# Spimp/sparc_ldpc

Hardware: AMD Instinct MI355X
Metric: decoded codewords/sec (T AMP iters) at L=512,M=512; achieved HBM GB/s vs roofline (higher is better)
Workload: dtype f32; 1 GPU; BASELINE configs[1]: L=512 M=512 R=1 P=4, T=64, single codeword; L=512, M=512, n=4608, T=64, backend=hadamard, precision=fp32, early_stop=False, parallelism=reps sharded over 1 GPU(s)

## Files before the change

### include/sparc_amp.h

```cpp
#ifndef SPARC_AMP_H
#define SPARC_AMP_H

#include <stdint.h>

#ifdef __cplusplus
extern "C" {
#endif

typedef struct sa_ctx sa_ctx;

enum {
  SA_OK = 0,
  SA_ERR_ARG = -1,
  SA_ERR_HIP = -2,
  SA_ERR_NOMEM = -3,
  SA_ERR_ORDERING = -4,
  SA_ERR_UNSUPPORTED = -5,
  SA_ERR_NO_DEVICE = -6
};

enum {
  SA_BACKEND_HADAMARD = 0,
  SA_BACKEND_DENSE = 1,
  SA_BACKEND_HOST = 2,
  SA_BACKEND_MATRIX = 3
};

enum { SA_PREC_F32 = 0, SA_PREC_F64 = 1 };

enum {
  SA_FLAG_NO_EARLY_STOP = 1,
  SA_FLAG_BETA0 = 0x100,
  SA_PTR_DEVICE = 0x200
};

int sa_create(sa_ctx** out, int L, int M, int n, const uint32_t* ordering,
              int backend, int precision, int device);

enum {
  SA_PLAN_DEFAULT = 0,
  SA_PLAN_SEC3 = 1 << 0,
  SA_PLAN_NO_SEC3 = 1 << 1,
  SA_PLAN_ROW16 = 1 << 2,
  SA_PLAN_NO_ROW16 = 1 << 3,
  SA_PLAN_NO_PT = 1 << 4,
  SA_PLAN_ZIL = 1 << 5,
  SA_PLAN_NO_ZIL = 1 << 6,
  SA_PLAN_WB8 = 1 << 7,
  SA_PLAN_WB16 = 1 << 8,
  SA_PLAN_NO_BANKS = 1 << 9,
  SA_PLAN_EAGER = 1 << 10,
  SA_PLAN_ONE_PASS = 1 << 11,
  SA_PLAN_NO_LANES = 1 << 12,
  SA_PLAN_SEC4Q = 1 << 13,
  SA_PLAN_NO_SEC4Q = 1 << 14,
  SA_PLAN_NO_FUSED_TAIL = 1 << 15,
  SA_PLAN_ALL = (1 << 16) - 1
};
int sa_create_ex(sa_ctx** out, int L, int M, int n, const uint32_t* ordering,
                 int backend, int precision, int device, int plan);

int sa_create_matrix(sa_ctx** out, int L, int M, int n, const double* A,
                     int precision, int device);

int sa_create_matrix_random(sa_ctx** out, int L, int M, int n, uint64_t seed, double scale,
                            int precision, int device);

int sa_subset(const sa_ctx* parent, const int64_t* sections, int Ls, sa_ctx** out);

int sa_create_twin(sa_ctx* src, sa_ctx** out);

void sa_destroy(sa_ctx* ctx);

int sa_Ab(sa_ctx* ctx, int B, const double* beta, double* out);

int sa_Az(sa_ctx* ctx, int B, const double* z, double* out);

int sa_amp(sa_ctx* ctx, int B, const double* y, const double* Pl, int T,
           const double* beta0, double* beta_out, int* iters_out, int flags);

int sa_reserve(sa_ctx* ctx, int B, int T);
int sa_stage(sa_ctx* ctx, int B, const double* y, const double* Pl, const double* beta0);
int sa_stage_power_batch(sa_ctx* ctx, int B, const double* Pl);
int sa_run(sa_ctx* ctx, int B, int T, int flags);
int sa_wait(sa_ctx* ctx);
int sa_fetch(sa_ctx* ctx, int B, double* beta_out, int* iters_out);
int sa_fetch_z(sa_ctx* ctx, int B, double* z_out);
int sa_fetch_y(sa_ctx* ctx, int B, double* y_out);
double sa_run_event_ms(sa_ctx* ctx);

int sa_profile(sa_ctx* ctx, int B, int T, int flags, double* out);
int sa_profile_kinds(void);
int sa_profile_rep(sa_ctx* ctx, int B, int T, int flags, int rep, double* out);
int sa_profile_dispatch(sa_ctx* ctx, int B, int T, int flags, double* out);

int sa_decide(sa_ctx* ctx, int B, int32_t* idx_out);

enum { SA_DECIDE_SLOTS = 4 };
int sa_decide_async(sa_ctx* ctx, int B, int slot);
int sa_decide_collect(sa_ctx* ctx, int B, int slot, int32_t* idx_out);


int sa_encode(sa_ctx* ctx, int B, const int32_t* idx, const double* noise);

int sa_stage_onehot(sa_ctx* ctx, int B, const int32_t* idx);

int sa_stage_onehot_scaled(sa_ctx* ctx, int B, const int32_t* idx, double scale);

int sa_llr(sa_ctx* ctx, int B, int l0, int ns, double* llr, int flags);

enum { SA_LLR_REFERENCE = 0, SA_LLR_TWO_SIDED = 1 };
int sa_llr_ex(sa_ctx* ctx, int B, int l0, int ns, double* llr, int flags, int mode, double clip);

int sa_soft_beta0(sa_ctx* ctx, int B, int l0, int ns, const double* app, int flags);

int sa_hard_cancel(sa_ctx* ctx, int B, int l0, int ns, const double* app, int flags, sa_ctx* dst,
                   int32_t* idx_out);

int sa_threshold(sa_ctx* ctx, int B, int l0, int ns, const double* app, int flags, double threshold,
                 int32_t* idx_out);

int sa_cancel(sa_ctx* ctx, int B, const int32_t* idx, sa_ctx* dst);

int sa_cancel_scaled(sa_ctx* ctx, int B, const int32_t* idx, double scale, sa_ctx* dst);

int sa_host_init(sa_ctx* ctx, int B, int T, const double* y, const double* Pl, const double* beta0,
                 const double* ab0);
int sa_host_tau(sa_ctx* ctx, int B, int t, int flags, int* stopped);
int sa_host_eta(sa_ctx* ctx, int B, int t, int flags, const double* az);
int sa_host_residual(sa_ctx* ctx, int B, int t, int flags, const double* ab);

int sa_draw_reps(const uint32_t* seeds, int count, int L, int M, int n, double sigma, int32_t* idx_out,
                 double* noise_out, int threads);
int sa_mc_stage(sa_ctx* ctx, int nreps, const int32_t* idx, const double* noise);
int sa_mc_run(sa_ctx* ctx, int B, int T, int flags, int32_t* dec_out, int32_t* iters_out, int32_t* errs_out,
              double* ms_out);
int sa_mc_draw(sa_ctx* ctx, int nreps, const uint32_t* seeds, const double* sigma, double* ms_out);
int sa_mc_fetch_draws(sa_ctx* ctx, int nreps, int32_t* idx_out, double* noise_out);
int sa_make_ordering(int L, int M, int n, uint32_t seed, uint32_t* out);

enum { SA_SE_MAX_M = 4096 };
int sa_se(int device, int B, int L, int M, int n, const double* Pl, const double* sigma, int T, int S,
          const uint32_t* seeds, const double* U, double* tau2_out, double* x_out, int64_t* miss_out,
          double* sec_out, double* ms_out);
int sa_se_draws(int device, int S, int M, const uint32_t* seeds, double* U_out);

typedef enum sa_sec_path {
  SA_SEC_K_SEC = 0,
  SA_SEC_K_SEC2 = 1,
  SA_SEC_K_SECB = 2,
  SA_SEC_DENSE = 3,
  SA_SEC_K_SEC4 = 4,
  SA_SEC_K_SEC43 = 5,
  SA_SEC_DENSE_I8 = 6,
  SA_SEC_MATRIX = 7,
  SA_SEC_K_SECG = 8,
  SA_SEC_K_SEC44 = 9
} sa_sec_path;
typedef enum sa_row_kernel {
  SA_ROW_K_ROW = 0,
  SA_ROW_K_ROW2 = 1,
  SA_ROW_K_ROWV16 = 2,
  SA_ROW_K_ROWV8 = 3,
  SA_ROW_K_ROW2_16 = 4,
  SA_ROW_K_ROWC = 5
} sa_row_kernel;
int sa_plan(sa_ctx* ctx, int B, int64_t* out8);
int sa_plan_batched(sa_ctx* ctx, int B, int64_t* out4);
int sa_info(const sa_ctx* ctx, int64_t* out8);
int sa_device_count(void);
const char* sa_last_error(void);
const char* sa_version(void);

#ifdef __cplusplus
}
#endif
#endif
```

### sparc_ldpc_amd/_lib.py

```python
from __future__ import annotations

import ctypes as ct
import os

import numpy as np

LIB_NAME = "libsparc_amp.so"
LIB_PATH = os.environ.get("SPARC_AMP_LIB") or os.path.join(os.path.dirname(os.path.abspath(__file__)), LIB_NAME)

SA_OK = 0
SA_ERR_ARG = -1
SA_ERR_HIP = -2
SA_ERR_NOMEM = -3
SA_ERR_ORDERING = -4
SA_ERR_UNSUPPORTED = -5
SA_ERR_NO_DEVICE = -6

SA_BACKEND_HADAMARD = 0
SA_BACKEND_DENSE = 1
SA_BACKEND_HOST = 2
SA_BACKEND_MATRIX = 3
SA_PREC_F32 = 0
SA_PREC_F64 = 1
SA_FLAG_NO_EARLY_STOP = 1
SA_FLAG_BETA0 = 0x100
SA_PTR_DEVICE = 0x200
SA_SE_MAX_M = 4096
SA_LLR_MODES = {"reference": 0, "two_sided": 1}

SA_PLAN = {
    "SEC3": 1 << 0, "NO_SEC3": 1 << 1, "ROW16": 1 << 2, "NO_ROW16": 1 << 3, "NO_PT": 1 << 4,
    "ZIL": 1 << 5, "NO_ZIL": 1 << 6, "WB8": 1 << 7, "WB16": 1 << 8, "NO_BANKS": 1 << 9, "EAGER": 1 << 10,
    "ONE_PASS": 1 << 11, "NO_LANES": 1 << 12, "SEC4Q": 1 << 13, "NO_SEC4Q": 1 << 14,
    "NO_FUSED_TAIL": 1 << 15,
}


def plan_bits(plan) -> int:
    if plan is None:
        return 0
    if isinstance(plan, int):
        return plan
    if isinstance(plan, str):
        plan = [plan]
    bits = 0
    for name in plan:
        key = name.upper()
        if key not in SA_PLAN:
            raise ValueError(f"unknown plan option {name!r}; known: {sorted(SA_PLAN)}")
        bits |= SA_PLAN[key]
    return bits

EXPORTS = (
    "sa_create", "sa_create_ex", "sa_create_matrix", "sa_create_matrix_random", "sa_subset", "sa_create_twin", "sa_destroy", "sa_Ab", "sa_Az", "sa_amp",
    "sa_reserve", "sa_stage", "sa_stage_power_batch", "sa_run", "sa_wait", "sa_fetch", "sa_fetch_z", "sa_fetch_y", "sa_run_event_ms",
    "sa_profile", "sa_profile_rep", "sa_profile_dispatch", "sa_profile_kinds", "sa_decide",
    "sa_decide_async", "sa_decide_collect", "sa_info", "sa_device_count", "sa_last_error", "sa_version",
    "sa_encode", "sa_stage_onehot", "sa_llr", "sa_llr_ex", "sa_soft_beta0", "sa_hard_cancel",
    "sa_threshold", "sa_cancel", "sa_plan", "sa_plan_batched", "sa_stage_onehot_scaled", "sa_cancel_scaled",
    "sa_host_init", "sa_host_tau", "sa_host_eta", "sa_host_residual",
    "sa_draw_reps", "sa_mc_stage", "sa_mc_run", "sa_make_ordering", "sa_mc_draw", "sa_mc_fetch_draws",
    "sa_se", "sa_se_draws",
)

_P = ct.c_void_p
_I = ct.c_int
_D = ct.POINTER(ct.c_double)
_SIG = {
    "sa_create": (_I, [ct.POINTER(_P), _I, _I, _I, ct.POINTER(ct.c_uint32), _I, _I, _I]),
    "sa_create_ex": (_I, [ct.POINTER(_P), _I, _I, _I, ct.POINTER(ct.c_uint32), _I, _I, _I, _I]),
    "sa_create_matrix": (_I, [ct.POINTER(_P), _I, _I, _I, _D, _I, _I]),
    "sa_create_matrix_random": (_I, [ct.POINTER(_P), _I, _I, _I, ct.c_uint64, ct.c_double, _I, _I]),
    "sa_subset": (_I, [_P, ct.POINTER(ct.c_int64), _I, ct.POINTER(_P)]),
    "sa_create_twin": (_I, [_P, ct.POINTER(_P)]),
    "sa_destroy": (None, [_P]),
    "sa_Ab": (_I, [_P, _I, _D, _D]),
    "sa_Az": (_I, [_P, _I, _D, _D]),
    "sa_amp": (_I, [_P, _I, _D, _D, _I, _D, _D, ct.POINTER(ct.c_int), _I]),
    "sa_reserve": (_I, [_P, _I, _I]),
    "sa_stage": (_I, [_P, _I, _D, _D, _D]),
    "sa_stage_power_batch": (_I, [_P, _I, _D]),
    "sa_run": (_I, [_P, _I, _I, _I]),
    "sa_wait": (_I, [_P]),
    "sa_fetch": (_I, [_P, _I, _D, ct.POINTER(ct.c_int)]),
    "sa_fetch_z": (_I, [_P, _I, _D]),
    "sa_fetch_y": (_I, [_P, _I, _D]),
    "sa_run_event_ms": (ct.c_double, [_P]),
    "sa_profile": (_I, [_P, _I, _I, _I, _D]),
    "sa_profile_rep": (_I, [_P, _I, _I, _I, _I, _D]),
    "sa_profile_dispatch": (_I, [_P, _I, _I, _I, _D]),
    "sa_profile_kinds": (_I, []),
    "sa_decide_async": (_I, [_P, _I, _I]),
    "sa_decide_collect": (_I, [_P, _I, _I, ct.POINTER(ct.c_int32)]),
    "sa_decide": (_I, [_P, _I, ct.POINTER(ct.c_int32)]),
    "sa_info": (_I, [_P, ct.POINTER(ct.c_int64)]),
    "sa_device_count": (_I, []),
    "sa_last_error": (ct.c_char_p, []),
    "sa_version": (ct.c_char_p, []),
    "sa_encode": (_I, [_P, _I, ct.POINTER(ct.c_int32), _D]),
    "sa_threshold": (_I, [_P, _I, _I, _I, _P, _I, ct.c_double, ct.POINTER(ct.c_int32)]),
    "sa_cancel": (_I, [_P, _I, ct.POINTER(ct.c_int32), _P]),
    "sa_plan": (_I, [_P, _I, ct.POINTER(ct.c_int64)]),
    "sa_plan_batched": (_I, [_P, _I, ct.POINTER(ct.c_int64)]),
    "sa_stage_onehot": (_I, [_P, _I, ct.POINTER(ct.c_int32)]),
    "sa_stage_onehot_scaled": (_I, [_P, _I, ct.POINTER(ct.c_int32), ct.c_double]),
    "sa_cancel_scaled": (_I, [_P, _I, ct.POINTER(ct.c_int32), ct.c_double, _P]),
    "sa_llr": (_I, [_P, _I, _I, _I, _P, _I]),
    "sa_llr_ex": (_I, [_P, _I, _I, _I, _P, _I, _I, ct.c_double]),
    "sa_soft_beta0": (_I, [_P, _I, _I, _I, _P, _I]),
    "sa_hard_cancel": (_I, [_P, _I, _I, _I, _P, _I, _P, ct.POINTER(ct.c_int32)]),
    "sa_host_init": (_I, [_P, _I, _I, _D, _D, _D, _D]),
    "sa_host_tau": (_I, [_P, _I, _I, _I, ct.POINTER(ct.c_int)]),
    "sa_host_eta": (_I, [_P, _I, _I, _I, _D]),
    "sa_host_residual": (_I, [_P, _I, _I, _I, _D]),
    "sa_draw_reps": (_I, [ct.POINTER(ct.c_uint32), _I, _I, _I, _I, ct.c_double, ct.POINTER(ct.c_int32), _D, _I]),
    "sa_mc_stage": (_I, [_P, _I, ct.POINTER(ct.c_int32), _D]),
    "sa_mc_run": (_I, [_P, _I, _I, _I, ct.POINTER(ct.c_int32), ct.POINTER(ct.c_int32), ct.POINTER(ct.c_int32), _D]),
    "sa_make_ordering": (_I, [_I, _I, _I, ct.c_uint32, ct.POINTER(ct.c_uint32)]),
    "sa_mc_draw": (_I, [_P, _I, ct.POINTER(ct.c_uint32), _D, _D]),
    "sa_mc_fetch_draws": (_I, [_P, _I, ct.POINTER(ct.c_int32), _D]),
    "sa_se": (_I, [_I, _I, _I, _I, _I, _D, _D, _I, _I, ct.POINTER(ct.c_uint32), _D, _D, _D, ct.POINTER(ct.c_int64), _D, _D]),
    "sa_se_draws": (_I, [_I, _I, _I, ct.POINTER(ct.c_uint32), _D]),
}

_lib = None

_SRC_DIR = os.path.join(os.path.dirname(os.path.abspath(__file__)), "csrc")
_INC_DIR = os.path.join(os.path.dirname(os.path.dirname(os.path.abspath(__file__))), "include")


def source_hash() -> str:
    import hashlib
    h = hashlib.sha256()
    files = sorted(f for f in os.listdir(_SRC_DIR) if f.endswith((".hip", ".h")) or f == "Makefile")
    paths = [os.path.join(_SRC_DIR, f) for f in files]
    if os.path.isdir(_INC_DIR):
        paths += [os.path.join(_INC_DIR, f) for f in sorted(os.listdir(_INC_DIR)) if f.endswith(".h")]
    for p in paths:
        h.update(os.path.basename(p).encode() + b"\0")
        with open(p, "rb") as fh:
            h.update(fh.read())
    return h.hexdigest()[:16]


class SparcAmpError(RuntimeError):

    def __init__(self, code: int, msg: str):
        super().__init__(f"libsparc_amp error {code}: {msg}")
        self.code = code


def load(path: str = LIB_PATH) -> ct.CDLL:
    global _lib
    if _lib is not None:
        return _lib
    if not os.path.exists(path):
        raise ImportError(
            f"{path} is missing: build it with `python -c 'import __graft_entry__ as g; g.build()'` "
            "(hipcc --offload-arch=gfx950). There is no CPU fallback.")
    lib = ct.CDLL(path)
    for name, (res, args) in _SIG.items():
        if not hasattr(lib, name):
            continue
        fn = getattr(lib, name)
        fn.restype = res
        fn.argtypes = args
    _lib = lib
    return lib


class SparcAmpArgumentError(SparcAmpError, AssertionError):
    """SA_ERR_ARG: the reference's ``assert`` cases.  An AssertionError, as the
    reference raises, and a SparcAmpError like every other refusal of the library."""


def check(rc: int) -> None:
    if rc != SA_OK:
        msg = load().sa_last_error().decode(errors="replace")
        if rc == SA_ERR_ARG:
            raise SparcAmpArgumentError(rc, msg)
        raise SparcAmpError(rc, msg)


def dptr(a: np.ndarray):
    return a.ctypes.data_as(_D)
# ... 5 lines not shown
```

### sparc_ldpc_amd/csrc/sa_common.h

```cpp
#pragma once
#include <hip/hip_runtime.h>
#include <hip/hip_ext.h>

#include <cfloat>
#include <cmath>
#include <cstdint>
#include <cstdio>
#include <cstdlib>
#include <cstring>
#include <algorithm>
#include <map>
#include <random>
#include <thread>
#include <string>
#include <tuple>
#include <type_traits>
#include <vector>

#include "sparc_amp.h"

namespace sa {

extern thread_local std::string g_err;
int fail(int code, const std::string& msg);
// ... 659 lines not shown
      *reinterpret_cast<float4*>(p + e0) = make_float4(x[i], x[i + 1], x[i + 2], x[i + 3]);
    } else {
#pragma unroll
      for (int q = 0; q < Q; ++q)
        if (e0 + q < M) p[e0 + q] = x[i + q];
    }
  }
}

template <typename real, int E>
__device__ __forceinline__ void load_section_any(const real* p, real (&x)[E], int lane, int M) {
  constexpr int Q = E < 4 ? E : 4;
#pragma unroll
  for (int i = 0; i < E; i += Q) {
    const int e0 = elem_index<E>(lane, i);
    if (Q == 4 && sizeof(real) == 4 && (M & 3) == 0 && e0 + 4 <= M) {
      const float4 t = *reinterpret_cast<const float4*>(p + e0);
      x[i] = t.x; x[i + 1] = t.y; x[i + 2] = t.z; x[i + 3] = t.w;
    } else {
#pragma unroll
      for (int q = 0; q < Q; ++q) x[i + q] = e0 + q < M ? p[e0 + q] : (real)0;
    }
  }
}

template <typename real, int E>
__device__ __forceinline__ void store_section_any(real* p, const real (&x)[E], int lane, int M) {
  constexpr int Q = E < 4 ? E : 4;
#pragma unroll
  for (int i = 0; i < E; i += Q) {
    const int e0 = elem_index<E>(lane, i);
    if (Q == 4 && sizeof(real) == 4 && (M & 3) == 0 && e0 + 4 <= M) {
      *reinterpret_cast<float4*>(p + e0) = make_float4(x[i], x[i + 1], x[i + 2], x[i + 3]);
    } else {
#pragma unroll
      for (int q = 0; q < Q; ++q)
        if (e0 + q < M) p[e0 + q] = x[i + q];
    }
  }
}


enum { SEC_AMP = 0, SEC_AZ = 1, SEC_AB = 2 };
enum { ROW_INIT0 = 0, ROW_INIT = 1, ROW_AMP = 2, ROW_ABOUT = 3 };

constexpr int kSpw = 4;
constexpr int kRowsPerBlk = 64;

template <typename real>
struct SecArgs {
  const uint16_t* __restrict__ inv;
  const uint16_t* __restrict__ invb;
  const uint16_t* __restrict__ invl;
  const uint32_t* __restrict__ hs;
  const ushort4* __restrict__ fwd;
  const ushort4* __restrict__ fwdb;
  const uint32_t* __restrict__ fwd2;
  const uint32_t* __restrict__ fwd3;
  const uint32_t* __restrict__ inv32;
  const real* __restrict__ c;
  const real* __restrict__ z;
  real* __restrict__ beta;
  real* __restrict__ beta_out;
  real* __restrict__ out;
  real* __restrict__ abp;
  real* __restrict__ bbp;
  const real* __restrict__ zzp;
  real* __restrict__ tau;
  int* __restrict__ iters;
  int L, M, n, w, nhi, G, NZ, T1, t, mode, early_stop;
  int cst;
  int RS;
  int pt;
  int B, NC;
  int zil;
  int gpx;
  real sqrt_n;
  const int* tb;
  int dead;
  int bzero;
  int32_t* dec;
  int itset;
};

template <typename real>
struct RowArgs {
  const real* __restrict__ tau;
  const real* __restrict__ y;
  const real* __restrict__ z_in;
  const real* __restrict__ bbp;
  const real* __restrict__ Pb;
  const real* __restrict__ abp;
  int n, G, Gb, NZ, T1, t, mode, early_stop;
  int Pbst;
  int pt;
  int Bc;
  int itset;
  real sqrt_n;
  real* __restrict__ z;
  real* __restrict__ zzp;
  real* __restrict__ out;
  int* __restrict__ iters;
  const int* tb;
};

constexpr int kZU = 10;
#define SA_ZU_EACH(X) X(0) X(1) X(2) X(3) X(4) X(5) X(6) X(7) X(8) X(9)
template <typename real, int NT = 256>
struct ZStage {
  using vec_t = typename std::conditional<sizeof(real) == 4, f4, d2v>::type;
  static constexpr int V = 16 / sizeof(real);
#define SA_ZU_DECL(u) vec_t t##u;
  SA_ZU_EACH(SA_ZU_DECL)
#undef SA_ZU_DECL
  int nv;
  __device__ __forceinline__ void issue(const real* zb, int n, int tid) {
    nv = ((reinterpret_cast<uintptr_t>(zb) & 15) == 0) ? n / V : 0;
    const vec_t* zv = reinterpret_cast<const vec_t*>(zb);
    const int last = nv > 0 ? nv - 1 : 0;
#define SA_ZU_LOAD(u) { const int j = u * NT + tid; t##u = zv[j < nv ? j : last]; }
    SA_ZU_EACH(SA_ZU_LOAD)
#undef SA_ZU_LOAD
  }
  __device__ __forceinline__ void store(real* zs, const real* zb, int n, int tid) const {
    vec_t* zsv = reinterpret_cast<vec_t*>(zs);
    const vec_t* zv = reinterpret_cast<const vec_t*>(zb);
#define SA_ZU_STORE(u) { const int j = u * NT + tid; if (j < nv) zsv[j] = t##u; }
    SA_ZU_EACH(SA_ZU_STORE)
#undef SA_ZU_STORE
    for (int j = kZU * NT + tid; j < nv; j += NT) zsv[j] = zv[j];
    for (int i = nv * V + tid; i < n; i += NT) zs[i] = zb[i];
    if (tid == 0) zs[n] = 0;
  }
};

template <typename real, int NT, int AUX = 0>
__device__ __forceinline__ bool stage_z_dma(const real* zb, real* zs, int n, int tid) {
  if (reinterpret_cast<uintptr_t>(zb) & 15) return false;
  const int lane = tid & 63, nbytes = n * (int)sizeof(real);
  for (int ch = tid >> 6; ch * 1024 < nbytes; ch += NT / 64) {
    const int off = ch * 1024 + lane * 16;
    if (off + 16 <= nbytes)
      __builtin_amdgcn_global_load_lds((__attribute__((address_space(1))) void*)((const char*)zb + off),
                                       (__attribute__((address_space(3))) void*)((char*)zs + ch * 1024), 16, 0, AUX);
  }
  return true;
}

template <typename real>
__device__ __forceinline__ void finish_z_dma(const real* zb, real* zs, int n, int tid) {
  const int n0 = n * (int)sizeof(real) / 16 * 16 / (int)sizeof(real);
  if (tid < n - n0) zs[n0 + tid] = zb[n0 + tid];
  if (tid == 0) zs[n] = 0;
}

template <int E, int KH>
__device__ __forceinline__ void load_buckets(const uint16_t* __restrict__ il, int h0, int nhi, int M,
                                             int lane, ushort4 (&tb)[KH][(E + 3) / 4]) {
  constexpr int Q = E < 4 ? E : 4;
#pragma unroll
  for (int hh = 0; hh < KH; ++hh) {
    const int h = h0 + hh < nhi ? h0 + hh : nhi - 1;
    const uint16_t* ih = il + (size_t)h * M;
#pragma unroll
    for (int i = 0; i < E; i += Q) {
      int e0 = elem_index<E>(lane, i);
// ... 158 lines not shown
```

### sparc_ldpc_amd/csrc/sa_glue.hip

```cpp
#include "sa_host.h"

namespace sa {

template <typename real>
__global__ void __launch_bounds__(256) k_colsum(const ushort4* __restrict__ fwd, const double* __restrict__ cd,
                                                const int32_t* __restrict__ idx, int ldi, int l0, int ns,
                                                const real* __restrict__ base, const double* __restrict__ add,
                                                real* __restrict__ out, int n, double sqrt_n, double amp) {
  extern __shared__ int32_t sidx[];
  const int b = blockIdx.y, r = blockIdx.x * 256 + threadIdx.x;
  for (int i = threadIdx.x; i < ns; i += 256) sidx[i] = idx[(size_t)b * ldi + i];
  __syncthreads();
  if (r >= n) return;
  double acc = 0.0;
  const int g0 = l0 / kSpw, g1 = (l0 + ns + kSpw - 1) / kSpw;
  for (int g = g0; g < g1; ++g) {
    const ushort4 f = fwd[(size_t)g * n + r];
    const unsigned short fq[4] = {f.x, f.y, f.z, f.w};
#pragma unroll
    for (int q = 0; q < 4; ++q) {
      const int l = g * kSpw + q;
      if (l < l0 || l >= l0 + ns || sidx[l - l0] < 0) continue;
      const unsigned k = fq[q] & 0x7fffu;
      const unsigned neg = (fq[q] >> 15) ^ (__popc(k & (unsigned)sidx[l - l0]) & 1u);
// ... 165 lines not shown

int grid_of(size_t tot) {
  const size_t g = (tot + 255) / 256;
  return (int)(g < 65536 ? (g > 0 ? g : 1) : 65536);
}

constexpr int kGlueMaxM = 8192;

int check_glue(sa_ctx* c, int B, int l0, int ns) {
  if (check_ctx(c)) return SA_ERR_ARG;
  if (B <= 0 || B > c->Bcap) return fail(SA_ERR_ARG, "batch larger than the context's workspace");
  if (l0 < 0 || ns <= 0 || l0 + ns > c->L) return fail(SA_ERR_ARG, "section range outside [0, L)");
  if (!c->power_set) return fail(SA_ERR_ARG, "power allocation not staged");
  if (c->M < 2) return fail(SA_ERR_UNSUPPORTED, "M < 2 carries no bits");
  if (!c->pow2) return fail(SA_ERR_UNSUPPORTED, "bit-level glue needs M a power of two (bits2indices, sparc_ldpc.py:317)");
  if (c->M > kGlueMaxM) return fail(SA_ERR_UNSUPPORTED, "SPARC<->LDPC glue stages a section in LDS: M <= 8192");
  return SA_OK;
}

int dev_in(sa_ctx* c, const double* p, size_t count, int flags, const double** out) {
  if (flags & SA_PTR_DEVICE) {
    *out = p;
    return SA_OK;
  }
  int rc = ensure_stage(c, count);
  if (rc) return rc;
  HIP_TRY(hipMemcpyAsync(c->at().d_stage, p, count * 8, hipMemcpyHostToDevice, c->at().stream));
  *out = c->at().d_stage;
  return SA_OK;
}

template <typename real>
int launch_colsum(sa_ctx* c, const int32_t* d_idx, int ldi, int l0, int ns, const real* base, const double* add,
                  real* out, int B, double amp = 1.0) {
  dim3 grid((c->n + 255) / 256, B);
  k_colsum<real><<<grid, 256, (size_t)ns * sizeof(int32_t), c->at().stream>>>(
      (const ushort4*)c->d_fwd, c->d_cd, d_idx, ldi, l0, ns, base, add, out, c->n, std::sqrt((double)c->n), amp);
  HIP_TRY(hipGetLastError());
  return SA_OK;
}

}

using namespace sa;

extern "C" {

int sa_encode(sa_ctx* c, int B, const int32_t* idx, const double* noise) {
  if (check_ctx(c)) return SA_ERR_ARG;
  if (B <= 0 || !idx) return fail(SA_ERR_ARG, "sa_encode: bad arguments");
  if (!c->power_set) return fail(SA_ERR_ARG, "sa_encode: power allocation not staged");
  if (int rc0 = check_tables(c, "sa_encode")) return rc0;
  if (!c->pow2) return fail(SA_ERR_UNSUPPORTED, "sa_encode: the row-parallel encoder needs M a power of two");
  HIP_TRY(hipSetDevice(c->device));
  int rc = ensure_workspace(c, B, c->Tcap > 0 ? c->Tcap : 1);
  if (rc) return rc;
  sa_lane& ln = c->at();
  for (size_t i = 0; i < (size_t)B * c->L; ++i)
    if (idx[i] < 0 || idx[i] >= c->M) return fail(SA_ERR_ARG, "sa_encode: index outside [0, M)");
  HIP_TRY(hipMemcpyAsync(c->d_idx, idx, (size_t)B * c->L * sizeof(int32_t), hipMemcpyHostToDevice, ln.stream));
  const double* d_noise = nullptr;
  if (noise && (rc = dev_in(c, noise, (size_t)B * c->n, 0, &d_noise))) return rc;
  if ((rc = y_begin_write(c, ln.stream, B))) return rc;
  rc = c->prec == SA_PREC_F64
           ? launch_colsum<double>(c, c->d_idx, c->L, 0, c->L, nullptr, d_noise, (double*)ln.d_y, B)
           : launch_colsum<float>(c, c->d_idx, c->L, 0, c->L, nullptr, d_noise, (float*)ln.d_y, B);
  if (rc) return rc;
  HIP_TRY(hipStreamSynchronize(ln.stream));
  return y_mark(c);
}

namespace {
int stage_onehot_impl(sa_ctx* c, int B, const int32_t* idx, double scale, bool allow_empty) {
  if (check_ctx(c)) return SA_ERR_ARG;
  if (B <= 0 || B > c->Bcap || !idx) return fail(SA_ERR_ARG, "sa_stage_onehot: bad arguments");
  if (!c->power_set) return fail(SA_ERR_ARG, "sa_stage_onehot: power allocation not staged");
  if (!std::isfinite(scale)) return fail(SA_ERR_ARG, "sa_stage_onehot: scale must be finite");
  if (c->dead) return fail(SA_ERR_UNSUPPORTED, "sa_stage_onehot: M must be a power of two (bits2indices)");
  for (size_t i = 0; i < (size_t)B * c->L; ++i)
    if (idx[i] >= c->M || (idx[i] < 0 && !(allow_empty && idx[i] == -1)))
      return fail(SA_ERR_ARG, "sa_stage_onehot: index outside [0, M)");
  HIP_TRY(hipSetDevice(c->device));
  sa_lane& ln = c->at();
  ln.fused_B = 0;
  HIP_TRY(hipMemcpyAsync(c->d_idx, idx, (size_t)B * c->L * sizeof(int32_t), hipMemcpyHostToDevice, ln.stream));
  const size_t tot = (size_t)B * c->L * c->M;
  if (c->prec == SA_PREC_F64)
    k_onehot<double><<<grid_of(tot), 256, 0, ln.stream>>>(c->d_idx, c->d_cd, c->L, c->M, B, scale, (double*)ln.d_beta);
  else
    k_onehot<float><<<grid_of(tot), 256, 0, ln.stream>>>(c->d_idx, c->d_cd, c->L, c->M, B, scale, (float*)ln.d_beta);
  HIP_TRY(hipGetLastError());
  HIP_TRY(hipStreamSynchronize(ln.stream));
  return SA_OK;
}
}

int sa_stage_onehot(sa_ctx* c, int B, const int32_t* idx) { return stage_onehot_impl(c, B, idx, 1.0, false); }

int sa_stage_onehot_scaled(sa_ctx* c, int B, const int32_t* idx, double scale) {
  return stage_onehot_impl(c, B, idx, scale, true);
}

int sa_llr(sa_ctx* c, int B, int l0, int ns, double* llr, int flags) {
  return sa_llr_ex(c, B, l0, ns, llr, flags, SA_LLR_REFERENCE, INFINITY);
}

int sa_llr_ex(sa_ctx* c, int B, int l0, int ns, double* llr, int flags, int mode, double clip) {
  int rc = check_glue(c, B, l0, ns);
  if (rc) return rc;
  if (!llr) return fail(SA_ERR_ARG, "sa_llr: llr is NULL");
  if (mode != SA_LLR_REFERENCE && mode != SA_LLR_TWO_SIDED) return fail(SA_ERR_ARG, "sa_llr_ex: unknown mode");
  if (!(clip >= 0.0)) return fail(SA_ERR_ARG, "sa_llr_ex: clip must be positive, or 0 / +inf for none");
  const double lim = std::isinf(clip) ? 0.0 : clip;
  HIP_TRY(hipSetDevice(c->device));
  sa_lane& ln = c->at();
  const int lgM = ilog2(c->M);
  const size_t cnt = (size_t)B * ns * lgM;
  double* d_out = llr;
  if (!(flags & SA_PTR_DEVICE)) {
    if ((rc = ensure_stage(c, cnt))) return rc;
    d_out = ln.d_stage;
  }
  const size_t lds = (size_t)c->M * sizeof(double);
  if (mode == SA_LLR_TWO_SIDED) {
    if (c->prec == SA_PREC_F64)
      k_llr2<double><<<B * ns, 64, lds, ln.stream>>>((const double*)ln.d_beta, c->d_cd, c->L, c->M, lgM, l0, ns, lim,
                                                     d_out);
    else
      k_llr2<float><<<B * ns, 64, lds, ln.stream>>>((const float*)ln.d_beta, c->d_cd, c->L, c->M, lgM, l0, ns, lim,
                                                    d_out);
  } else {
    if (c->prec == SA_PREC_F64)
      k_llr<double><<<B * ns, 64, lds, ln.stream>>>((const double*)ln.d_beta, c->d_cd, c->L, c->M, lgM, l0, ns, d_out);
    else
      k_llr<float><<<B * ns, 64, lds, ln.stream>>>((const float*)ln.d_beta, c->d_cd, c->L, c->M, lgM, l0, ns, d_out);
    if (lim > 0.0) k_llr_clip<<<grid_of(cnt), 256, 0, ln.stream>>>(d_out, cnt, lim);
  }
  HIP_TRY(hipGetLastError());
  if (!(flags & SA_PTR_DEVICE)) HIP_TRY(hipMemcpyAsync(llr, d_out, cnt * 8, hipMemcpyDeviceToHost, ln.stream));
  HIP_TRY(hipStreamSynchronize(ln.stream));
  return SA_OK;
}

int sa_soft_beta0(sa_ctx* c, int B, int l0, int ns, const double* app, int flags) {
  int rc = check_glue(c, B, l0, ns);
  if (rc) return rc;
  if (!app) return fail(SA_ERR_ARG, "sa_soft_beta0: app is NULL");
  HIP_TRY(hipSetDevice(c->device));
  sa_lane& ln = c->at();
  ln.fused_B = 0;
  const int lgM = ilog2(c->M);
  const size_t na = (size_t)B * ns * lgM;
  const double* d_app = app;
  if (!(flags & SA_PTR_DEVICE)) {
    if ((rc = ensure_stage(c, na))) return rc;
    HIP_TRY(hipMemcpyAsync(ln.d_stage, app, na * 8, hipMemcpyHostToDevice, ln.stream));
    d_app = ln.d_stage;
  }
  const size_t tot = (size_t)B * c->L * c->M, lds = (size_t)c->M * sizeof(double);
  if (c->prec == SA_PREC_F64) {
    if (ns < c->L) k_rescale<double><<<grid_of(tot), 256, 0, ln.stream>>>((double*)ln.d_beta, c->d_cd, c->L, c->M, l0, ns, B);
    k_soft_sec<double><<<B * ns, 64, lds, ln.stream>>>(d_app, c->d_cd, c->L, c->M, lgM, l0, ns, (double*)ln.d_beta);
  } else {
    if (ns < c->L) k_rescale<float><<<grid_of(tot), 256, 0, ln.stream>>>((float*)ln.d_beta, c->d_cd, c->L, c->M, l0, ns, B);
    k_soft_sec<float><<<B * ns, 64, lds, ln.stream>>>(d_app, c->d_cd, c->L, c->M, lgM, l0, ns, (float*)ln.d_beta);
  }
  HIP_TRY(hipGetLastError());
  HIP_TRY(hipStreamSynchronize(ln.stream));
  return SA_OK;
}

int sa_hard_cancel(sa_ctx* c, int B, int l0, int ns, const double* app, int flags, sa_ctx* dst, int32_t* idx_out) {
  if (dst && check_tables(c, "sa_hard_cancel")) return SA_ERR_UNSUPPORTED;
  int rc = check_glue(c, B, l0, ns);
  if (rc) return rc;
  if (!app) return fail(SA_ERR_ARG, "sa_hard_cancel: app is NULL");
  if (dst && (dst->n != c->n || dst->prec != c->prec || dst->device != c->device))
    return fail(SA_ERR_ARG, "sa_hard_cancel: dst must share n, precision and device");
  HIP_TRY(hipSetDevice(c->device));
  if (dst && (rc = ensure_workspace(dst, B, dst->Tcap > 0 ? dst->Tcap : 1))) return rc;
  sa_lane& ln = c->at();
  const int lgM = ilog2(c->M);
  const double* d_app = nullptr;
  if ((rc = dev_in(c, app, (size_t)B * ns * lgM, flags, &d_app))) return rc;
  k_app_idx<<<(B * ns + 255) / 256, 256, 0, ln.stream>>>(d_app, lgM, ns, B, c->d_idx);
  HIP_TRY(hipGetLastError());
  if (dst) {
    if ((rc = y_sync(c)) || (rc = y_begin_write(dst, ln.stream, B))) return rc;
    rc = c->prec == SA_PREC_F64
             ? launch_colsum<double>(c, c->d_idx, ns, l0, ns, (const double*)ln.d_y, nullptr, (double*)dst->at().d_y, B)
             : launch_colsum<float>(c, c->d_idx, ns, l0, ns, (const float*)ln.d_y, nullptr, (float*)dst->at().d_y, B);
    if (rc) return rc;
  }
  if (idx_out)
    HIP_TRY(hipMemcpyAsync(idx_out, c->d_idx, (size_t)B * ns * sizeof(int32_t), hipMemcpyDeviceToHost, ln.stream));
  HIP_TRY(hipStreamSynchronize(ln.stream));
  return dst ? y_mark(dst) : SA_OK;
}

int sa_threshold(sa_ctx* c, int B, int l0, int ns, const double* app, int flags, double threshold,
                 int32_t* idx_out) {
  int rc = check_glue(c, B, l0, ns);
  if (rc) return rc;
  if (!app || !idx_out) return fail(SA_ERR_ARG, "sa_threshold: null argument");
  HIP_TRY(hipSetDevice(c->device));
  sa_lane& ln = c->at();
  const int lgM = ilog2(c->M);
  const double* d_app = nullptr;
  if ((rc = dev_in(c, app, (size_t)B * ns * lgM, flags, &d_app))) return rc;
  k_threshold<<<B * ns, 256, (size_t)c->M * sizeof(double), ln.stream>>>(d_app, c->M, lgM, ns, threshold, c->d_idx);
  HIP_TRY(hipGetLastError());
  HIP_TRY(hipMemcpyAsync(idx_out, c->d_idx, (size_t)B * ns * sizeof(int32_t), hipMemcpyDeviceToHost, ln.stream));
  HIP_TRY(hipStreamSynchronize(ln.stream));
  return SA_OK;
}

int sa_cancel_scaled(sa_ctx* c, int B, const int32_t* idx, double scale, sa_ctx* dst) {
  if (check_ctx(c) || check_ctx(dst)) return SA_ERR_ARG;
  if (int rc0 = check_tables(c, "sa_cancel")) return rc0;
  if (!c->pow2) return fail(SA_ERR_UNSUPPORTED, "sa_cancel: needs M a power of two");
  if (B <= 0 || B > c->Bcap || !idx) return fail(SA_ERR_ARG, "sa_cancel: bad arguments");
  if (!c->power_set) return fail(SA_ERR_ARG, "sa_cancel: power allocation not staged");
  if (dst->n != c->n || dst->prec != c->prec || dst->device != c->device)
    return fail(SA_ERR_ARG, "sa_cancel: dst must share n, precision and device");
  for (size_t i = 0; i < (size_t)B * c->L; ++i)
    if (idx[i] >= c->M) return fail(SA_ERR_ARG, "sa_cancel: index >= M");
  if (!std::isfinite(scale)) return fail(SA_ERR_ARG, "sa_cancel: scale must be finite");
  HIP_TRY(hipSetDevice(c->device));
  int rc;
  if ((rc = ensure_workspace(dst, B, dst->Tcap > 0 ? dst->Tcap : 1))) return rc;
  sa_lane& ln = c->at();
  HIP_TRY(hipMemcpyAsync(c->d_idx, idx, (size_t)B * c->L * sizeof(int32_t), hipMemcpyHostToDevice, ln.stream));
  if ((rc = y_sync(c)) || (rc = y_begin_write(dst, ln.stream, B))) return rc;
// ... 12 lines not shown
```

### sparc_ldpc_amd/csrc/sa_host.h

```cpp
#pragma once
#include "sa_common.h"

namespace sa {

struct Prof {
  std::vector<std::tuple<int, hipEvent_t, hipEvent_t>> ev;
  int rep = 1;
  bool dispatch = false;
  int kind = 0;
  int begin(hipStream_t s, int k) {
    kind = k;
    if (dispatch) return 0;
    hipEvent_t a = nullptr, b = nullptr;
    if (add(&a, &b)) return -1;
    return hipEventRecord(a, s) == hipSuccess ? 0 : -1;
  }
  void end(hipStream_t s) {
    if (!dispatch) (void)hipEventRecord(std::get<2>(ev.back()), s);
  }
  int add(hipEvent_t* a, hipEvent_t* b) {
    *a = *b = nullptr;
    if (hipEventCreate(a) != hipSuccess || hipEventCreate(b) != hipSuccess) return -1;
    ev.emplace_back(kind, *a, *b);
    return 0;
  }
  ~Prof() {
    for (auto& e : ev) {
      (void)hipEventDestroy(std::get<1>(e));
      (void)hipEventDestroy(std::get<2>(e));
    }
  }
};

enum { K_SEC = 0, K_ROW = 1, K_DAZ = 2, K_DDEN = 3, K_DAB = 4, K_QNT = 5, K_NKINDS = 6 };

}

struct sa_lane {
  hipStream_t stream = nullptr;
  hipEvent_t ev0 = nullptr, ev1 = nullptr;
  void *d_y = nullptr, *d_z = nullptr, *d_beta = nullptr, *d_abp = nullptr;
  void *d_bbp = nullptr, *d_zzp = nullptr, *d_tau = nullptr;
  void* d_beta2 = nullptr;
  int* d_iters = nullptr;
  double* d_stage = nullptr;
  size_t stage_cap = 0;
  int beta2_cap = 0;
  std::map<std::tuple<int, int, int, int>, hipGraphExec_t> graphs;
  hipEvent_t y_ev = nullptr;
  unsigned long long y_ver = 0;
  bool y_read = false;
  int32_t *h_dec = nullptr, *d_dec = nullptr;
  int fused_B = 0;
  int row_B = 0, row_T = 0;
};

struct sa_ctx {
  sa::Prof* prof = nullptr;
  enum { kLanes = 2 };
  sa_lane lane[kLanes];
  int cur = 0;
  sa_lane& at() { return lane[cur]; }
  const sa_lane& at() const { return lane[cur]; }
  bool lanes_on = false;
  unsigned long long y_ver = 0;
  int y_lane = 0;
  std::vector<double> h_Pl;
  std::vector<double> h_Plb;
  int L = 0, M = 0, n = 0, w = 0, nhi = 0, backend = 0, prec = 0, device = 0;
  int plan = 0;
  bool pow2 = true;
  int Mu = 0, dead = 0;
  int G = 0, NZ = 0, E = 1;
  int n_cus = 256;
  int Gb = 0, CB = 0;
  int WB = 8;
  int gpx = 1 << 20;
  size_t secb_lds = 0;
  int RS = 1, KS = 1, Gd = 0;
  size_t lda = 0;
  size_t sec_lds = 0;
  int G2 = 0;
  int G3 = 0;
  bool sec3 = false;
  size_t sec3_lds = 0;
  int G4 = 0;
  bool sec4q = false;
  size_t sec4q_lds = 0;
  uint32_t* d_fwd3 = nullptr;
  bool pt_on = false;
  bool sec4 = false;
  size_t sec4_lds = 0;
  int NZ16 = 0;
  int NZh = 0;
  bool row16 = false;
  int NZ4 = 0, NZ2 = 0;
  bool zil_last = false;
  size_t sec2_lds = 0;
  std::vector<uint32_t> ordering;
  uint16_t* d_inv = nullptr;
  bool big = false;
  uint32_t* d_inv32 = nullptr;
  uint16_t* d_invb = nullptr;
  uint16_t* d_fwdb = nullptr;
  uint16_t* d_invl = nullptr;
  uint32_t* d_hs = nullptr;
  bool borrowed = false;
  bool invb_done = false;
  uint16_t* d_fwd = nullptr;
  uint32_t* d_fwd2 = nullptr;
  void* d_A = nullptr;
  int8_t *d_A8 = nullptr, *d_AT8 = nullptr, *d_zq = nullptr, *d_bq = nullptr;
  double *d_zsc = nullptr, *d_bsc0 = nullptr, *d_bfix = nullptr;
  long long np8 = 0, LMp8 = 0;
  int Bp8 = 0;
  long long np = 0, nk = 0, LMy = 0;
  void *d_AT = nullptr, *d_xz = nullptr, *d_xb = nullptr;
  int fg_cap = 0;
  double cmax = 0;
  int Bcap = 0, Tcap = 0;
  void *d_out = nullptr, *d_c = nullptr, *d_azp = nullptr;
  int* d_stop = nullptr;
  int32_t* d_idx = nullptr;
  double* d_cd = nullptr;
  double P = 0;
  bool power_set = false;
  void* d_cb = nullptr;
  void* d_Pb = nullptr;
  void* d_P1 = nullptr;
  bool pb_on = false;
  bool shared_power = false;
  size_t bytes = 0;
  int last_B = 0, last_T = 0;
  int32_t* h_dec = nullptr;
  int32_t* d_dec = nullptr;
  size_t dec_cap = 0;
  hipEvent_t dec_ev[SA_DECIDE_SLOTS] = {};
// ... 47 lines not shown
  return SA_OK;
}

constexpr int kI8MinB = 4;
constexpr int kI8MaxS = 16;
constexpr int kFMinB = 4;
constexpr int kFMaxS = 16;

inline size_t rsz(const sa_ctx* c) { return c->prec == SA_PREC_F64 ? 8 : 4; }

inline bool is_dense(const sa_ctx* c) { return c->backend == SA_BACKEND_DENSE || c->backend == SA_BACKEND_MATRIX; }
inline bool use_i8(const sa_ctx* c, int B) { return c->backend == SA_BACKEND_DENSE && B >= kI8MinB; }
inline bool use_fgemm(const sa_ctx* c, int B) { return c->backend == SA_BACKEND_MATRIX && B >= kFMinB; }
inline bool use_batched(const sa_ctx* c, int B) { return c->CB > 0 && B >= 4; }

inline bool zil_for(const sa_ctx* c, int B) {
  const bool on = (c->plan & SA_PLAN_NO_ZIL) ? false : true;
  return on && c->backend == SA_BACKEND_HADAMARD && use_batched(c, B) && c->CB * (int)rsz(c) == 16;
}

int dense_parts(const sa_ctx* c, int B);

struct Plan {
  sa_sec_path sec = SA_SEC_K_SEC;
  sa_row_kernel row = SA_ROW_K_ROW;
  int nz = 0;
  int G = 0, Gb = 0;
  int pt = 0;
  int rs = 1;
  int CB = 1;
  bool zil = false;
  bool dense() const { return sec == SA_SEC_DENSE || sec == SA_SEC_DENSE_I8 || sec == SA_SEC_MATRIX; }
  bool batched() const { return sec == SA_SEC_K_SECB; }
  bool multiwave() const {
    return sec == SA_SEC_K_SEC2 || sec == SA_SEC_K_SEC4 || sec == SA_SEC_K_SEC43 || sec == SA_SEC_K_SEC44;
  }
  bool row_sets_iters() const { return row == SA_ROW_K_ROW2 || row == SA_ROW_K_ROW2_16; }
  bool it_row() const { return !dense() && !batched() && row_sets_iters(); }
  bool bzero() const { return sec == SA_SEC_K_SEC4 || sec == SA_SEC_K_SEC43 || sec == SA_SEC_K_SEC44; }
};

inline Plan plan_for(const sa_ctx* c, int B) {
  Plan p;
  const bool f32 = c->prec == SA_PREC_F32;
  p.zil = zil_for(c, B);
  if (p.zil) {
    p.row = SA_ROW_K_ROWC; p.nz = c->NZ2;
  } else if ((long long)B * c->NZ < 4LL * c->n_cus) {
    if (c->row16 && B == 1) { p.row = SA_ROW_K_ROW2_16; p.nz = c->NZh; }
    else { p.row = SA_ROW_K_ROW2; p.nz = c->NZ16; }
  } else if (c->n % (f32 ? 4 : 2) == 0 && (long long)B * (f32 ? c->NZ4 : c->NZ2) >= 2LL * c->n_cus) {
    p.row = SA_ROW_K_ROWV16; p.nz = f32 ? c->NZ4 : c->NZ2;
  } else if (f32 && c->n % 2 == 0 && (long long)B * c->NZ2 >= 2LL * c->n_cus) {
    p.row = SA_ROW_K_ROWV8; p.nz = c->NZ2;
  } else {
    p.row = SA_ROW_K_ROW; p.nz = c->NZ;
  }
  const int wgs = c->G * B;
  p.rs = std::min(4, std::max(1, (c->n_cus + wgs - 1) / wgs));
  if (is_dense(c)) {
    p.sec = use_i8(c, B) ? SA_SEC_DENSE_I8 : (use_fgemm(c, B) ? SA_SEC_MATRIX : SA_SEC_DENSE);
    p.G = dense_parts(c, B);
    p.Gb = c->Gd;
  } else if (use_batched(c, B)) {
    p.sec = SA_SEC_K_SECB;
    p.G = p.Gb = c->Gb;
    p.CB = c->CB;
  } else if (c->backend == SA_BACKEND_HADAMARD && c->G2 > 0 && c->G2 * B * 2 >= c->n_cus) {
    p.sec = c->sec3 ? SA_SEC_K_SEC43 : (c->sec4q ? SA_SEC_K_SEC44 : (c->sec4 ? SA_SEC_K_SEC4 : SA_SEC_K_SEC2));
    p.G = p.Gb = c->sec3 ? c->G3 : (c->sec4q ? c->G4 : c->G2);
    if (p.sec != SA_SEC_K_SEC2 && p.row_sets_iters() && c->pt_on) p.pt = p.row == SA_ROW_K_ROW2_16 ? 16 : kRow2Rows;
  } else {
    p.sec = c->big ? SA_SEC_K_SECG : SA_SEC_K_SEC;
    p.G = p.Gb = c->G;
  }
  return p;
}

inline bool fused_tail(const sa_ctx* c, const Plan& p, int T, int flags) {
  return p.bzero() && p.it_row() && (flags & SA_FLAG_NO_EARLY_STOP) && T > 0 && c->dead == 0 && !c->prof &&
         !(c->plan & SA_PLAN_NO_FUSED_TAIL);
}

template <typename real>
SecArgs<real> sec_args(sa_ctx* c, const Plan& p, int mode, int t, int early_stop, const int* tb = nullptr) {
  SecArgs<real> a;
  const sa_lane& ln = c->at();
  a.inv = c->d_inv; a.inv32 = c->d_inv32; a.invb = c->d_invb; a.invl = c->d_invl; a.hs = c->d_hs;
  a.fwd = (const ushort4*)c->d_fwd;
  a.fwdb = (const ushort4*)c->d_fwdb; a.fwd2 = c->d_fwd2; a.fwd3 = c->d_fwd3; a.c = (const real*)c->d_c;
  a.z = (const real*)ln.d_z; a.beta = (real*)ln.d_beta; a.beta_out = (real*)ln.d_beta; a.out = (real*)c->d_out;
  a.abp = (real*)ln.d_abp; a.bbp = (real*)ln.d_bbp; a.zzp = (const real*)ln.d_zzp;
  a.tau = (real*)ln.d_tau; a.iters = ln.d_iters;
  a.L = c->L; a.M = c->M; a.n = c->n; a.w = c->w; a.nhi = c->nhi; a.G = c->G; a.NZ = p.nz;
  a.T1 = c->Tcap + 1; a.t = t; a.mode = mode; a.early_stop = early_stop;
  a.RS = 1;
  a.pt = 0;
  a.B = 0; a.NC = 0; a.zil = 0; a.gpx = 1 << 20;
  a.cst = c->pb_on ? c->L : 0;
  if (c->pb_on) a.c = (const real*)c->d_cb;
  a.sqrt_n = (real)std::sqrt((double)c->n);
  a.tb = tb;
  a.dead = c->dead;
  a.bzero = 0;
  a.dec = nullptr;
  a.itset = 0;
  return a;
}

template <typename real>
RowArgs<real> row_args(sa_ctx* c, const Plan& p, int mode, int t, int early_stop, int G, int Gb, const int* tb = nullptr) {
  RowArgs<real> a;
  const sa_lane& ln = c->at();
  a.y = (const real*)ln.d_y; a.z = (real*)ln.d_z; a.z_in = a.z; a.abp = (const real*)ln.d_abp;
  a.bbp = (const real*)ln.d_bbp; a.zzp = (real*)ln.d_zzp; a.tau = (const real*)ln.d_tau;
  a.out = (real*)c->d_out;
  a.n = c->n; a.G = G; a.NZ = p.nz;
  a.Gb = Gb; a.T1 = c->Tcap + 1; a.t = t; a.mode = mode;
  a.early_stop = early_stop;
  a.sqrt_n = c->backend != SA_BACKEND_HADAMARD ? (real)1 : (real)std::sqrt((double)c->n);
  a.Pb = c->pb_on ? (const real*)c->d_Pb : (const real*)c->d_P1;
  a.Pbst = c->pb_on ? 1 : 0;
  a.pt = 0;
  a.Bc = 0;
  a.tb = tb;
  a.iters = ln.d_iters;
  a.itset = 0;
  return a;
}

template <typename F>
void parallel_for(int count, int grain, F f) {
  const int blocks = (count + grain - 1) / grain;
  unsigned nth = std::thread::hardware_concurrency();
  nth = nth == 0 ? 1 : (nth > 16 ? 16 : nth);
  if ((int)nth > blocks) nth = blocks > 0 ? blocks : 1;
  auto run = [&](int t) {
    for (int b = t; b < blocks; b += (int)nth)
      for (int i = b * grain; i < count && i < (b + 1) * grain; ++i) f(i);
  };
  std::vector<std::thread> th;
  for (int t = 1; t < (int)nth; ++t) th.emplace_back(run, t);
  run(0);
  for (auto& x : th) x.join();
}

int check_ctx(const sa_ctx* c);
int check_tables(const sa_ctx* c, const char* what);
int dev_alloc(sa_ctx* c, void** p, size_t bytes);
void dev_free(void* p);
using GraphMap = std::map<std::tuple<int, int, int, int>, hipGraphExec_t>;
void graphs_clear(GraphMap& m);
void drop_graphs(sa_ctx* c);
int sync_all(sa_ctx* c);
inline void lane_switch(sa_ctx* c, int k) { c->cur = k; }
int lanes_release(sa_ctx* c);
int row_flush(sa_ctx* c, int k);
inline int tail_settle(sa_ctx* c) {
  c->at().fused_B = 0;
  return row_flush(c, c->cur);
}
int y_sync(sa_ctx* c, int k);
int y_begin_write(sa_ctx* c, int k, hipStream_t s, int B);
int y_mark(sa_ctx* c, int k);
inline int y_sync(sa_ctx* c) { return y_sync(c, c->cur); }
inline int y_begin_write(sa_ctx* c, hipStream_t s, int B) { return y_begin_write(c, c->cur, s, B); }
inline int y_mark(sa_ctx* c) { return y_mark(c, c->cur); }
int ensure_workspace(sa_ctx* c, int B, int T);
int ensure_stage(sa_ctx* c, sa_lane& l, size_t count);
int upload(sa_ctx* c, sa_lane& l, void* dst, const double* src, size_t count);
int download(sa_ctx* c, sa_lane& l, double* dst, const void* src, size_t count);
inline int ensure_stage(sa_ctx* c, size_t count) { return ensure_stage(c, c->at(), count); }
inline int upload(sa_ctx* c, void* dst, const double* src, size_t count) { return upload(c, c->at(), dst, src, count); }
inline int download(sa_ctx* c, double* dst, const void* src, size_t count) { return download(c, c->at(), dst, src, count); }
int set_power(sa_ctx* c, const double* Pl);
int ensure_invb(sa_ctx* c);
int create_impl(sa_ctx** out, int L, int M, int n, const uint32_t* ordering, int backend, int prec, int device,
                int plan, const sa_ctx* share = nullptr);
extern __global__ void k_fill32(uint32_t* p, uint32_t v, size_t nw);

template <typename real>
int launch_sec(sa_ctx* c, const Plan& p, int B, int mode, int t, int es, void* bin = nullptr, void* bout = nullptr);
template <typename real>
int launch_sec2(sa_ctx* c, const Plan& p, int B, int t, int es, void* bin, void* bout, int bzero = 0,
                int32_t* dec = nullptr, int itset = 0);
hipError_t sec_lds_attrs();

template <typename real>
int launch_secb(sa_ctx* c, const Plan& p, int B, int t, int es, const int* tb = nullptr);
hipError_t secb_lds_attrs();
bool secb_no_static_lds();

template <typename real>
int launch_row(sa_ctx* c, const Plan& p, int B, int mode, int t, int es, int G, int Gb, int itset = 0,
               const int* tb = nullptr);
int launch_decide(sa_ctx* c, int B, int32_t* idx);

int dense_den_groups(const sa_ctx* c);
template <typename real>
int dense_start(sa_ctx* c, const Plan& p, int B);
template <typename real>
int dense_iter(sa_ctx* c, const Plan& p, int B, int t, int es);
template <typename real>
int dense_ab(sa_ctx* c, const Plan& p, int B);
template <typename real>
int dense_az(sa_ctx* c, const Plan& p, int B);
int ensure_i8(sa_ctx* c, int B);
int ensure_fgemm(sa_ctx* c, int B);
int i8_set_bfix(sa_ctx* c);
int build_dense(sa_ctx* c);
int matrix_init(sa_ctx* c);
hipError_t dense_lds_attrs();

void mc_release(sa_ctx* c);
hipError_t mc_lds_attrs();

#ifdef SA_STAMPS
hipError_t stamps_add_sec(unsigned long long* out);
hipError_t stamps_add_secb(unsigned long long* out);
#endif

}
```

### sparc_ldpc_amd/csrc/sa_mc.hip

```cpp
#include "sa_host.h"
#include "legacy_mt.h"
#include "legacy_mt_dev.h"

#include <thread>

namespace sa {

using legacy_rng::LegacyMT;


struct McArgs {
  int* rep;
  int* tb;
  int* done;
  int* fresh;
  int* fin_list;
  int* fresh_list;
  int* ctl;
  int* iters;
  int32_t* dec;
  int32_t* its;
  int32_t* errs;
  const int32_t* idx;
  const double* noise;
// ... 402 lines not shown
}

int sa_mc_stage(sa_ctx* c, int nreps, const int32_t* idx, const double* noise) {
  if (check_tables(c, "sa_mc_stage")) return SA_ERR_UNSUPPORTED;
  if (nreps <= 0 || !idx || !noise) return fail(SA_ERR_ARG, "sa_mc_stage: bad arguments");
  for (size_t i = 0; i < (size_t)nreps * c->L; ++i)
    if (idx[i] < 0 || idx[i] >= c->M) return fail(SA_ERR_ARG, "sa_mc_stage: index outside [0, M)");
  HIP_TRY(hipSetDevice(c->device));
  lane_switch(c, 0);
  if (int rc = mc_ensure_reps(c, nreps)) return rc;
  HIP_TRY(hipMemcpyAsync(c->d_mc_idx, idx, (size_t)nreps * c->L * sizeof(int32_t), hipMemcpyHostToDevice, c->at().stream));
  HIP_TRY(hipMemcpyAsync(c->d_mc_noise, noise, (size_t)nreps * c->n * sizeof(double), hipMemcpyHostToDevice,
                         c->at().stream));
  HIP_TRY(hipStreamSynchronize(c->at().stream));
  c->mc_nreps = nreps;
  return SA_OK;
}

int sa_mc_draw(sa_ctx* c, int nreps, const uint32_t* seeds, const double* sigma, double* ms_out) {
  if (int rc = check_tables(c, "sa_mc_draw")) return rc;
  if (nreps <= 0 || !seeds || !sigma) return fail(SA_ERR_ARG, "sa_mc_draw: bad arguments");
  if (!c->pow2 || c->M < 2)
    return fail(SA_ERR_UNSUPPORTED, "sa_mc_draw: the device generator draws randint(0, M) for M a power of two only");
  if (c->n > (1 << 27) || c->L > (1 << 27)) return fail(SA_ERR_UNSUPPORTED, "sa_mc_draw: n or L above 2^27");
  HIP_TRY(hipSetDevice(c->device));
  lane_switch(c, 0);
  int rc;
  if ((rc = mc_ensure_reps(c, nreps))) return rc;
  if ((rc = mc_ensure_seeds(c, nreps))) return rc;
  c->mc_nreps = 0;
  sa_lane& ln = c->at();
  HIP_TRY(hipMemcpyAsync(c->d_mc_seeds, seeds, (size_t)nreps * sizeof(uint32_t), hipMemcpyHostToDevice, ln.stream));
  HIP_TRY(hipMemcpyAsync(c->d_mc_sigma, sigma, (size_t)nreps * sizeof(double), hipMemcpyHostToDevice, ln.stream));
  HIP_TRY(hipMemsetAsync(c->d_mc_err, 0, sizeof(int), ln.stream));
  HIP_TRY(hipEventRecord(ln.ev0, ln.stream));
  k_mc_draw<<<nreps, legacy_rng_dev::kThreads, 0, ln.stream>>>(c->d_mc_seeds, c->d_mc_sigma, c->d_mc_idx,
                                                                c->d_mc_noise, c->L, c->M, c->n,
                                                                legacy_rng_dev::randn_chunk_cap(c->n), c->d_mc_err);
  HIP_TRY(hipGetLastError());
  HIP_TRY(hipEventRecord(ln.ev1, ln.stream));
  int err = 0;
  HIP_TRY(hipMemcpyAsync(&err, c->d_mc_err, sizeof(int), hipMemcpyDeviceToHost, ln.stream));
  HIP_TRY(hipStreamSynchronize(ln.stream));
  if (err) return fail(SA_ERR_HIP, "sa_mc_draw: a rep's randn ran into the chunk cap");
  if (ms_out) {
    float ms = -1.f;
    HIP_TRY(hipEventElapsedTime(&ms, ln.ev0, ln.ev1));
    *ms_out = ms;
  }
  c->mc_nreps = nreps;
  return SA_OK;
}

int sa_mc_fetch_draws(sa_ctx* c, int nreps, int32_t* idx_out, double* noise_out) {
  if (check_ctx(c)) return SA_ERR_ARG;
  if (nreps <= 0 || nreps > c->mc_nreps) return fail(SA_ERR_ARG, "sa_mc_fetch_draws: nreps outside the staged reps");
  HIP_TRY(hipSetDevice(c->device));
  hipStream_t st = c->lane[0].stream;
  if (idx_out)
    HIP_TRY(hipMemcpyAsync(idx_out, c->d_mc_idx, (size_t)nreps * c->L * sizeof(int32_t), hipMemcpyDeviceToHost, st));
  if (noise_out)
    HIP_TRY(hipMemcpyAsync(noise_out, c->d_mc_noise, (size_t)nreps * c->n * sizeof(double), hipMemcpyDeviceToHost, st));
  HIP_TRY(hipStreamSynchronize(st));
  return SA_OK;
}

int sa_mc_run(sa_ctx* c, int B, int T, int flags, int32_t* dec_out, int32_t* iters_out, int32_t* errs_out,
              double* ms_out) {
  if (check_ctx(c)) return SA_ERR_ARG;
  if (B < 4 || B > kMcStepThreads || T <= 0) return fail(SA_ERR_ARG, "sa_mc_run: B in [4, 1024], T > 0");
  if (c->mc_nreps <= 0) return fail(SA_ERR_ARG, "sa_mc_run: no reps staged (sa_mc_stage)");
  if (!c->shared_power || c->pb_on) return fail(SA_ERR_ARG, "sa_mc_run: one power allocation must be staged");
  if (c->backend != SA_BACKEND_HADAMARD || !c->pow2 || c->big || !zil_for(c, B))
    return fail(SA_ERR_UNSUPPORTED, "sa_mc_run: needs the batched codeword-interleaved Hadamard decode "
                                    "(k_secb + k_rowc)");
  HIP_TRY(hipSetDevice(c->device));
  lane_switch(c, 0);
  int rc;
  if ((rc = ensure_workspace(c, B, T))) return rc;
  if ((rc = ensure_invb(c))) return rc;
  if ((rc = mc_ensure_slots(c, B))) return rc;
  sa_lane& ln = c->at();
  ln.row_B = ln.row_T = 0;
  ln.fused_B = 0;
  if (!c->h_mc_live) {
    HIP_TRY(hipHostMalloc((void**)&c->h_mc_live, 4 * sizeof(int), hipHostMallocDefault));
    for (auto& e : c->mc_ev) HIP_TRY(hipEventCreateWithFlags(&e, hipEventDisableTiming));
  }
  const int es = (flags & SA_FLAG_NO_EARLY_STOP) ? 0 : 1;
  const bool f64 = c->prec == SA_PREC_F64;
  const int nreps = c->mc_nreps;
  const Plan p = plan_for(c, B);
  c->zil_last = true;
  {
    const int S = c->slot_cap, n0 = std::min(B, nreps);
    std::vector<int> h(6 * (size_t)S + 8, -1);
    for (int b = 0; b < S; ++b) {
      const bool on = b < n0;
      h[b] = on ? b : -1;
      h[S + b] = on ? 0 : -1;
      h[2 * (size_t)S + b] = -1;
      h[3 * (size_t)S + b] = on ? 1 : 0;
      h[5 * (size_t)S + b] = b;
    }
    int* ctl = h.data() + 6 * (size_t)S;
    ctl[0] = n0;
    ctl[1] = n0;
    ctl[2] = nreps;
    ctl[3] = 0;
    ctl[4] = n0;
    HIP_TRY(hipMemcpyAsync(c->d_slots, h.data(), h.size() * sizeof(int), hipMemcpyHostToDevice, ln.stream));
    HIP_TRY(hipMemsetAsync(ln.d_beta, 0, (size_t)B * c->L * c->M * rsz(c), ln.stream));
    k_fill32<<<(B + 255) / 256, 256, 0, ln.stream>>>((uint32_t*)ln.d_iters, 0xffffffffu, (size_t)B);
    k_fill32<<<(nreps + 255) / 256, 256, 0, ln.stream>>>((uint32_t*)(c->d_mc_its + c->mc_cap), 0u, (size_t)nreps);
    HIP_TRY(hipGetLastError());
    HIP_TRY(hipStreamSynchronize(ln.stream));
  }
  HIP_TRY(hipEventRecord(ln.ev0, ln.stream));
  const McArgs a = mc_args(c, B, T);
  if ((rc = f64 ? mc_encode_all<double>(c, a, nreps) : mc_encode_all<float>(c, a, nreps))) return rc;
  if ((rc = f64 ? mc_turnover<double>(c, a) : mc_turnover<float>(c, a))) return rc;
  const int K = 8;
  const auto key = std::make_tuple(B, T, K, flags & 0xff);
  auto it = c->mc_graphs.find(key);
  if (it == c->mc_graphs.end()) {
    hipGraphExec_t ex = nullptr;
    rc = capture_graph(ln.stream, [&] {
      return f64 ? mc_iterations<double>(c, p, B, T, K, es) : mc_iterations<float>(c, p, B, T, K, es);
    }, &ex);
    if (rc) return rc;
    it = c->mc_graphs.emplace(key, ex).first;
  }
  const long long max_replays = ((long long)(nreps + B - 1) / B * T + T + K - 1) / K + 2;
  int* live_dev = c->d_slots + 6 * c->slot_cap + 1;
  long long r = 0;
  for (; r < max_replays; ++r) {
    HIP_TRY(hipGraphLaunch(it->second, ln.stream));
    HIP_TRY(hipMemcpyAsync(c->h_mc_live + (r & 3), live_dev, sizeof(int), hipMemcpyDeviceToHost, ln.stream));
    HIP_TRY(hipEventRecord(c->mc_ev[r & 3], ln.stream));
    if (r >= 2) {
      HIP_TRY(hipEventSynchronize(c->mc_ev[(r - 2) & 3]));
      if (c->h_mc_live[(r - 2) & 3] == 0) break;
    }
  }
  HIP_TRY(hipEventRecord(ln.ev1, ln.stream));
  HIP_TRY(hipStreamSynchronize(ln.stream));
  int ctl[2] = {0, 0};
  HIP_TRY(hipMemcpy(ctl, c->d_slots + 6 * c->slot_cap, sizeof(ctl), hipMemcpyDeviceToHost));
  if (ctl[1] != 0 || ctl[0] != nreps) return fail(SA_ERR_HIP, "sa_mc_run: the stream did not drain");
  if (ms_out) {
    float ms = -1.f;
    HIP_TRY(hipEventElapsedTime(&ms, ln.ev0, ln.ev1));
    *ms_out = ms;
  }
  if (dec_out)
    HIP_TRY(hipMemcpyAsync(dec_out, c->d_mc_dec, (size_t)nreps * c->L * sizeof(int32_t), hipMemcpyDeviceToHost,
                           ln.stream));
  if (iters_out)
    HIP_TRY(hipMemcpyAsync(iters_out, c->d_mc_its, (size_t)nreps * sizeof(int32_t), hipMemcpyDeviceToHost, ln.stream));
  if (errs_out)
    HIP_TRY(hipMemcpyAsync(errs_out, c->d_mc_its + c->mc_cap, (size_t)nreps * sizeof(int32_t), hipMemcpyDeviceToHost,
                           ln.stream));
  HIP_TRY(hipStreamSynchronize(ln.stream));
  c->last_B = B;
  c->last_T = T;
  return SA_OK;
// ... 4 lines not shown
```

### sparc_ldpc_amd/csrc/sa_row.hip

```cpp
#include "sa_host.h"

namespace sa {

template <typename real, int kRowWaves>
__global__ void __launch_bounds__(kRowWaves * 64) k_row(RowArgs<real> a) {
  __shared__ real red[kRowWaves][kRowsPerBlk];
  const int b = blockIdx.y, tid = threadIdx.x, lane = tid & 63, wv = tid >> 6;
  const int r = blockIdx.x * kRowsPerBlk + lane;
  const int n = a.n;
  real tau = 1, last = 0;
  if (a.mode == ROW_AMP) {
    tau = ld_vmem(a.tau + (size_t)b * a.T1 + a.t);
    last = a.t > 0 ? ld_vmem(a.tau + (size_t)b * a.T1 + a.t - 1) : (real)0;
  }
  const size_t o = (size_t)b * n + (r < n ? r : 0);
  real yv = 0, zv = 0, Pv = 0, bbv[2] = {0, 0};
  if (wv == 0) {
    yv = a.y[o];
    if (a.mode == ROW_AMP) {
      zv = a.z[o];
      Pv = ld_vmem(a.Pb + (size_t)b * a.Pbst);
      const real* bp = a.bbp + (size_t)b * a.Gb;
      bbv[0] = lane < a.Gb ? bp[lane] : (real)0;
      bbv[1] = lane + 64 < a.Gb ? bp[lane + 64] : (real)0;
// ... 296 lines not shown
    constexpr int U = 256 / NG;
    if (pt && (R == 16 || sizeof(real) == 4) && G == NG * U) {
      const real* pb = abp_p + (size_t)b * G * ((size_t)NZ * R) + (size_t)blockIdx.x * G * R;
      real tt[U];
#pragma unroll
      for (int u = 0; u < U; ++u)
        tt[u] = ld_off(pb, (unsigned)(((pg + NG * u) * R + rl) * (int)sizeof(real)));
#pragma unroll
      for (int u = 0; u < U; ++u) acc += tt[u];
    } else if (pt && (R == 16 || sizeof(real) == 4) && G == NG * (U / 2)) {
      constexpr int UH = U / 2;
      const real* pb = abp_p + (size_t)b * G * ((size_t)NZ * R) + (size_t)blockIdx.x * G * R;
      real tt[UH];
#pragma unroll
      for (int u = 0; u < UH; ++u)
        tt[u] = ld_off(pb, (unsigned)(((pg + NG * u) * R + rl) * (int)sizeof(real)));
#pragma unroll
      for (int u = 0; u < UH; ++u) acc += tt[u];
    } else
    for (int g0 = pg; g0 < G; g0 += NG * U) {
      real tt[U];
#pragma unroll
      for (int u = 0; u < U; ++u) {
        const int g = g0 + NG * u;
        tt[u] = p[(size_t)(g < G ? g : pg) * gs];
      }
#pragma unroll
      for (int u = 0; u < U; ++u)
        if (g0 + NG * u < G) acc += tt[u];
    }
    red[pg][rl] = acc;
  }
  if (mode == ROW_AMP && es && tau == last) return;
  const real tau2 = tau * tau;
  __syncthreads();
  if (tid >= 64) return;
  if (itset != 0 && blockIdx.x == 0 && tid == 0) iters_p[b] = itset;
  real ons = 0;
  if (mode == ROW_AMP) {
    real bb;
    if (Gb <= 256) {
      real sacc = 0;
#pragma unroll
      for (int q = 0; q < 4; ++q) sacc += bbv[q];
      bb = wave_sum(sacc);
    } else {
      bb = wave_sum_parts(bbp_p + (size_t)b * Gb, Gb);
    }
    ons = Pv - bb / (real)n;
  }
  real zn = 0;
  if (tid < R && r < n) {
    if (mode == ROW_INIT0) {
      zn = yv;
    } else {
      real acc = 0;
#pragma unroll
      for (int q = 0; q < NG; ++q) acc += red[q][rl];
      const real ab = acc / sqrt_n;
      if (mode == ROW_ABOUT) {
        out_p[o] = ab;
        return;
      }
      zn = yv - ab;
      if (mode == ROW_AMP) zn += (zv / tau2) * ons;
    }
    z_p[o] = zn;
  }
  if (mode == ROW_ABOUT) return;
  const real sz = wave_sum(zn * zn);
  if (tid == 0) zzp_p[(size_t)b * NZ + blockIdx.x] = sz;
}

template <typename real, int E>
__global__ void __launch_bounds__(256) k_decide(const real* beta, int32_t* idx, int L, int M, int dead) {
  const int lane = threadIdx.x & 63;
  const int l = blockIdx.x * 4 + (threadIdx.x >> 6), b = blockIdx.y;
  if (l >= L) return;
  const int bi = section_argmax<real, E>(beta + ((size_t)b * L + l) * M, lane, M, dead);
  if (lane == 0) idx[(size_t)b * L + l] = bi;
}

template <typename real>
int launch_row(sa_ctx* c, const Plan& p, int B, int mode, int t, int es, int G, int Gb, int itset, const int* tb) {
  RowArgs<real> a = row_args<real>(c, p, mode, t, es, G, Gb, tb);
  a.pt = mode == ROW_AMP ? p.pt : 0;
  if (itset && !p.row_sets_iters()) return fail(SA_ERR_UNSUPPORTED, "launch_row: only k_row2 writes iters");
  a.itset = itset;
  if (c->prof) c->prof->begin(c->at().stream, K_ROW);
  switch (mode == ROW_ABOUT ? SA_ROW_K_ROW : p.row) {
    case SA_ROW_K_ROWC: {
      constexpr int CBz = 16 / (int)sizeof(real);
      a.Bc = B;
      if ((a.G + 3) / 4 > 8 && (a.G + 3) / 4 <= 12)
        plaunch(c, k_rowc<real, CBz, 12>, dim3(p.nz, (B + CBz - 1) / CBz), 256, 0, a, mode == ROW_AMP ? 1 : 0);
      else
        plaunch(c, k_rowc<real, CBz>, dim3(p.nz, (B + CBz - 1) / CBz), 256, 0, a, mode == ROW_AMP ? 1 : 0);
      break;
    }
    case SA_ROW_K_ROW2: plaunch(c, k_row2<real>, dim3(p.nz, B), 512, 0, a); break;
    case SA_ROW_K_ROW2_16: plaunch(c, k_row2<real, 16>, dim3(p.nz, B), 512, 0, a); break;
    case SA_ROW_K_ROWV16: {
      constexpr int V = 16 / (int)sizeof(real);
      plaunch(c, k_rowv<real, V>, dim3(p.nz, B), 256, 0, a);
      break;
    }
    case SA_ROW_K_ROWV8:
      if constexpr (sizeof(real) == 4) {
        plaunch(c, k_rowv<float, 2>, dim3(p.nz, B), 256, 0, a);
        break;
      } else {
        return SA_ERR_UNSUPPORTED;
      }
    case SA_ROW_K_ROW: plaunch(c, k_row<real, 4>, dim3(c->NZ, B), 4 * 64, 0, a); break;
  }
  if (c->prof) c->prof->end(c->at().stream);
  HIP_TRY(hipGetLastError());
  return SA_OK;
}

int launch_decide(sa_ctx* c, int B, int32_t* idx) {
  dim3 grid((c->L + 3) / 4, B);
  const sa_lane& ln = c->at();
#define SA_DEC(EE)                                                                                             \
  case EE:                                                                                                     \
    if (c->prec == SA_PREC_F64)                                                                                \
      k_decide<double, EE><<<grid, 256, 0, ln.stream>>>((const double*)ln.d_beta, idx, c->L, c->M, c->dead);   \
    else                                                                                                       \
      k_decide<float, EE><<<grid, 256, 0, ln.stream>>>((const float*)ln.d_beta, idx, c->L, c->M, c->dead);     \
    break;
  switch (c->E) { SA_DEC(1) SA_DEC(2) SA_DEC(4) SA_DEC(8) SA_DEC(16) SA_DEC(32) SA_DEC(64) }
#undef SA_DEC
  HIP_TRY(hipGetLastError());
  return SA_OK;
}

template int launch_row<float>(sa_ctx*, const Plan&, int, int, int, int, int, int, int, const int*);
template int launch_row<double>(sa_ctx*, const Plan&, int, int, int, int, int, int, int, const int*);

}
```

### sparc_ldpc_amd/csrc/sa_sec.hip

```cpp
#include "sa_host.h"

namespace sa {



template <typename real, int E>
__global__ void __launch_bounds__(256) k_sec(SecArgs<real> a) {
  STAMP(0);
  extern __shared__ __attribute__((aligned(16))) unsigned char smem[];
  constexpr int KH = E >= 16 ? 2 : (E >= 8 ? 16 : 16);
  constexpr int NQ = (E + 3) / 4;
  constexpr int KR = 8;
  int g, rsi;
  if (a.RS > 1 && (a.G & 7) == 0) {
    const int j = blockIdx.x, u = j >> 3;
    rsi = u % a.RS;
    g = (u / a.RS) * 8 + (j & 7);
  } else {
    g = blockIdx.x / a.RS;
    rsi = blockIdx.x % a.RS;
  }
  const int b = blockIdx.y;
  const int rows_per = (a.n + a.RS - 1) / a.RS;
  const int rb0 = rsi * rows_per, rb1 = min(a.n, rb0 + rows_per);
// ... 398 lines not shown
  S2 = red[w0 * 4 + 2] + red[(w0 + 1) * 4 + 2];
  const real scale = cl / S;
#pragma unroll
  for (int i = 0; i < E2; ++i) v[i] = have ? v[i] * scale : (real)0;
  if (have) store_section<real, E2>(blo, v, lane, Mh);
  const real bb = have ? S2 * scale * scale : (real)0;

  STAMP(5);
  fwht_wave<real, E2>(v, lane, 64);
  top_bit_stage<real, E2>(v, mine, other, lane, w);
  STAMP(6);
  {
    real* tl = ts + sidx * M + eoff;
#pragma unroll
    for (int i = 0; i < E2; ++i) tl[elem_index<E2>(lane, i)] = v[i];
  }
  if (lane == 0) red[wv * 4 + 3] = bb;
  __syncthreads();
  STAMP(7);
  if (tid == 0) a.bbp[(size_t)b * a.G + g] = red[0 * 4 + 3] + red[2 * 4 + 3];
  real* abp = a.abp + ((size_t)b * a.G + g) * n;
  for (int r0 = 0; r0 < n; r0 += 256 * KR) {
    if (r0 > 0) {
#pragma unroll
      for (int u = 0; u < KR; ++u) {
        const int r = r0 + u * 256 + tid;
        f[u] = fw[r < n ? r : 0];
      }
    }
#pragma unroll
    for (int u = 0; u < KR; ++u) {
      const int r = r0 + u * 256 + tid;
      if (r < n) {
        const uint32_t e = f[u];
        const real v0 = ts[e & 0x7fffu];
        const real v1 = ts[M + ((e >> 16) & 0x7fffu)];
        real t = (e & 0x8000u) ? -v0 : v0;
        t += (e & 0x80000000u) ? -v1 : v1;
        st_part(&abp[r], t);
      }
    }
  }
#ifdef SA_STAMPS
  STAMP(8);
  asm volatile("s_waitcnt vmcnt(0)" ::: "memory");
  STAMP(9);
#endif
}
template <typename real, int EQ, int QW>
__device__ __forceinline__ void topq_stage(real (&v)[EQ], real* xs, int lane, int q) {
  constexpr int QS = EQ * 64;
#pragma unroll
  for (int i = 0; i < EQ; ++i) xs[q * QS + i * 64 + lane] = v[i];
  __syncthreads();
#pragma unroll
  for (int i = 0; i < EQ; ++i) {
    real x[QW];
#pragma unroll
    for (int j = 0; j < QW; ++j) x[j] = xs[j * QS + i * 64 + lane];
#pragma unroll
    for (int k = 0, span = 1; span < QW; ++k, span <<= 1)
#pragma unroll
      for (int j = 0; j < QW; j += 2 * span) x[j] = ((q >> k) & 1) ? x[j] - x[j + span] : x[j] + x[j + span];
    v[i] = x[0];
  }
  __syncthreads();
}

template <typename real, int QW, bool MAX>
__device__ __forceinline__ real combine_q(const real* red, int w0, int f) {
  real x[QW];
#pragma unroll
  for (int j = 0; j < QW; ++j) x[j] = red[(w0 + j) * 4 + f];
#pragma unroll
  for (int span = 1; span < QW; span <<= 1)
#pragma unroll
    for (int j = 0; j < QW; j += 2 * span) {
      if constexpr (MAX) x[j] = x[j] > x[j + span] ? x[j] : x[j + span];
      else x[j] = x[j] + x[j + span];
    }
  return x[0];
}

template <typename real, int EQ, int QW, int SPW = 2>
__device__ __forceinline__ void secq_body(const SecArgs<real>& a) {
  static_assert(SPW == 2 || SPW == 3 || SPW == 4, "sections per workgroup");
  STAMP(0);
  extern __shared__ __attribute__((aligned(16))) unsigned char smem[];
  constexpr int NT = SPW * QW * 64;
  constexpr int KH = EQ >= 8 ? 4 : ((SPW == 3 || (SPW == 4 && sizeof(real) == 8)) ? 8 : 16);
  constexpr int NQ = (EQ + 3) / 4;
  constexpr int KR = ((SPW == 3 ? 8448 : 4608) + NT - 1) / NT;
  constexpr int FW = SPW == 4 ? 2 : 1;
  const int g = blockIdx.x, b = blockIdx.y;
  const int tid = threadIdx.x, lane = tid & 63, wv = tid >> 6;
  const int sidx = wv / QW, q = wv % QW;
  const int M = a.M, n = a.n, Mq = M / QW;
  const size_t LM = (size_t)a.L * M;
  const int l = g * SPW + sidx;
  const bool have = l < a.L;
  const int lc = have ? l : a.L - 1;
  const int eoff = q * Mq;

  real* zs = reinterpret_cast<real*>(smem);
  const int zslots = ((n + 1) * (int)sizeof(real) + 15) / 16 * 16 / (int)sizeof(real);
  real* ts = zs + zslots;
  real* xb = ts + SPW * M;
  real* red = xb + SPW * M;

  real v[EQ];
  real bprev[EQ];
  const real* bl = a.beta + (size_t)b * LM + (size_t)lc * M + eoff;
  real* blo = a.beta_out + (size_t)b * LM + (size_t)lc * M + eoff;
  const uint16_t* ibase = a.inv + (size_t)g * SPW * a.w;
  const unsigned ioff = (unsigned)((lc - g * SPW) * a.w + eoff);
  const uint32_t* fw = (SPW == 3 ? a.fwd3 : a.fwd2) + (size_t)(SPW == 4 ? 2 * g : g) * n;
  const uint32_t* fw1 = a.fwd2 + (size_t)(2 * g + 1 < (a.L + 1) / 2 ? 2 * g + 1 : 2 * g) * n;
  ushort4 tb[KH][NQ];
  uint32_t f[KR][FW];

  const real* zb = a.z + (size_t)b * n;
  ZStage<real, NT> zst;
  const real* zzb = a.zzp + (size_t)b * a.NZ;
  ZZParts<real, 5> zz;
  const bool dma = stage_z_dma<real, NT>(zb, zs, n, tid);
  if (!dma) zst.issue(zb, n, tid);
  zz.issue(zzb, a.NZ, lane);
  const real last = a.t > 0 ? ld_vmem(a.tau + (size_t)b * a.T1 + a.t - 1) : (real)0;
  load_buckets_off<EQ, KH>(ibase, ioff, 0, a.nhi, M, lane, tb);
  load_section<real, EQ>(bl, bprev, lane, Mq);
  const real cl = ld_vmem(a.c + (size_t)b * a.cst + lc);
  const real tau = zz.tau(zzb, a.NZ, n);
  if (a.bzero) {
#pragma unroll
    for (int i = 0; i < EQ; ++i) bprev[i] = 0;
  }
  const bool stop = a.early_stop && (tau == last);
  if (g == 0 && tid == 0) {
    a.tau[(size_t)b * a.T1 + a.t] = tau;
    if (stop && a.iters[b] < 0) a.iters[b] = a.t;
    if (a.itset != 0 && !stop) a.iters[b] = a.itset;
  }
  if (stop) {
    if (dma) asm volatile("s_waitcnt vmcnt(0)" ::: "memory");
    if (a.bzero && have) {
      store_section<real, EQ>(a.beta + (size_t)b * LM + (size_t)lc * M + eoff, bprev, lane, Mq);
    }
    return;
  }
  const real tau2 = tau * tau;
  const real inv_sn = (real)1 / a.sqrt_n;
  const real kk = cl / tau2;
  STAMP(1);
  if (!dma) zst.store(zs, zb, n, tid);
  else finish_z_dma<real>(zb, zs, n, tid);
  __syncthreads();
  STAMP(2);
#ifdef SA_STAMPS
  asm volatile("s_waitcnt vmcnt(0)" ::: "memory");
  STAMP(10);
#endif
#pragma unroll
  for (int i = 0; i < EQ; ++i) v[i] = 0;
  for (int h0 = 0; h0 < a.nhi; h0 += KH) {
    ushort4 tn[KH][NQ];
    const bool more = h0 + KH < a.nhi;
    if (more) load_buckets_off<EQ, KH>(ibase, ioff, h0 + KH, a.nhi, M, lane, tn);
    gather_buckets<real, EQ, KH>(zs, h0, a.nhi, tb, v);
    if (more) {
#pragma unroll
      for (int hh = 0; hh < KH; ++hh)
#pragma unroll
        for (int j = 0; j < NQ; ++j) tb[hh][j] = tn[hh][j];
    }
  }
  real* xs = xb + sidx * M;
#pragma unroll
  for (int u = 0; u < KR; ++u) {
    const int r = u * NT + tid;
    f[u][0] = ld_off(fw, (unsigned)(r < n ? r : 0) * 4u);
    if constexpr (SPW == 4) f[u][1] = ld_off(fw1, (unsigned)(r < n ? r : 0) * 4u);
  }
  STAMP(3);
  fwht_wave<real, EQ>(v, lane, 64);
  topq_stage<real, EQ, QW>(v, xs, lane, q);
  STAMP(4);


  real mx = neg_inf<real>();
#pragma unroll
  for (int i = 0; i < EQ; ++i) {
    v[i] = fma(v[i], inv_sn, bprev[i]) * kk;
    mx = v[i] > mx ? v[i] : mx;
  }
  mx = wave_max(mx);
  if (lane == 0) red[wv * 4] = mx;
  __syncthreads();
  const int w0 = wv & ~(QW - 1);
  mx = combine_q<real, QW, true>(red, w0, 0);
  real S = 0, S2 = 0;
#pragma unroll
  for (int i = 0; i < EQ; ++i) {
    v[i] = dexp<real>(v[i] - mx);
    S += v[i];
    S2 += v[i] * v[i];
  }
  wave_sum2(S, S2);
  if (lane == 0) {
    red[wv * 4 + 1] = S;
    red[wv * 4 + 2] = S2;
  }
  __syncthreads();
  S = combine_q<real, QW, false>(red, w0, 1);
  S2 = combine_q<real, QW, false>(red, w0, 2);
  const real scale = cl * rcp_fast(S);
#pragma unroll
  for (int i = 0; i < EQ; ++i) v[i] = have ? v[i] * scale : (real)0;
  if (have) store_section<real, EQ>(blo, v, lane, Mq);
  const real bb = have ? S2 * scale * scale : (real)0;
  real dbest = neg_inf<real>();
  int dbi = M;
  if (a.dec) {
#pragma unroll
    for (int i = 0; i < EQ; ++i) {
      const int e = eoff + elem_index<EQ>(lane, i);
      if (v[i] > dbest || (v[i] == dbest && e < dbi)) { dbest = v[i]; dbi = e; }
    }
#pragma unroll
    for (int m = 32; m >= 1; m >>= 1) {
      const real ob = __shfl_xor(dbest, m);
      const int oi = __shfl_xor(dbi, m);
      if (ob > dbest || (ob == dbest && oi < dbi)) { dbest = ob; dbi = oi; }
    }
  }

  STAMP(5);
  fwht_wave<real, EQ>(v, lane, 64);
  topq_stage<real, EQ, QW>(v, xs, lane, q);
  STAMP(6);
  {
    real* tl = ts + sidx * M + eoff;
#pragma unroll
    for (int i = 0; i < EQ; ++i) tl[elem_index<EQ>(lane, i)] = v[i];
  }
  if (lane == 0) {
    red[wv * 4 + 3] = bb;
    if (a.dec) {
      red[wv * 4] = dbest;
      red[wv * 4 + 1] = (real)dbi;
    }
  }
  __syncthreads();
  STAMP(7);
  if (a.dec && have && q == 0 && lane == 0) {
    real best = red[wv * 4];
    int bi = (int)red[wv * 4 + 1];
#pragma unroll
    for (int j = 1; j < QW; ++j) {
      const real ob = red[(wv + j) * 4];
      const int oi = (int)red[(wv + j) * 4 + 1];
      if (ob > best || (ob == best && oi < bi)) { best = ob; bi = oi; }
    }
    a.dec[(size_t)b * a.L + l] = bi >= M ? 0 : bi;
  }
  if (tid == 0) {
    real bsum = red[0 * 4 + 3] + red[QW * 4 + 3];
    if constexpr (SPW >= 3) bsum += red[2 * QW * 4 + 3];
    if constexpr (SPW == 4) bsum += red[3 * QW * 4 + 3];
    a.bbp[(size_t)b * a.G + g] = bsum;
  }
  real* abp = a.abp + ((size_t)b * a.G + g) * n;
  const int psh = a.pt == 16 ? 4 : 5;
  const size_t npad = (size_t)((n + (1 << psh) - 1) >> psh) << psh;
  real* abq = a.abp + (size_t)b * a.G * npad + ((size_t)g << psh);
  real* const sbase = a.pt ? abq : abp;
  const int sh = a.pt ? psh : 31;
  const size_t gstride = (size_t)a.G << sh;
  const int smask = (int)((1u << sh) - 1u);
  static_assert(NT % 32 == 0, "a pass of rows is a whole number of row blocks");
  const size_t ustep = sh < 31 ? (size_t)(NT >> sh) * gstride : (size_t)NT;
  for (int r0 = 0; r0 < n; r0 += NT * KR) {
    if (r0 > 0) {
#pragma unroll
      for (int u = 0; u < KR; ++u) {
        const int r = r0 + u * NT + tid;
        f[u][0] = fw[r < n ? r : 0];
        if constexpr (SPW == 4) f[u][1] = fw1[r < n ? r : 0];
      }
    }
    real* const pbase = sbase + (size_t)((r0 + tid) >> sh) * gstride + ((r0 + tid) & smask);
    auto row = [&](int u, int r) {
      real t;
      if constexpr (SPW == 2) {
        const uint32_t e = f[u][0];
        const real v0 = ts[e & 0x7fffu];
        const real v1 = ts[M + ((e >> 16) & 0x7fffu)];
        t = (e & 0x8000u) ? -v0 : v0;
        t += (e & 0x80000000u) ? -v1 : v1;
      } else if constexpr (SPW == 4) {
        const uint32_t e = f[u][0], e1 = f[u][1];
        const real v0 = ts[e & 0x7fffu];
        const real v1 = ts[M + ((e >> 16) & 0x7fffu)];
        const real v2 = ts[2 * M + (e1 & 0x7fffu)];
        const real v3 = ts[3 * M + ((e1 >> 16) & 0x7fffu)];
        t = (e & 0x8000u) ? -v0 : v0;
        t += (e & 0x80000000u) ? -v1 : v1;
        real t1 = (e1 & 0x8000u) ? -v2 : v2;
        t1 += (e1 & 0x80000000u) ? -v3 : v3;
        t += t1;
      } else {
        const uint32_t e = f[u][0];
        const real v0 = ts[e & 0x1ffu];
        const real v1 = ts[M + ((e >> 10) & 0x1ffu)];
        const real v2 = ts[2 * M + ((e >> 20) & 0x1ffu)];
        t = (e & 0x200u) ? -v0 : v0;
        t += (e & 0x80000u) ? -v1 : v1;
        t += (e & 0x20000000u) ? -v2 : v2;
      }
      if constexpr (SPW == 3) st_part(pbase + u * ustep, t);
      else st_part(&sbase[(size_t)(r >> sh) * gstride + (r & smask)], t);
    };
    if (r0 + NT * KR <= n) {
#pragma unroll
      for (int u = 0; u < KR; ++u) row(u, r0 + u * NT + tid);
    } else if (SPW == 4 && r0 + NT * (KR - 1) <= n) {
#pragma unroll
      for (int u = 0; u < KR - 1; ++u) row(u, r0 + u * NT + tid);
      if (r0 + (KR - 1) * NT + tid < n) row(KR - 1, r0 + (KR - 1) * NT + tid);
    } else {
#pragma unroll
      for (int u = 0; u < KR; ++u) {
        const int r = r0 + u * NT + tid;
        if (r < n) row(u, r);
      }
    }
  }
#ifdef SA_STAMPS
  STAMP(8);
  asm volatile("s_waitcnt vmcnt(0)" ::: "memory");
  STAMP(9);
#endif
}

template <typename real, int E4>
__global__ void __launch_bounds__(512) k_sec4(SecArgs<real> a) { secq_body<real, E4, 4, 2>(a); }
template <typename real, int E4>
__global__ void __launch_bounds__(768) k_sec43(SecArgs<real> a) { secq_body<real, E4, 4, 3>(a); }
template <typename real, int E4>
__global__ void __launch_bounds__(1024) k_sec44(SecArgs<real> a) { secq_body<real, E4, 4, 4>(a); }

template <typename real, int E>
void launch_sec_e(sa_ctx* c, const Plan& p, int B, SecArgs<real> a) {
  a.RS = p.rs;
  dim3 grid(c->G * a.RS, B);
  if (c->prof) c->prof->begin(c->at().stream, K_SEC);
  if (c->big)
    plaunch(c, k_secg<real, E>, grid, 256, c->sec_lds, a);
  else
    plaunch(c, k_sec<real, E>, grid, 256, c->sec_lds, a);
  if (c->prof) c->prof->end(c->at().stream);
}

template <typename real>
int launch_sec2(sa_ctx* c, const Plan& p, int B, int t, int es, void* bin, void* bout, int bzero, int32_t* dec,
                int itset) {
  SecArgs<real> a = sec_args<real>(c, p, SEC_AMP, t, es);
  a.pt = p.pt;
  if (bzero && !p.bzero()) return fail(SA_ERR_UNSUPPORTED, "k_sec2 reads its previous estimate");
  if ((dec || itset) && (!p.bzero() || es || c->dead))
    return fail(SA_ERR_UNSUPPORTED, "launch_sec2: no fused decision on this path");
  a.bzero = bzero;
  a.dec = dec;
  a.itset = itset;
  a.beta = (real*)bin;
  a.beta_out = (real*)bout;
  a.G = p.G;
  dim3 grid(a.G, B);
  if (c->prof) c->prof->begin(c->at().stream, K_SEC);
  switch (p.sec) {
    case SA_SEC_K_SEC43:
      switch (c->M / 256) {
        case 1: plaunch(c, k_sec43<real, 1>, grid, 768, c->sec3_lds, a); break;
        case 2: plaunch(c, k_sec43<real, 2>, grid, 768, c->sec3_lds, a); break;
        default: return fail(SA_ERR_UNSUPPORTED, "k_sec43: M");
      }
      break;
    case SA_SEC_K_SEC44:
      switch (c->M / 256) {
        case 1: plaunch(c, k_sec44<real, 1>, grid, 1024, c->sec4q_lds, a); break;
        case 2: plaunch(c, k_sec44<real, 2>, grid, 1024, c->sec4q_lds, a); break;
        default: return fail(SA_ERR_UNSUPPORTED, "k_sec44: M");
      }
      break;
    case SA_SEC_K_SEC4:
      switch (c->M / 256) {
        case 1: plaunch(c, k_sec4<real, 1>, grid, 512, c->sec4_lds, a); break;
        case 2: plaunch(c, k_sec4<real, 2>, grid, 512, c->sec4_lds, a); break;
        case 4: plaunch(c, k_sec4<real, 4>, grid, 512, c->sec4_lds, a); break;
        case 8: plaunch(c, k_sec4<real, 8>, grid, 512, c->sec4_lds, a); break;
        case 16: plaunch(c, k_sec4<real, 16>, grid, 512, c->sec4_lds, a); break;
        default: return fail(SA_ERR_UNSUPPORTED, "k_sec4: M");
      }
      break;
    case SA_SEC_K_SEC2:
      switch (c->M / 128) {
        case 1: plaunch(c, k_sec2<real, 1>, grid, 256, c->sec2_lds, a); break;
        case 2: plaunch(c, k_sec2<real, 2>, grid, 256, c->sec2_lds, a); break;
        case 4: plaunch(c, k_sec2<real, 4>, grid, 256, c->sec2_lds, a); break;
        case 8: plaunch(c, k_sec2<real, 8>, grid, 256, c->sec2_lds, a); break;
        case 16: plaunch(c, k_sec2<real, 16>, grid, 256, c->sec2_lds, a); break;
        case 32: plaunch(c, k_sec2<real, 32>, grid, 256, c->sec2_lds, a); break;
        default: return fail(SA_ERR_UNSUPPORTED, "k_sec2: M");
      }
      break;
    default: return fail(SA_ERR_ARG, "launch_sec2: the plan runs no multi-wave section kernel");
  }
  if (c->prof) c->prof->end(c->at().stream);
  HIP_TRY(hipGetLastError());
  return SA_OK;
}

template <typename real>
int launch_sec(sa_ctx* c, const Plan& p, int B, int mode, int t, int es, void* bin, void* bout) {
  SecArgs<real> a = sec_args<real>(c, p, mode, t, es);
  if (bin) a.beta = (real*)bin;
  if (bout) a.beta_out = (real*)bout;
  switch (c->E) {
    case 1: launch_sec_e<real, 1>(c, p, B, a); break;
    case 2: launch_sec_e<real, 2>(c, p, B, a); break;
    case 4: launch_sec_e<real, 4>(c, p, B, a); break;
    case 8: launch_sec_e<real, 8>(c, p, B, a); break;
    case 16: launch_sec_e<real, 16>(c, p, B, a); break;
    case 32: launch_sec_e<real, 32>(c, p, B, a); break;
    case 64: launch_sec_e<real, 64>(c, p, B, a); break;
    default: return fail(SA_ERR_UNSUPPORTED, "bad E");
  }
  HIP_TRY(hipGetLastError());
  return SA_OK;
}

template int launch_sec<float>(sa_ctx*, const Plan&, int, int, int, int, void*, void*);
template int launch_sec<double>(sa_ctx*, const Plan&, int, int, int, int, void*, void*);
template int launch_sec2<float>(sa_ctx*, const Plan&, int, int, int, void*, void*, int, int32_t*, int);
template int launch_sec2<double>(sa_ctx*, const Plan&, int, int, int, void*, void*, int, int32_t*, int);

template <typename real>
static hipError_t sec_lds_attrs_t() {
  const int mx = 160 * 1024;
  hipError_t e = hipSuccess;
#define SA_A(F) if (e == hipSuccess) e = hipFuncSetAttribute((const void*)F, hipFuncAttributeMaxDynamicSharedMemorySize, mx);
  SA_A((k_sec<real, 1>)) SA_A((k_sec<real, 2>)) SA_A((k_sec<real, 4>)) SA_A((k_sec<real, 8>))
  SA_A((k_sec<real, 16>)) SA_A((k_sec<real, 32>)) SA_A((k_sec<real, 64>))
  SA_A((k_secg<real, 1>)) SA_A((k_secg<real, 2>)) SA_A((k_secg<real, 4>)) SA_A((k_secg<real, 8>))
  SA_A((k_secg<real, 16>)) SA_A((k_secg<real, 32>)) SA_A((k_secg<real, 64>))
  SA_A((k_sec2<real, 1>)) SA_A((k_sec2<real, 2>)) SA_A((k_sec2<real, 4>)) SA_A((k_sec2<real, 8>))
  SA_A((k_sec2<real, 16>)) SA_A((k_sec2<real, 32>))
  SA_A((k_sec4<real, 1>)) SA_A((k_sec4<real, 2>)) SA_A((k_sec4<real, 4>)) SA_A((k_sec4<real, 8>))
  SA_A((k_sec4<real, 16>))
  SA_A((k_sec43<real, 1>)) SA_A((k_sec43<real, 2>))
  SA_A((k_sec44<real, 1>)) SA_A((k_sec44<real, 2>))
#undef SA_A
  return e;
}

hipError_t sec_lds_attrs() {
  hipError_t e = sec_lds_attrs_t<float>();
  return e == hipSuccess ? sec_lds_attrs_t<double>() : e;
}

#ifdef SA_STAMPS
hipError_t stamps_add_sec(unsigned long long* out) {
  unsigned long long s[16 * 16];
  hipError_t e = hipMemcpyFromSymbol(s, HIP_SYMBOL(g_stamps), sizeof(s));
  for (int i = 0; i < 16 * 16; ++i) out[i] += s[i];
  return e;
}
#endif

}
```

### sparc_ldpc_amd/csrc/sparc_amp.hip

```cpp

#define SA_VERSION "sparc_amp 0.4 gfx950"

#include "sa_host.h"

namespace sa {

thread_local std::string g_err;

int fail(int code, const std::string& msg) {
  g_err = msg;
  return code;
}

template <typename src_t, typename dst_t>
__global__ void k_convert(const src_t* s, dst_t* d, size_t N) {
  for (size_t i = blockIdx.x * (size_t)blockDim.x + threadIdx.x; i < N;
       i += (size_t)gridDim.x * blockDim.x)
    d[i] = (dst_t)s[i];
}

__global__ void k_fill32(uint32_t* p, uint32_t v, size_t nw) {
  for (size_t i = blockIdx.x * (size_t)blockDim.x + threadIdx.x; i < nw; i += (size_t)gridDim.x * blockDim.x)
    p[i] = v;
}
// ... 30 lines not shown

void dev_free(void* p) {
  if (p) (void)hipFree(p);
}


int sync_all(sa_ctx* c) {
  for (auto& l : c->lane)
    if (l.stream) HIP_TRY(hipStreamSynchronize(l.stream));
  return SA_OK;
}

static int y_wait_reader(sa_ctx* c, int k, hipStream_t s) {
  sa_lane& o = c->lane[1 - k];
  if (c->lanes_on && o.y_read) {
    HIP_TRY(hipStreamWaitEvent(s, o.y_ev, 0));
    o.y_read = false;
  }
  return SA_OK;
}

int y_begin_write(sa_ctx* c, int k, hipStream_t s, int B) {
  if (c->lane[k].row_B) {
    sa_lane& l = c->lane[k];
    if (int rc = row_flush(c, k)) return rc;
    if (s != l.stream) {
      HIP_TRY(hipEventRecord(l.y_ev, l.stream));
      HIP_TRY(hipStreamWaitEvent(s, l.y_ev, 0));
    }
  }
  if (!c->lanes_on) return SA_OK;
  if (B < c->Bcap) {
    if (int rc = y_sync(c, k)) return rc;
    if (s != c->lane[k].stream) HIP_TRY(hipStreamWaitEvent(s, c->lane[k].y_ev, 0));
  }
  return y_wait_reader(c, k, s);
}

int y_mark(sa_ctx* c, int k) {
  sa_lane& l = c->lane[k];
  l.y_ver = ++c->y_ver;
  c->y_lane = k;
  if (l.y_ev) HIP_TRY(hipEventRecord(l.y_ev, l.stream));
  return SA_OK;
}

int y_sync(sa_ctx* c, int k) {
  sa_lane& l = c->lane[k];
  if (!c->lanes_on || l.y_ver == c->y_ver) return SA_OK;
  sa_lane& src = c->lane[c->y_lane];
  if (int rcf = row_flush(c, k)) return rcf;
  HIP_TRY(hipStreamWaitEvent(l.stream, src.y_ev, 0));
  if (int rc = y_wait_reader(c, k, l.stream)) return rc;
  HIP_TRY(hipMemcpyAsync(l.d_y, src.d_y, (size_t)c->Bcap * c->n * rsz(c), hipMemcpyDeviceToDevice, l.stream));
  HIP_TRY(hipEventRecord(l.y_ev, l.stream));
  l.y_ver = c->y_ver;
  l.y_read = true;
  return SA_OK;
}

static int lane_open(sa_lane& l) {
  if (!l.stream) HIP_TRY(hipStreamCreateWithFlags(&l.stream, hipStreamNonBlocking));
  if (!l.ev0) HIP_TRY(hipEventCreate(&l.ev0));
  if (!l.ev1) HIP_TRY(hipEventCreate(&l.ev1));
  if (!l.y_ev) HIP_TRY(hipEventCreateWithFlags(&l.y_ev, hipEventDisableTiming));
  return SA_OK;
}

static int beta2_alloc(sa_ctx* c, sa_lane& l, size_t nB) {
  int rc = dev_alloc(c, &l.d_beta2, nB * c->L * c->M * rsz(c));
  if (!rc) l.beta2_cap = (int)nB;
  return rc;
}

static int lane_alloc(sa_ctx* c, sa_lane& l, size_t nB, size_t nBp, int T, int Gmax, bool beta2) {
  const size_t s = rsz(c), LM = (size_t)c->L * c->M;
  int rc;
  if ((rc = dev_alloc(c, &l.d_y, nB * c->n * s))) return rc;
  if ((rc = dev_alloc(c, &l.d_z, nBp * c->n * s))) return rc;
  if ((rc = dev_alloc(c, &l.d_beta, nB * LM * s))) return rc;
  if ((rc = dev_alloc(c, &l.d_abp, nBp * Gmax * ((size_t)c->NZ16 * kRow2Rows) * s))) return rc;
  if ((rc = dev_alloc(c, &l.d_bbp, nB * Gmax * s))) return rc;
  if ((rc = dev_alloc(c, &l.d_zzp, nB * c->NZh * s))) return rc;
  if ((rc = dev_alloc(c, &l.d_tau, nB * (T + 1) * s))) return rc;
  if ((rc = dev_alloc(c, (void**)&l.d_iters, nB * sizeof(int)))) return rc;
  if (hipHostMalloc((void**)&l.h_dec, nB * c->L * sizeof(int32_t), hipHostMallocDefault) != hipSuccess ||
      hipHostGetDevicePointer((void**)&l.d_dec, l.h_dec, 0) != hipSuccess) {
    if (l.h_dec) (void)hipHostFree(l.h_dec);
    l.h_dec = l.d_dec = nullptr;
    return fail(SA_ERR_NOMEM, "hipHostMalloc(lane decisions) failed");
  }
  return beta2 ? beta2_alloc(c, l, nB) : SA_OK;
}

static void lane_free(sa_lane& l) {
  void** bufs[] = {&l.d_y, &l.d_z, &l.d_beta, &l.d_beta2, &l.d_abp, &l.d_bbp, &l.d_zzp, &l.d_tau, (void**)&l.d_iters};
  for (void** p : bufs) {
    dev_free(*p);
    *p = nullptr;
  }
  l.beta2_cap = 0;
  if (l.h_dec) (void)hipHostFree(l.h_dec);
  l.h_dec = l.d_dec = nullptr;
  l.fused_B = l.row_B = l.row_T = 0;
}

static void dec_rescue(sa_ctx* c, int k) {
  for (int s = 0; s < SA_DECIDE_SLOTS; ++s)
    if (c->dec_B[s] != 0 && c->dec_lane[s] == k && c->h_dec && c->lane[k].h_dec) {
      std::memcpy(c->h_dec + (size_t)s * c->dec_cap, c->lane[k].h_dec, (size_t)c->dec_B[s] * c->L * sizeof(int32_t));
      c->dec_lane[s] = -1;
    }
}

static int dec_spill(sa_ctx* c, int k) {
  sa_lane& l = c->lane[k];
  for (int s = 0; s < SA_DECIDE_SLOTS; ++s)
    if (c->dec_B[s] != 0 && c->dec_lane[s] == k) {
      const size_t N = (size_t)c->dec_B[s] * c->L;
      k_copy32<<<(int)std::min<size_t>((N + 255) / 256, 1024), 256, 0, l.stream>>>(l.d_dec, c->d_dec + (size_t)s * c->dec_cap, N);
      HIP_TRY(hipGetLastError());
      HIP_TRY(hipEventRecord(c->dec_ev[s], l.stream));
      c->dec_lane[s] = -1;
    }
  return SA_OK;
}

static void stage_free(sa_lane& l) {
  dev_free(l.d_stage);
  l.d_stage = nullptr;
  l.stage_cap = 0;
}

static int lane_create(sa_ctx* c) {
  sa_lane& l = c->lane[1];
  if (int rco = lane_open(l)) return rco;
  const int Gmax = std::max(c->G, std::max(c->G2, c->G3));
  if (int rc = lane_alloc(c, l, c->Bcap, c->Bcap, c->Tcap, Gmax, true)) return rc;
  if (int rc = ensure_stage(c, l, c->lane[0].stage_cap)) return rc;
  l.y_ver = 0;
  l.y_read = false;
  c->lanes_on = true;
  return SA_OK;
}

static bool pipelining(const sa_ctx* c) {
  for (int k = 0; k < SA_DECIDE_SLOTS; ++k)
    if (c->dec_B[k] != 0) return true;
  return c->at().ev1 && hipEventQuery(c->at().ev1) == hipErrorNotReady;
}

static bool lane_shape(const sa_ctx* c, int B) {
  return c->backend == SA_BACKEND_HADAMARD && !use_batched(c, B) && !(c->plan & (SA_PLAN_EAGER | SA_PLAN_NO_LANES));
}

void graphs_clear(GraphMap& m) {
  for (auto& kv : m) (void)hipGraphExecDestroy(kv.second);
  m.clear();
}

int lanes_release(sa_ctx* c) {
  int rc = sync_all(c);
  if (!c->lanes_on) return rc;
  if (!rc) dec_rescue(c, 1);
  lane_switch(c, 0);
  sa_lane &l0 = c->lane[0], &l = c->lane[1];
  if (!rc) rc = y_sync(c, 0);
  if (!rc && l0.stream && hipStreamSynchronize(l0.stream) != hipSuccess)
    rc = fail(SA_ERR_HIP, "lanes_release: sync failed");
  graphs_clear(l.graphs);
  lane_free(l);
  stage_free(l);
  l.y_read = false;
  l0.y_read = false;
  l0.y_ver = c->y_ver;
  c->y_lane = 0;
  c->lanes_on = false;
  return rc;
}

void drop_graphs(sa_ctx* c) {
  for (auto& l : c->lane) graphs_clear(l.graphs);
  graphs_clear(c->mc_graphs);
}

void free_workspace(sa_ctx* c) {
  lane_free(c->lane[0]);
// ... 41 lines not shown
  if ((rc = lane_alloc(c, c->lane[0], nB, nBp, nT, Gmax, false))) return rc;
  if ((rc = dev_alloc(c, &c->d_out, nB * (LM > (size_t)c->n ? LM : (size_t)c->n) * s))) return rc;
  if ((rc = dev_alloc(c, (void**)&c->d_stop, nB * sizeof(int)))) return rc;
  if ((rc = dev_alloc(c, (void**)&c->d_idx, nB * c->L * sizeof(int32_t)))) return rc;
  if ((rc = dev_alloc(c, &c->d_cb, nB * c->L * s))) return rc;
  if ((rc = dev_alloc(c, &c->d_Pb, nB * s))) return rc;
  if (is_dense(c))
    if ((rc = dev_alloc(c, &c->d_azp, nB * c->RS * c->lda * s))) return rc;
  if (c->backend == SA_BACKEND_HOST)
    if ((rc = dev_alloc(c, &c->d_azp, nB * c->lda * s))) return rc;
  c->Bcap = (int)nB;
  c->Tcap = nT;
  return SA_OK;
}

int ensure_stage(sa_ctx* c, sa_lane& l, size_t count) {
  if (count <= l.stage_cap) return SA_OK;
  HIP_TRY(hipStreamSynchronize(l.stream));
  stage_free(l);
  int rc = dev_alloc(c, (void**)&l.d_stage, count * sizeof(double));
  if (rc) return rc;
  l.stage_cap = count;
  return SA_OK;
}

int upload(sa_ctx* c, sa_lane& l, void* dst, const double* src, size_t count) {
  if (c->prec == SA_PREC_F64) {
    HIP_TRY(hipMemcpyAsync(dst, src, count * 8, hipMemcpyHostToDevice, l.stream));
    return SA_OK;
  }
  int rc = ensure_stage(c, l, count);
  if (rc) return rc;
  HIP_TRY(hipMemcpyAsync(l.d_stage, src, count * 8, hipMemcpyHostToDevice, l.stream));
  const int blocks = (int)((count + 255) / 256 < 4096 ? (count + 255) / 256 : 4096);
  k_convert<double, float><<<blocks > 0 ? blocks : 1, 256, 0, l.stream>>>(l.d_stage, (float*)dst, count);
  HIP_TRY(hipGetLastError());
  return SA_OK;
}

int download(sa_ctx* c, sa_lane& l, double* dst, const void* src, size_t count) {
  if (c->prec == SA_PREC_F64) {
    HIP_TRY(hipMemcpyAsync(dst, src, count * 8, hipMemcpyDeviceToHost, l.stream));
    return SA_OK;
  }
  int rc = ensure_stage(c, l, count);
  if (rc) return rc;
  const int blocks = (int)((count + 255) / 256 < 4096 ? (count + 255) / 256 : 4096);
  k_convert<float, double><<<blocks > 0 ? blocks : 1, 256, 0, l.stream>>>((const float*)src, l.d_stage, count);
  HIP_TRY(hipGetLastError());
  HIP_TRY(hipMemcpyAsync(dst, l.d_stage, count * 8, hipMemcpyDeviceToHost, l.stream));
  return SA_OK;
}




template <typename real>
int seq_ab(sa_ctx* c, int B) {
  const Plan p = plan_for(c, B);
  if (p.dense()) return dense_ab<real>(c, p, B);
  if (int rc = launch_sec<real>(c, p, B, SEC_AB, 0, 0)) return rc;
  return launch_row<real>(c, p, B, ROW_ABOUT, 0, 0, c->G, c->G);
}

template <typename real>
int seq_az(sa_ctx* c, int B) {
  const Plan p = plan_for(c, B);
  if (p.dense()) return dense_az<real>(c, p, B);
  return launch_sec<real>(c, p, B, SEC_AZ, 0, 0);
}

template <typename real>
int seq_amp(sa_ctx* c, int B, int T, int flags, int has_b0) {
  const int es = (flags & SA_FLAG_NO_EARLY_STOP) ? 0 : 1;
  sa_lane& ln = c->at();
  const Plan p = plan_for(c, B);
  const bool dense = p.dense(), batched = p.batched();
  c->zil_last = p.zil;
  int rc;
  const bool it_row = p.it_row() && T > 0;
  const bool bzero = !has_b0 && p.bzero() && T > 0;
  const int flip = (bzero && !es) ? (T & 1) : 0;
  const bool ft = fused_tail(c, p, T, flags);
  if (!it_row) k_fill32<<<(B + 255) / 256, 256, 0, ln.stream>>>((uint32_t*)ln.d_iters, 0xffffffffu, (size_t)B);
  if (has_b0) {
    if (dense) {
      if ((rc = dense_start<real>(c, p, B))) return rc;
    } else {
      if ((rc = launch_sec<real>(c, p, B, SEC_AB, 0, 0))) return rc;
      if ((rc = launch_row<real>(c, p, B, ROW_INIT, 0, 0, c->G, c->G, it_row ? -1 : 0))) return rc;
    }
  } else {
    if (!bzero) {
      const size_t nw = (size_t)B * c->L * c->M * rsz(c) / 4;
      k_fill32<<<(int)std::min<size_t>((nw + 255) / 256, 8192), 256, 0, ln.stream>>>((uint32_t*)ln.d_beta, 0u, nw);
    }
    if ((rc = launch_row<real>(c, p, B, ROW_INIT0, 0, 0, p.G, p.Gb, it_row ? -1 : 0))) return rc;
  }
  for (int t = 0; t < T; ++t) {
    if (dense) {
      if ((rc = dense_iter<real>(c, p, B, t, es))) return rc;
    } else if (batched) {
      if ((rc = launch_secb<real>(c, p, B, t, es))) return rc;
    } else {
      void* pin = ((t ^ flip) & 1) ? ln.d_beta2 : ln.d_beta;
      void* pout = ((t ^ flip) & 1) ? ln.d_beta : ln.d_beta2;
      if (p.multiwave()) {
        const bool tail = ft && t == T - 1;
        if ((rc = launch_sec2<real>(c, p, B, t, es, pin, pout, bzero && t == 0, tail ? ln.d_dec : nullptr, tail ? T : 0)))
          return rc;
      } else if ((rc = launch_sec<real>(c, p, B, SEC_AMP, t, es, pin, pout))) {
        return rc;
      }
    }
    if (ft && t == T - 1) break;
    if ((rc = launch_row<real>(c, p, B, ROW_AMP, t, es, p.G, p.Gb, it_row && t == T - 1 ? T : 0))) return rc;
  }
  if (!it_row) k_iters_final<<<(B + 255) / 256, 256, 0, ln.stream>>>(ln.d_iters, B, T);
  HIP_TRY(hipGetLastError());
  const bool home = !es && (((T - 1) ^ flip) & 1);
  if (!dense && !batched && T > 0 && !home) {
    const size_t LM = (size_t)c->L * c->M;
    k_beta_final<real><<<dim3((unsigned)std::min<size_t>((LM + 255) / 256, 4096), B), 256, 0, ln.stream>>>(
        (real*)ln.d_beta, (const real*)ln.d_beta2, ln.d_iters, LM);
    HIP_TRY(hipGetLastError());
  }
  return SA_OK;
}

int row_flush(sa_ctx* c, int k) {
  sa_lane& l = c->lane[k];
  if (!l.row_B) return SA_OK;
  const int B = l.row_B, T = l.row_T, keep = c->cur;
  l.row_B = l.row_T = 0;
  const Plan p = plan_for(c, B);
  lane_switch(c, k);
  const int rc = c->prec == SA_PREC_F64 ? launch_row<double>(c, p, B, ROW_AMP, T - 1, 0, p.G, p.Gb, 0)
                                        : launch_row<float>(c, p, B, ROW_AMP, T - 1, 0, p.G, p.Gb, 0);
  lane_switch(c, keep);
  return rc;
}

static void tail_mark(sa_ctx* c, int B, int T, int flags) {
  sa_lane& ln = c->at();
  const bool ft = fused_tail(c, plan_for(c, B), T, flags);
  ln.fused_B = ft ? B : 0;
  ln.row_B = ft ? B : 0;
  ln.row_T = ft ? T : 0;
}

int ensure_beta2(sa_ctx* c, int B) {
  if (is_dense(c) || use_batched(c, B) || c->at().beta2_cap >= c->Bcap) return SA_OK;
  if (int rcl = lanes_release(c)) return rcl;
  if (int rc = beta2_alloc(c, c->lane[0], c->Bcap)) return rc;
  drop_graphs(c);
  return SA_OK;
}

int ensure_invb(sa_ctx* c);

template <typename real>
int run_graph(sa_ctx* c, int B, int T, int flags, int has_b0) {
  int rc0 = ensure_beta2(c, B);
  if (!rc0 && use_batched(c, B)) rc0 = ensure_invb(c);
  if (rc0) return rc0;
  if (lane_shape(c, B) && !c->prof && !has_b0 && pipelining(c)) {
    if (!c->lanes_on)
      if (int rcl = lane_create(c)) return rcl;
    lane_switch(c, 1 - c->cur);
  } else if (use_batched(c, B)) {
    lane_switch(c, 0);
  }
  {
    sa_lane& l = c->at();
    l.row_B = l.row_T = 0;
    if (int rcd = dec_spill(c, c->cur)) return rcd;
    l.fused_B = 0;
  }
  if (int rcy = y_sync(c)) return rcy;
  sa_lane& ln = c->at();
  if (c->plan & SA_PLAN_EAGER) {
    HIP_TRY(hipEventRecord(ln.ev0, ln.stream));
    int rc = seq_amp<real>(c, B, T, flags, has_b0);
    if (rc) return rc;
    HIP_TRY(hipEventRecord(ln.ev1, ln.stream));
    tail_mark(c, B, T, flags);
    c->last_B = B;
    c->last_T = T;
    c->zil_last = zil_for(c, B);
    return SA_OK;
  }
  const auto key = std::make_tuple(B, T, flags | (c->pb_on ? 0x10000 : 0), has_b0);
  auto it = ln.graphs.find(key);
  if (it == ln.graphs.end()) {
    hipGraphExec_t ex = nullptr;
    if (int rc = capture_graph(ln.stream, [&] { return seq_amp<real>(c, B, T, flags, has_b0); }, &ex)) return rc;
    it = ln.graphs.emplace(key, ex).first;
  }
  HIP_TRY(hipEventRecord(ln.ev0, ln.stream));
  HIP_TRY(hipGraphLaunch(it->second, ln.stream));
  HIP_TRY(hipEventRecord(ln.ev1, ln.stream));
  tail_mark(c, B, T, flags);
  c->last_B = B;
  c->last_T = T;
  c->zil_last = zil_for(c, B);
  return SA_OK;
}

int check_ctx(const sa_ctx* c) {
  if (!c) return fail(SA_ERR_ARG, "null context");
  return SA_OK;
}

int check_tables(const sa_ctx* c, const char* what) {
  if (!c) return fail(SA_ERR_ARG, "null context");
  if (c->backend != SA_BACKEND_HADAMARD && c->backend != SA_BACKEND_DENSE)
    return fail(SA_ERR_UNSUPPORTED, std::string(what) + ": needs a design built from an ordering "
                                                        "(use sa_Ab for a caller's matrix)");
  return SA_OK;
}

int check_op(const sa_ctx* c, const char* what) {
  if (!c) return fail(SA_ERR_ARG, "null context");
  if (c->backend == SA_BACKEND_HOST)
    return fail(SA_ERR_UNSUPPORTED, std::string(what) + ": a host-operator context has no device operator");
  return SA_OK;
}

int upload_sections(sa_ctx* c, void* dst, const double* src, int B) {
  const size_t LM = (size_t)c->L * c->M;
  if (c->dead == 0) return upload(c, dst, src, (size_t)B * LM);
  std::vector<double> pad((size_t)B * LM, 0.0);
  for (size_t bl = 0; bl < (size_t)B * c->L; ++bl)
    std::memcpy(pad.data() + bl * c->M + c->dead, src + bl * c->Mu, (size_t)c->Mu * sizeof(double));
  int rc = upload(c, dst, pad.data(), pad.size());
  if (rc) return rc;
  HIP_TRY(hipStreamSynchronize(c->at().stream));
  return SA_OK;
}

int download_sections(sa_ctx* c, double* dst, const void* src, int B) {
  const size_t LM = (size_t)c->L * c->M;
  if (c->dead == 0) return download(c, dst, src, (size_t)B * LM);
  std::vector<double> pad((size_t)B * LM);
  int rc = download(c, pad.data(), src, pad.size());
  if (rc) return rc;
  HIP_TRY(hipStreamSynchronize(c->at().stream));
  for (size_t bl = 0; bl < (size_t)B * c->L; ++bl)
    std::memcpy(dst + bl * c->Mu, pad.data() + bl * c->M + c->dead, (size_t)c->Mu * sizeof(double));
  return SA_OK;
}

int set_power(sa_ctx* c, const double* Pl) {
  if (!Pl) return fail(SA_ERR_ARG, "Pl is NULL");
  std::vector<double> cl(c->L);
  double P = 0;
  for (int l = 0; l < c->L; ++l) {
    if (!(Pl[l] >= 0)) return fail(SA_ERR_ARG, "Pl must be non-negative");
    cl[l] = std::sqrt((double)c->n * Pl[l]);
    P += Pl[l];
  }
  for (int k = 0; k < sa_ctx::kLanes; ++k)
    if (int rcf = row_flush(c, k)) return rcf;
  const bool same = c->h_Pl.size() == (size_t)c->L && std::memcmp(c->h_Pl.data(), Pl, (size_t)c->L * 8) == 0;
  if (same) {
    c->pb_on = false;
    c->shared_power = true;
    c->power_set = true;
    return SA_OK;
  }
  if (int rcs = sync_all(c)) return rcs;
  c->h_Pl.clear();
  c->P = P;
  c->cmax = 0;
  for (int l = 0; l < c->L; ++l) c->cmax = cl[l] > c->cmax ? cl[l] : c->cmax;
  int rc = upload(c, c->d_c, cl.data(), c->L);
  if (!rc) rc = upload(c, c->d_P1, &P, 1);
  if (rc) return rc;
  HIP_TRY(hipMemcpyAsync(c->d_cd, cl.data(), (size_t)c->L * 8, hipMemcpyHostToDevice, c->at().stream));
  HIP_TRY(hipStreamSynchronize(c->at().stream));
  c->pb_on = false;
  c->shared_power = true;
  c->power_set = true;
  if (c->d_bfix && (rc = i8_set_bfix(c))) return rc;
  c->h_Pl.assign(Pl, Pl + c->L);
// ... 655 lines not shown
    dev_free(c->d_fwd3);
  }
  dev_free(c->d_A);
  dev_free(c->d_AT); dev_free(c->d_xz); dev_free(c->d_xb);
  dev_free(c->d_A8); dev_free(c->d_AT8); dev_free(c->d_zq); dev_free(c->d_bq);
  dev_free(c->d_zsc); dev_free(c->d_bsc0); dev_free(c->d_bfix);
  dev_free(c->d_c);
  dev_free(c->d_cd);
  dev_free(c->d_P1);
  for (auto& e : c->dec_ev)
    if (e) (void)hipEventDestroy(e);
  if (c->h_dec) (void)hipHostFree(c->h_dec);
  for (auto& l : c->lane) {
    stage_free(l);
    if (l.y_ev) (void)hipEventDestroy(l.y_ev);
    if (l.ev0) (void)hipEventDestroy(l.ev0);
    if (l.ev1) (void)hipEventDestroy(l.ev1);
    if (l.stream) (void)hipStreamDestroy(l.stream);
  }
  delete c;
}

int sa_Ab(sa_ctx* c, int B, const double* beta, double* out) {
  if (int rc0 = check_op(c, "sa_Ab")) return rc0;
  if (B <= 0 || !beta || !out) return fail(SA_ERR_ARG, "sa_Ab: bad arguments");
  HIP_TRY(hipSetDevice(c->device));
  int rc = ensure_workspace(c, B, c->Tcap > 0 ? c->Tcap : 1);
  if (rc) return rc;
  if ((rc = tail_settle(c))) return rc;
  if ((rc = upload_sections(c, c->at().d_beta, beta, B))) return rc;
  rc = c->prec == SA_PREC_F64 ? seq_ab<double>(c, B) : seq_ab<float>(c, B);
  if (rc) return rc;
  if ((rc = download(c, out, c->d_out, (size_t)B * c->n))) return rc;
  HIP_TRY(hipStreamSynchronize(c->at().stream));
  return SA_OK;
}

int sa_Az(sa_ctx* c, int B, const double* z, double* out) {
  if (int rc0 = check_op(c, "sa_Az")) return rc0;
  if (B <= 0 || !z || !out) return fail(SA_ERR_ARG, "sa_Az: bad arguments");
  HIP_TRY(hipSetDevice(c->device));
  int rc = ensure_workspace(c, B, c->Tcap > 0 ? c->Tcap : 1);
  if (rc) return rc;
  if ((rc = row_flush(c, c->cur))) return rc;
  if ((rc = upload(c, c->at().d_z, z, (size_t)B * c->n))) return rc;
  c->zil_last = false;
  if (c->prec == SA_PREC_F64) {
    rc = seq_az<double>(c, B);
  } else {
    rc = seq_az<float>(c, B);
  }
  if (rc) return rc;
  if ((rc = download_sections(c, out, c->d_out, B))) return rc;
  HIP_TRY(hipStreamSynchronize(c->at().stream));
  return SA_OK;
}

int sa_reserve(sa_ctx* c, int B, int T) {
  if (check_ctx(c)) return SA_ERR_ARG;
  if (B <= 0 || T < 0) return fail(SA_ERR_ARG, "sa_reserve: bad arguments");
  HIP_TRY(hipSetDevice(c->device));
  int rc = ensure_workspace(c, B, T > 0 ? T : 1);
  if (!rc && c->backend == SA_BACKEND_HADAMARD && use_batched(c, B)) rc = ensure_invb(c);
  return rc;
}

int sa_stage(sa_ctx* c, int B, const double* y, const double* Pl, const double* beta0) {
  if (check_ctx(c)) return SA_ERR_ARG;
  if (B <= 0) return fail(SA_ERR_ARG, "sa_stage: bad arguments");
  HIP_TRY(hipSetDevice(c->device));
  int rc = ensure_workspace(c, B, c->Tcap > 0 ? c->Tcap : 1);
  if (rc) return rc;
  if (Pl && (rc = set_power(c, Pl))) return rc;
  if (y) {
    const bool rotate = c->lanes_on && !beta0 && lane_shape(c, B) && pipelining(c);
    const int k = rotate ? 1 - c->cur : c->cur;
    sa_lane& l = c->lane[k];
    rc = y_begin_write(c, k, l.stream, B);
    if (!rc) rc = upload(c, l, l.d_y, y, (size_t)B * c->n);
    if (!rc) rc = y_mark(c, k);
    if (rc) return rc;
  }
  if (beta0) {
    c->at().fused_B = 0;
    if ((rc = upload_sections(c, c->at().d_beta, beta0, B))) return rc;
  }
  return SA_OK;
}

int sa_stage_power_batch(sa_ctx* c, int B, const double* Pl) {
  if (check_ctx(c)) return SA_ERR_ARG;
  if (B <= 0) return fail(SA_ERR_ARG, "sa_stage_power_batch: bad arguments");
  HIP_TRY(hipSetDevice(c->device));
  int rc = ensure_workspace(c, B, c->Tcap > 0 ? c->Tcap : 1);
  if (rc) return rc;
  return set_power_batch(c, B, Pl);
}

int sa_run(sa_ctx* c, int B, int T, int flags) {
  if (int rc0 = check_op(c, "sa_run")) return rc0;
  if (B <= 0 || T < 0) return fail(SA_ERR_ARG, "sa_run: bad arguments");
  if (!c->power_set) return fail(SA_ERR_ARG, "sa_run: power allocation not staged");
  if (B > c->Bcap) return fail(SA_ERR_ARG, "sa_run: batch larger than the staged batch");
  HIP_TRY(hipSetDevice(c->device));
  if (T > c->Tcap) {
    return fail(SA_ERR_ARG, "sa_run: T larger than the workspace (call sa_reserve first)");
  }
  const int has_b0 = (flags & SA_FLAG_BETA0) ? 1 : 0;
  return c->prec == SA_PREC_F64 ? run_graph<double>(c, B, T, flags & 0xff, has_b0)
                                : run_graph<float>(c, B, T, flags & 0xff, has_b0);
}

int sa_wait(sa_ctx* c) {
  if (check_ctx(c)) return SA_ERR_ARG;
  HIP_TRY(hipSetDevice(c->device));
  return sync_all(c);
}

double sa_run_event_ms(sa_ctx* c) {
  if (!c) return -1.0;
  float ms = -1.f;
  if (hipEventElapsedTime(&ms, c->at().ev0, c->at().ev1) != hipSuccess) return -1.0;
  return ms;
}

int sa_fetch_z(sa_ctx* c, int B, double* z_out) {
  if (check_ctx(c) || !z_out) return fail(SA_ERR_ARG, "sa_fetch_z: bad arguments");
  if (B <= 0 || B > c->Bcap) return fail(SA_ERR_ARG, "sa_fetch_z: bad batch");
  HIP_TRY(hipSetDevice(c->device));
  int rc;
  if ((rc = row_flush(c, c->cur))) return rc;
  if (c->zil_last) {
    const int CB = 16 / (int)rsz(c), NC = (B + CB - 1) / CB;
    std::vector<double> il((size_t)NC * CB * c->n);
    if ((rc = download(c, il.data(), c->at().d_z, il.size()))) return rc;
    HIP_TRY(hipStreamSynchronize(c->at().stream));
    for (int b = 0; b < B; ++b)
      for (int r = 0; r < c->n; ++r) z_out[(size_t)b * c->n + r] = il[((size_t)(b / CB) * c->n + r) * CB + b % CB];
    return SA_OK;
  }
  if ((rc = download(c, z_out, c->at().d_z, (size_t)B * c->n))) return rc;
  HIP_TRY(hipStreamSynchronize(c->at().stream));
  return SA_OK;
}

int sa_fetch_y(sa_ctx* c, int B, double* y_out) {
  if (check_ctx(c) || !y_out) return fail(SA_ERR_ARG, "sa_fetch_y: bad arguments");
  if (B <= 0 || B > c->Bcap) return fail(SA_ERR_ARG, "sa_fetch_y: bad batch");
  HIP_TRY(hipSetDevice(c->device));
  int rc;
  if ((rc = y_sync(c))) return rc;
  if ((rc = download(c, y_out, c->at().d_y, (size_t)B * c->n))) return rc;
  HIP_TRY(hipStreamSynchronize(c->at().stream));
  return SA_OK;
}

int sa_fetch(sa_ctx* c, int B, double* beta_out, int* iters_out) {
  if (check_ctx(c)) return SA_ERR_ARG;
  if (B <= 0 || B > c->Bcap) return fail(SA_ERR_ARG, "sa_fetch: bad batch");
  HIP_TRY(hipSetDevice(c->device));
  int rc;
  if (beta_out && (rc = download_sections(c, beta_out, c->at().d_beta, B))) return rc;
  const sa_lane& ln = c->at();
  if (iters_out) HIP_TRY(hipMemcpyAsync(iters_out, ln.d_iters, (size_t)B * sizeof(int), hipMemcpyDeviceToHost, ln.stream));
  HIP_TRY(hipStreamSynchronize(ln.stream));
  return SA_OK;
}

int sa_amp(sa_ctx* c, int B, const double* y, const double* Pl, int T, const double* beta0, double* beta_out,
           int* iters_out, int flags) {
  if (int rc0 = check_op(c, "sa_amp")) return rc0;
  if (B <= 0 || T < 0 || !y || !Pl || !beta_out) return fail(SA_ERR_ARG, "sa_amp: bad arguments");
  HIP_TRY(hipSetDevice(c->device));
  int rc = ensure_workspace(c, B, T > 0 ? T : 1);
  if (rc) return rc;
  if ((rc = sa_stage(c, B, y, Pl, beta0))) return rc;
  if (T == 0) {
    c->at().fused_B = 0;
    if (!beta0) HIP_TRY(hipMemsetAsync(c->at().d_beta, 0, (size_t)B * c->L * c->M * rsz(c), c->at().stream));
    HIP_TRY(hipMemsetAsync(c->at().d_iters, 0, (size_t)B * sizeof(int), c->at().stream));
  } else {
    if ((rc = sa_run(c, B, T, (flags & 0xff) | (beta0 ? SA_FLAG_BETA0 : 0)))) return rc;
  }
  return sa_fetch(c, B, beta_out, iters_out);
}

int sa_profile(sa_ctx* c, int B, int T, int flags, double* out) { return sa_profile_rep(c, B, T, flags, 1, out); }

int sa_profile_kinds(void) { return K_NKINDS; }

extern "C++" {
namespace {
int profile_impl(sa_ctx* c, int B, int T, int flags, int rep, bool dispatch, double* out) {
  if (int rc0 = check_op(c, "sa_profile")) return rc0;
  if (B <= 0 || T <= 0 || !out || B > c->Bcap || T > c->Tcap || !c->power_set || rep < 1 || rep > 1024)
    return fail(SA_ERR_ARG, "sa_profile: bad arguments (reserve and stage first)");
  HIP_TRY(hipSetDevice(c->device));
  if (int rcs = sync_all(c)) return rcs;
  if (int rcb = ensure_beta2(c, B)) return rcb;
  if (use_batched(c, B)) lane_switch(c, 0);
  c->at().row_B = c->at().row_T = 0;
  c->at().fused_B = 0;
  if (int rcy = y_sync(c)) return rcy;
  if (use_batched(c, B))
    if (int rci = ensure_invb(c)) return rci;
  Prof prof;
  prof.rep = rep;
  prof.dispatch = dispatch;
  c->prof = &prof;
  hipEvent_t e0 = nullptr, e1 = nullptr;
  HIP_TRY(hipEventCreate(&e0));
  HIP_TRY(hipEventCreate(&e1));
  HIP_TRY(hipEventRecord(e0, c->at().stream));
  const int has_b0 = (flags & SA_FLAG_BETA0) ? 1 : 0;
  int rc = c->prec == SA_PREC_F64 ? seq_amp<double>(c, B, T, flags & 0xff, has_b0)
                                  : seq_amp<float>(c, B, T, flags & 0xff, has_b0);
  c->prof = nullptr;
  (void)hipEventRecord(e1, c->at().stream);
  hipError_t e = hipStreamSynchronize(c->at().stream);
  if (rc == SA_OK && e != hipSuccess) rc = fail(SA_ERR_HIP, std::string("sa_profile: ") + hipGetErrorString(e));
  double sum[K_NKINDS] = {0}, cnt[K_NKINDS] = {0};
  if (rc == SA_OK) {
    for (auto& ev : prof.ev) {
      float ms = 0.f;
      if (hipEventElapsedTime(&ms, std::get<1>(ev), std::get<2>(ev)) == hipSuccess) {
        sum[std::get<0>(ev)] += ms / rep;
        cnt[std::get<0>(ev)] += 1;
      }
    }
    float tot = 0.f;
    (void)hipEventElapsedTime(&tot, e0, e1);
    for (int k = 0; k < K_NKINDS; ++k) {
      out[2 * k] = cnt[k] > 0 ? sum[k] / cnt[k] : 0.0;
      out[2 * k + 1] = cnt[k];
    }
    out[2 * K_NKINDS] = tot;
  }
  (void)hipEventDestroy(e0);
  (void)hipEventDestroy(e1);
  return rc;
}
}
}

int sa_profile_rep(sa_ctx* c, int B, int T, int flags, int rep, double* out) {
  return profile_impl(c, B, T, flags, rep, false, out);
}

int sa_profile_dispatch(sa_ctx* c, int B, int T, int flags, double* out) {
  return profile_impl(c, B, T, flags, 1, true, out);
}


int sa_decide(sa_ctx* c, int B, int32_t* idx_out) {
  if (check_ctx(c)) return SA_ERR_ARG;
  if (B <= 0 || B > c->Bcap || !idx_out) return fail(SA_ERR_ARG, "sa_decide: bad arguments");
  HIP_TRY(hipSetDevice(c->device));
  if (c->at().fused_B >= B) {
    HIP_TRY(hipStreamSynchronize(c->at().stream));
    std::memcpy(idx_out, c->at().h_dec, (size_t)B * c->L * sizeof(int32_t));
    return SA_OK;
  }
  if (int rc = launch_decide(c, B, c->d_idx)) return rc;
  HIP_TRY(hipMemcpyAsync(idx_out, c->d_idx, (size_t)B * c->L * sizeof(int32_t), hipMemcpyDeviceToHost, c->at().stream));
  HIP_TRY(hipStreamSynchronize(c->at().stream));
  return SA_OK;
}

int sa_decide_async(sa_ctx* c, int B, int slot) {
  if (check_ctx(c)) return SA_ERR_ARG;
  if (B <= 0 || B > c->Bcap || slot < 0 || slot >= SA_DECIDE_SLOTS)
    return fail(SA_ERR_ARG, "sa_decide_async: bad arguments");
  HIP_TRY(hipSetDevice(c->device));
  const size_t per = (size_t)c->Bcap * c->L;
  if (!c->h_dec || c->dec_cap < per) {
    for (int k = 0; k < SA_DECIDE_SLOTS; ++k)
      if (c->h_dec && c->dec_B[k] != 0)
        return fail(SA_ERR_ARG, "sa_decide_async: the staged batch grew while slot " + std::to_string(k) +
                                    " holds decisions not yet collected (sa_decide_collect them first)");
    if (int rcs = sync_all(c)) return rcs;
    if (c->h_dec) (void)hipHostFree(c->h_dec);
    c->h_dec = nullptr;
    c->d_dec = nullptr;
    c->dec_cap = 0;
    HIP_TRY(hipHostMalloc((void**)&c->h_dec, per * SA_DECIDE_SLOTS * sizeof(int32_t), hipHostMallocDefault));
    HIP_TRY(hipHostGetDevicePointer((void**)&c->d_dec, c->h_dec, 0));
    c->dec_cap = per;
    for (int k = 0; k < SA_DECIDE_SLOTS; ++k) {
      if (!c->dec_ev[k]) HIP_TRY(hipEventCreateWithFlags(&c->dec_ev[k], hipEventDisableTiming));
      c->dec_B[k] = 0;
      c->dec_lane[k] = -1;
    }
  }
  if (c->at().fused_B >= B) {
    c->dec_lane[slot] = c->cur;
    c->dec_B[slot] = B;
    return SA_OK;
  }
  c->dec_lane[slot] = -1;
  if (int rc = launch_decide(c, B, c->d_dec + (size_t)slot * c->dec_cap)) return rc;
  HIP_TRY(hipEventRecord(c->dec_ev[slot], c->at().stream));
  c->dec_B[slot] = B;
  return SA_OK;
}

int sa_decide_collect(sa_ctx* c, int B, int slot, int32_t* idx_out) {
  if (check_ctx(c)) return SA_ERR_ARG;
  if (slot < 0 || slot >= SA_DECIDE_SLOTS || !idx_out || !c->h_dec || c->dec_B[slot] != B || B <= 0)
    return fail(SA_ERR_ARG, "sa_decide_collect: no decision of this batch queued in the slot");
  HIP_TRY(hipSetDevice(c->device));
  if (const int k = c->dec_lane[slot]; k >= 0) {
    HIP_TRY(hipEventSynchronize(c->lane[k].ev1));
    std::memcpy(idx_out, c->lane[k].h_dec, (size_t)B * c->L * sizeof(int32_t));
    c->dec_B[slot] = 0;
    c->dec_lane[slot] = -1;
    return SA_OK;
  }
  HIP_TRY(hipEventSynchronize(c->dec_ev[slot]));
  std::memcpy(idx_out, c->h_dec + (size_t)slot * c->dec_cap, (size_t)B * c->L * sizeof(int32_t));
  c->dec_B[slot] = 0;
  return SA_OK;
}


int sa_plan(sa_ctx* c, int B, int64_t* o) {
  if (check_ctx(c) || !o || B <= 0) return fail(SA_ERR_ARG, "sa_plan: bad arguments");
  const Plan p = plan_for(c, B);
  o[0] = p.sec;
  o[1] = p.G;
  o[2] = (p.sec == SA_SEC_K_SEC || p.sec == SA_SEC_K_SECG) ? p.rs : 1;
  o[3] = p.CB;
  o[4] = p.nz;
  o[5] = c->w;
  o[6] = p.row;
  o[7] = c->n_cus;
  return SA_OK;
}

int sa_plan_batched(sa_ctx* c, int B, int64_t* o) {
  if (check_ctx(c) || !o || B <= 0) return fail(SA_ERR_ARG, "sa_plan_batched: bad arguments");
  if (is_dense(c) || !use_batched(c, B)) return fail(SA_ERR_ARG, "sa_plan_batched: this batch does not run k_secb");
  const int NC = (B + c->CB - 1) / c->CB;
  const bool xcd = (c->Gb % 8) == 0 && ((long long)c->Gb * NC) % 8 == 0;
  const int gx = xcd ? c->Gb / 8 : c->Gb;
  const int gp = xcd ? std::min(c->gpx, gx) : gx;
  o[0] = c->Gb;
  o[1] = c->WB;
  o[2] = gp;
  o[3] = (gx + gp - 1) / gp;
  return SA_OK;
}

int sa_info(const sa_ctx* c, int64_t* o) {
  if (check_ctx(c) || !o) return fail(SA_ERR_ARG, "sa_info: bad arguments");
  o[0] = c->L; o[1] = c->Mu; o[2] = c->n; o[3] = c->w; o[4] = c->backend; o[5] = c->prec;
  o[6] = c->device; o[7] = (int64_t)c->bytes;
  return SA_OK;
}

int sa_device_count(void) {
  int n = 0;
  if (hipGetDeviceCount(&n) != hipSuccess) return 0;
  return n;
}

const char* sa_last_error(void) { return g_err.c_str(); }

const char* sa_version(void) { return SA_VERSION; }

#ifdef SA_STAMPS
int sa_debug_stamps(unsigned long long* out) {
  HIP_TRY(hipDeviceSynchronize());
  std::memset(out, 0, sizeof(unsigned long long) * 16 * 16);
  HIP_TRY(stamps_add_sec(out));
  HIP_TRY(stamps_add_secb(out));
  return SA_OK;
}
#endif

}
```

### sparc_ldpc_amd/operators.py

```python
from __future__ import annotations

import hashlib
import os
from collections import OrderedDict

import numpy as np

from . import _lib
from ._lib import as_f64, check, dptr

__all__ = [
    "SparcOperator", "AbOp", "AzOp", "HostOperatorLoop", "make_ordering", "sub_fht", "block_sub_fht",
    "sparc_transforms", "sparc_transforms_shorter", "dense_transforms", "gaussian_transforms", "default_device",
]

_BACKENDS = {"hadamard": _lib.SA_BACKEND_HADAMARD, "dense": _lib.SA_BACKEND_DENSE}
_PRECS = {"fp32": _lib.SA_PREC_F32, "fp64": _lib.SA_PREC_F64}

DEFAULT_BACKEND = os.environ.get("SPARC_AMP_BACKEND", "hadamard")
DEFAULT_PRECISION = os.environ.get("SPARC_AMP_PRECISION", "fp32")


def default_device() -> int:
    lib = _lib.load()
# ... 166 lines not shown
            assert beta0.size == B * self.L * self.M, "β₀ must hold L*M values per codeword"
            b0p = dptr(beta0)
        out = np.empty((B, self.L * self.M))
        iters = np.empty(B, dtype=np.int32)
        flags = 0 if early_stop else _lib.SA_FLAG_NO_EARLY_STOP
        check(self._lib.sa_amp(self._ctx, B, dptr(y), dptr(Pl), T, b0p, dptr(out),
                               iters.ctypes.data_as(_lib.ct.POINTER(_lib.ct.c_int)), flags))
        return out, iters

    def decide(self, B: int) -> np.ndarray:
        idx = np.empty((B, self.L), dtype=np.int32)
        check(self._lib.sa_decide(self._ctx, B, idx.ctypes.data_as(_lib.ct.POINTER(_lib.ct.c_int32))))
        return idx

    DECIDE_SLOTS = 4

    def decide_async(self, B: int, slot: int) -> None:
        check(self._lib.sa_decide_async(self._ctx, int(B), int(slot)))

    def decide_collect(self, B: int, slot: int) -> np.ndarray:
        idx = np.empty((B, self.L), dtype=np.int32)
        check(self._lib.sa_decide_collect(self._ctx, int(B), int(slot),
                                          idx.ctypes.data_as(_lib.ct.POINTER(_lib.ct.c_int32))))
        return idx

    def reserve(self, B, T):
        check(self._lib.sa_reserve(self._ctx, int(B), int(T)))

    def stage(self, y, Pl=None, beta0=None):
        y = as_f64(y)
        B = y.shape[0] if y.ndim == 2 else 1
        Pl = None if Pl is None else as_f64(Pl)
        beta0 = None if beta0 is None else as_f64(beta0)
        check(self._lib.sa_stage(self._ctx, B, dptr(y), None if Pl is None else dptr(Pl),
                                 None if beta0 is None else dptr(beta0)))
        return B

    def run(self, B, T, early_stop=True, beta0=False):
        flags = (0 if early_stop else _lib.SA_FLAG_NO_EARLY_STOP) | (_lib.SA_FLAG_BETA0 if beta0 else 0)
        check(self._lib.sa_run(self._ctx, int(B), int(T), flags))

    def wait(self):
        check(self._lib.sa_wait(self._ctx))

    def last_run_ms(self) -> float:
        return float(self._lib.sa_run_event_ms(self._ctx))

    KERNEL_KINDS = ("k_sec", "k_row", "k_dense_az", "k_dense_den", "k_dense_ab", "k_i8_quant")

    def profile(self, B, T, early_stop=True, beta0=False, rep=1):
        flags = (0 if early_stop else _lib.SA_FLAG_NO_EARLY_STOP) | (_lib.SA_FLAG_BETA0 if beta0 else 0)
        nk = len(self.KERNEL_KINDS)
        if int(self._lib.sa_profile_kinds()) != nk:
            raise _lib.SparcAmpError(_lib.SA_ERR_UNSUPPORTED, f"libsparc_amp profiles {self._lib.sa_profile_kinds()} kernel kinds, "
                                f"this module knows {nk}: rebuild the library")
        out = np.zeros(2 * nk + 1)
        if rep == 0:
            check(self._lib.sa_profile_dispatch(self._ctx, int(B), int(T), flags, dptr(out)))
        else:
            check(self._lib.sa_profile_rep(self._ctx, int(B), int(T), flags, int(rep), dptr(out)))
        kinds = {k: (float(out[2 * i]), int(out[2 * i + 1])) for i, k in enumerate(self.KERNEL_KINDS)}
        return kinds, float(out[2 * nk])

    def fetch(self, B):
        out = np.empty((B, self.L * self.M))
        iters = np.empty(B, dtype=np.int32)
        check(self._lib.sa_fetch(self._ctx, B, dptr(out), iters.ctypes.data_as(_lib.ct.POINTER(_lib.ct.c_int))))
        return out, iters

    def iters(self, B):
        it = np.empty(B, dtype=np.int32)
        check(self._lib.sa_fetch(self._ctx, B, None, it.ctypes.data_as(_lib.ct.POINTER(_lib.ct.c_int))))
        return it

    SECTION_KERNELS = ("k_sec", "k_sec2", "k_secb", "dense", "k_sec4", "k_sec43", "dense_mfma", "matrix_mfma",
                       "k_secg", "k_sec44")
    ROW_KERNELS = ("k_row", "k_row2", "k_rowv16B", "k_rowv8B", "k_row2_16", "k_rowc")

    def fetch_z(self, B):
        z = np.empty((B, self.n))
        check(self._lib.sa_fetch_z(self._ctx, int(B), z.ctypes.data_as(_lib.ct.POINTER(_lib.ct.c_double))))
        return z

    def fetch_y(self, B):
        y = np.empty((B, self.n))
        check(self._lib.sa_fetch_y(self._ctx, int(B), dptr(y)))
        return y

    def plan(self, B):
        o = np.zeros(8, dtype=np.int64)
        check(self._lib.sa_plan(self._ctx, int(B), o.ctypes.data_as(_lib.ct.POINTER(_lib.ct.c_int64))))
        return dict(section_kernel=self.SECTION_KERNELS[int(o[0])], partials=int(o[1]), row_splits=int(o[2]),
                    codewords_per_wg=int(o[3]), zz_partials=int(o[4]), w=int(o[5]),
                    row_kernel=self.ROW_KERNELS[int(o[6])], cus=int(o[7]))

    def mc_supported(self, B):
        if self.backend != "hadamard" or not 4 <= int(B) <= 1024:
            return False
        p = self.plan(B)
        return p["section_kernel"] == "k_secb" and p["row_kernel"] == "k_rowc"

    def mc_stage(self, idx, noise):
        idx = np.ascontiguousarray(idx, dtype=np.int32)
        R = idx.shape[0]
        assert idx.shape == (R, self.L), "idx must be (R, L)"
        noise = as_f64(noise)
        assert noise.size == R * self.n, "noise must be (R, n)"
        check(self._lib.sa_mc_stage(self._ctx, R, idx.ctypes.data_as(_lib.ct.POINTER(_lib.ct.c_int32)), dptr(noise)))
        self._mc_reps = R
        return R

    def mc_draw(self, seeds, sigma):
        seeds = seed_array(seeds)
        R = len(seeds)
        sig = np.ascontiguousarray(np.broadcast_to(np.asarray(sigma, dtype=np.float64), (R,)))
        ms = np.zeros(1)
        self._mc_reps = 0
        check(self._lib.sa_mc_draw(self._ctx, R, seeds.ctypes.data_as(_lib.ct.POINTER(_lib.ct.c_uint32)), dptr(sig),
                                   dptr(ms)))
        self._mc_reps = R
        return float(ms[0])

    def mc_fetch_draws(self):
        R = int(getattr(self, "_mc_reps", 0))
        idx = np.empty((R, self.L), dtype=np.int32)
        noise = np.empty((R, self.n))
        check(self._lib.sa_mc_fetch_draws(self._ctx, R, idx.ctypes.data_as(_lib.ct.POINTER(_lib.ct.c_int32)),
                                          dptr(noise)))
        return idx, noise

    def mc_run(self, B, T, early_stop=True, decisions=True):
        R = int(getattr(self, "_mc_reps", 0))
        i32 = _lib.ct.POINTER(_lib.ct.c_int32)
        dec = np.empty((R, self.L), dtype=np.int32) if decisions else None
        its = np.empty(R, dtype=np.int32)
        errs = np.empty(R, dtype=np.int32)
        ms = np.zeros(1)
        flags = 0 if early_stop else _lib.SA_FLAG_NO_EARLY_STOP
        check(self._lib.sa_mc_run(self._ctx, int(B), int(T), flags, None if dec is None else dec.ctypes.data_as(i32),
                                  its.ctypes.data_as(i32), errs.ctypes.data_as(i32), dptr(ms)))
        return dec, its, errs, float(ms[0])

    def plan_batched(self, B):
        o = np.zeros(4, dtype=np.int64)
        check(self._lib.sa_plan_batched(self._ctx, int(B), o.ctypes.data_as(_lib.ct.POINTER(_lib.ct.c_int64))))
        return dict(groups=int(o[0]), sections_per_wg=int(o[1]), groups_per_pass=int(o[2]), passes=int(o[3]))

    def info(self):
        o = np.zeros(8, dtype=np.int64)
        check(self._lib.sa_info(self._ctx, o.ctypes.data_as(_lib.ct.POINTER(_lib.ct.c_int64))))
        keys = ("L", "M", "n", "w", "backend", "precision", "device", "device_bytes")
        return dict(zip(keys, (int(v) for v in o)))

    @staticmethod
    def _ptr(x):
        if isinstance(x, int):
            return _lib.ct.c_void_p(x), _lib.SA_PTR_DEVICE
        return _lib.ct.c_void_p(x.ctypes.data), 0

    def stage_power(self, B, Pl):
        Pl = as_f64(Pl).reshape(-1)
        assert Pl.size == self.L, "Pl must hold L section powers"
        check(self._lib.sa_stage(self._ctx, int(B), None, dptr(Pl), None))

    def stage_power_batch(self, B, Pl):
        Pl = as_f64(Pl)
        assert Pl.shape == (B, self.L), "Pl must be (B, L)"
        check(self._lib.sa_stage_power_batch(self._ctx, int(B), dptr(Pl)))

    def encode(self, idx, noise=None):
        idx = np.ascontiguousarray(idx, dtype=np.int32)
        B = idx.shape[0]
        assert idx.shape == (B, self.L)
        nz = None
        if noise is not None:
            noise = as_f64(noise)
            assert noise.size == B * self.n
# ... 255 lines not shown
```

Baseline: 2373 codewords/s.

## Add short-chain AMP schedule that skips init row launch and defers tail work

Adds a 'short chain' decode schedule for fused-tail runs with no beta0. The initial ROW_INIT0 launch is dropped: the first section pass reads y plus cached |y|^2 partials (refreshed only when y changes), and the first row pass takes y as its z input. The final section kernel runs only the estimate part; the row part is deferred to a flush that runs only if beta is later needed. This removes a kernel launch and some tail work per decode in exchange for more split-mode code paths and state tracking that must stay consistent.

```diff
diff --git a/include/sparc_amp.h b/include/sparc_amp.h
--- a/include/sparc_amp.h
+++ b/include/sparc_amp.h
@@ -55,7 +55,8 @@
   SA_PLAN_SEC4Q = 1 << 13,
   SA_PLAN_NO_SEC4Q = 1 << 14,
   SA_PLAN_NO_FUSED_TAIL = 1 << 15,
-  SA_PLAN_ALL = (1 << 16) - 1
+  SA_PLAN_NO_SHORT_CHAIN = 1 << 16,
+  SA_PLAN_ALL = (1 << 17) - 1
 };
 int sa_create_ex(sa_ctx** out, int L, int M, int n, const uint32_t* ordering,
                  int backend, int precision, int device, int plan);
@@ -87,6 +88,7 @@
 int sa_fetch(sa_ctx* ctx, int B, double* beta_out, int* iters_out);
 int sa_fetch_z(sa_ctx* ctx, int B, double* z_out);
 int sa_fetch_y(sa_ctx* ctx, int B, double* y_out);
+int sa_fetch_tau(sa_ctx* ctx, int B, int T, double* tau_out);
 double sa_run_event_ms(sa_ctx* ctx);
 
 int sa_profile(sa_ctx* ctx, int B, int T, int flags, double* out);
@@ -166,6 +168,7 @@
   SA_ROW_K_ROWC = 5
 } sa_row_kernel;
 int sa_plan(sa_ctx* ctx, int B, int64_t* out8);
+int sa_plan_run(sa_ctx* ctx, int B, int T, int flags, int64_t* out4);
 int sa_plan_batched(sa_ctx* ctx, int B, int64_t* out4);
 int sa_info(const sa_ctx* ctx, int64_t* out8);
 int sa_device_count(void);
diff --git a/sparc_ldpc_amd/_lib.py b/sparc_ldpc_amd/_lib.py
--- a/sparc_ldpc_amd/_lib.py
+++ b/sparc_ldpc_amd/_lib.py
@@ -32,7 +32,7 @@
     "SEC3": 1 << 0, "NO_SEC3": 1 << 1, "ROW16": 1 << 2, "NO_ROW16": 1 << 3, "NO_PT": 1 << 4,
     "ZIL": 1 << 5, "NO_ZIL": 1 << 6, "WB8": 1 << 7, "WB16": 1 << 8, "NO_BANKS": 1 << 9, "EAGER": 1 << 10,
     "ONE_PASS": 1 << 11, "NO_LANES": 1 << 12, "SEC4Q": 1 << 13, "NO_SEC4Q": 1 << 14,
-    "NO_FUSED_TAIL": 1 << 15,
+    "NO_FUSED_TAIL": 1 << 15, "NO_SHORT_CHAIN": 1 << 16,
 }
 
 
@@ -53,11 +53,11 @@
 
 EXPORTS = (
     "sa_create", "sa_create_ex", "sa_create_matrix", "sa_create_matrix_random", "sa_subset", "sa_create_twin", "sa_destroy", "sa_Ab", "sa_Az", "sa_amp",
-    "sa_reserve", "sa_stage", "sa_stage_power_batch", "sa_run", "sa_wait", "sa_fetch", "sa_fetch_z", "sa_fetch_y", "sa_run_event_ms",
+    "sa_reserve", "sa_stage", "sa_stage_power_batch", "sa_run", "sa_wait", "sa_fetch", "sa_fetch_z", "sa_fetch_y", "sa_fetch_tau", "sa_run_event_ms",
     "sa_profile", "sa_profile_rep", "sa_profile_dispatch", "sa_profile_kinds", "sa_decide",
     "sa_decide_async", "sa_decide_collect", "sa_info", "sa_device_count", "sa_last_error", "sa_version",
     "sa_encode", "sa_stage_onehot", "sa_llr", "sa_llr_ex", "sa_soft_beta0", "sa_hard_cancel",
-    "sa_threshold", "sa_cancel", "sa_plan", "sa_plan_batched", "sa_stage_onehot_scaled", "sa_cancel_scaled",
+    "sa_threshold", "sa_cancel", "sa_plan", "sa_plan_run", "sa_plan_batched", "sa_stage_onehot_scaled", "sa_cancel_scaled",
     "sa_host_init", "sa_host_tau", "sa_host_eta", "sa_host_residual",
     "sa_draw_reps", "sa_mc_stage", "sa_mc_run", "sa_make_ordering", "sa_mc_draw", "sa_mc_fetch_draws",
     "sa_se", "sa_se_draws",
@@ -85,6 +85,7 @@
     "sa_fetch": (_I, [_P, _I, _D, ct.POINTER(ct.c_int)]),
     "sa_fetch_z": (_I, [_P, _I, _D]),
     "sa_fetch_y": (_I, [_P, _I, _D]),
+    "sa_fetch_tau": (_I, [_P, _I, _I, _D]),
     "sa_run_event_ms": (ct.c_double, [_P]),
     "sa_profile": (_I, [_P, _I, _I, _I, _D]),
     "sa_profile_rep": (_I, [_P, _I, _I, _I, _I, _D]),
@@ -101,6 +102,7 @@
     "sa_threshold": (_I, [_P, _I, _I, _I, _P, _I, ct.c_double, ct.POINTER(ct.c_int32)]),
     "sa_cancel": (_I, [_P, _I, ct.POINTER(ct.c_int32), _P]),
     "sa_plan": (_I, [_P, _I, ct.POINTER(ct.c_int64)]),
+    "sa_plan_run": (_I, [_P, _I, _I, _I, ct.POINTER(ct.c_int64)]),
     "sa_plan_batched": (_I, [_P, _I, ct.POINTER(ct.c_int64)]),
     "sa_stage_onehot": (_I, [_P, _I, ct.POINTER(ct.c_int32)]),
     "sa_stage_onehot_scaled": (_I, [_P, _I, ct.POINTER(ct.c_int32), ct.c_double]),
diff --git a/sparc_ldpc_amd/csrc/sa_common.h b/sparc_ldpc_amd/csrc/sa_common.h
--- a/sparc_ldpc_amd/csrc/sa_common.h
+++ b/sparc_ldpc_amd/csrc/sa_common.h
@@ -765,6 +765,7 @@
   int32_t* dec;
   int itset;
 };
+enum { SEC_PART_ALL = SEC_AMP, SEC_PART_EST = 3, SEC_PART_ROWS = 4 };
 
 template <typename real>
 struct RowArgs {
diff --git a/sparc_ldpc_amd/csrc/sa_glue.hip b/sparc_ldpc_amd/csrc/sa_glue.hip
--- a/sparc_ldpc_amd/csrc/sa_glue.hip
+++ b/sparc_ldpc_amd/csrc/sa_glue.hip
@@ -271,7 +271,7 @@
       return fail(SA_ERR_ARG, "sa_stage_onehot: index outside [0, M)");
   HIP_TRY(hipSetDevice(c->device));
   sa_lane& ln = c->at();
-  ln.fused_B = 0;
+  if (int rc = beta_settle(c)) return rc;
   HIP_TRY(hipMemcpyAsync(c->d_idx, idx, (size_t)B * c->L * sizeof(int32_t), hipMemcpyHostToDevice, ln.stream));
   const size_t tot = (size_t)B * c->L * c->M;
   if (c->prec == SA_PREC_F64)
@@ -337,7 +337,7 @@
   if (!app) return fail(SA_ERR_ARG, "sa_soft_beta0: app is NULL");
   HIP_TRY(hipSetDevice(c->device));
   sa_lane& ln = c->at();
-  ln.fused_B = 0;
+  if ((rc = beta_settle(c))) return rc;
   const int lgM = ilog2(c->M);
   const size_t na = (size_t)B * ns * lgM;
   const double* d_app = app;
diff --git a/sparc_ldpc_amd/csrc/sa_host.h b/sparc_ldpc_amd/csrc/sa_host.h
--- a/sparc_ldpc_amd/csrc/sa_host.h
+++ b/sparc_ldpc_amd/csrc/sa_host.h
@@ -53,6 +53,10 @@
   int32_t *h_dec = nullptr, *d_dec = nullptr;
   int fused_B = 0;
   int row_B = 0, row_T = 0;
+  bool row_short = false;
+  void* d_yyp = nullptr;
+  unsigned long long yy_ver = 0;
+  int yy_B = 0, yy_nz = 0;
 };
 
 struct sa_ctx {
@@ -266,6 +270,25 @@
          !(c->plan & SA_PLAN_NO_FUSED_TAIL);
 }
 
+inline bool short_chain(const sa_ctx* c, const Plan& p, int T, int flags, int has_b0) {
+  return fused_tail(c, p, T, flags) && !has_b0 && !(c->plan & SA_PLAN_NO_SHORT_CHAIN);
+}
+
+inline int decode_launches(const sa_ctx* c, const Plan& p, int T, int flags, int has_b0) {
+  if (p.dense()) return -1;
+  const bool es = !(flags & SA_FLAG_NO_EARLY_STOP);
+  const bool it_row = p.it_row() && T > 0, bzero = !has_b0 && p.bzero() && T > 0;
+  const bool ft = fused_tail(c, p, T, flags), sc = short_chain(c, p, T, flags, has_b0);
+  int k = it_row ? 0 : 2;
+  k += has_b0 ? 2 : (bzero ? 0 : 1);
+  k += (has_b0 || sc) ? 0 : 1;
+  k += 2 * T - (ft ? 1 : 0);
+  const int flip = (bzero && !es) ? (T & 1) : 0;
+  const bool home = !es && (((T - 1) ^ flip) & 1);
+  if (!p.batched() && T > 0 && !home) k += 1;
+  return k;
+}
+
 template <typename real>
 SecArgs<real> sec_args(sa_ctx* c, const Plan& p, int mode, int t, int early_stop, const int* tb = nullptr) {
   SecArgs<real> a;
@@ -344,6 +367,10 @@
   c->at().fused_B = 0;
   return row_flush(c, c->cur);
 }
+inline int beta_settle(sa_ctx* c) {
+  c->at().fused_B = 0;
+  return c->at().row_short ? row_flush(c, c->cur) : SA_OK;
+}
 int y_sync(sa_ctx* c, int k);
 int y_begin_write(sa_ctx* c, int k, hipStream_t s, int B);
 int y_mark(sa_ctx* c, int k);
@@ -367,7 +394,9 @@
 int launch_sec(sa_ctx* c, const Plan& p, int B, int mode, int t, int es, void* bin = nullptr, void* bout = nullptr);
 template <typename real>
 int launch_sec2(sa_ctx* c, const Plan& p, int B, int t, int es, void* bin, void* bout, int bzero = 0,
-                int32_t* dec = nullptr, int itset = 0);
+                int32_t* dec = nullptr, int itset = 0,
+                int part = SEC_PART_ALL,
+                const void* z = nullptr, const void* zzp = nullptr);
 hipError_t sec_lds_attrs();
 
 template <typename real>
@@ -377,7 +406,8 @@
 
 template <typename real>
 int launch_row(sa_ctx* c, const Plan& p, int B, int mode, int t, int es, int G, int Gb, int itset = 0,
-               const int* tb = nullptr);
+               const int* tb = nullptr,
+               const void* z_in = nullptr, void* zzp = nullptr);
 int launch_decide(sa_ctx* c, int B, int32_t* idx);
 
 int dense_den_groups(const sa_ctx* c);
diff --git a/sparc_ldpc_amd/csrc/sa_mc.hip b/sparc_ldpc_amd/csrc/sa_mc.hip
--- a/sparc_ldpc_amd/csrc/sa_mc.hip
+++ b/sparc_ldpc_amd/csrc/sa_mc.hip
@@ -508,6 +508,8 @@
   if ((rc = mc_ensure_slots(c, B))) return rc;
   sa_lane& ln = c->at();
   ln.row_B = ln.row_T = 0;
+  ln.row_short = false;
+  ln.yy_B = 0;
   ln.fused_B = 0;
   if (!c->h_mc_live) {
     HIP_TRY(hipHostMalloc((void**)&c->h_mc_live, 4 * sizeof(int), hipHostMallocDefault));
diff --git a/sparc_ldpc_amd/csrc/sa_row.hip b/sparc_ldpc_amd/csrc/sa_row.hip
--- a/sparc_ldpc_amd/csrc/sa_row.hip
+++ b/sparc_ldpc_amd/csrc/sa_row.hip
@@ -402,8 +402,12 @@
 }
 
 template <typename real>
-int launch_row(sa_ctx* c, const Plan& p, int B, int mode, int t, int es, int G, int Gb, int itset, const int* tb) {
+int launch_row(sa_ctx* c, const Plan& p, int B, int mode, int t, int es, int G, int Gb, int itset, const int* tb,
+               const void* z_in, void* zzp) {
   RowArgs<real> a = row_args<real>(c, p, mode, t, es, G, Gb, tb);
+  if ((z_in || zzp) && !p.row_sets_iters()) return fail(SA_ERR_UNSUPPORTED, "launch_row: only k_row2 takes z_in / zzp");
+  if (z_in) a.z_in = (const real*)z_in;
+  if (zzp) a.zzp = (real*)zzp;
   a.pt = mode == ROW_AMP ? p.pt : 0;
   if (itset && !p.row_sets_iters()) return fail(SA_ERR_UNSUPPORTED, "launch_row: only k_row2 writes iters");
   a.itset = itset;
@@ -455,7 +459,7 @@
   return SA_OK;
 }
 
-template int launch_row<float>(sa_ctx*, const Plan&, int, int, int, int, int, int, int, const int*);
-template int launch_row<double>(sa_ctx*, const Plan&, int, int, int, int, int, int, int, const int*);
-
-}
+template int launch_row<float>(sa_ctx*, const Plan&, int, int, int, int, int, int, int, const int*, const void*, void*);
+template int launch_row<double>(sa_ctx*, const Plan&, int, int, int, int, int, int, int, const int*, const void*, void*);
+
+}
diff --git a/sparc_ldpc_amd/csrc/sa_sec.hip b/sparc_ldpc_amd/csrc/sa_sec.hip
--- a/sparc_ldpc_amd/csrc/sa_sec.hip
+++ b/sparc_ldpc_amd/csrc/sa_sec.hip
@@ -504,9 +504,10 @@
   return x[0];
 }
 
-template <typename real, int EQ, int QW, int SPW = 2>
+template <typename real, int EQ, int QW, int SPW = 2, bool SPLIT = false>
 __device__ __forceinline__ void secq_body(const SecArgs<real>& a) {
   static_assert(SPW == 2 || SPW == 3 || SPW == 4, "sections per workgroup");
+  const int part = SPLIT ? a.mode : (int)SEC_PART_ALL;
   STAMP(0);
   extern __shared__ __attribute__((aligned(16))) unsigned char smem[];
   constexpr int NT = SPW * QW * 64;
@@ -540,157 +541,185 @@
   const uint32_t* fw1 = a.fwd2 + (size_t)(2 * g + 1 < (a.L + 1) / 2 ? 2 * g + 1 : 2 * g) * n;
   ushort4 tb[KH][NQ];
   uint32_t f[KR][FW];
-
-  const real* zb = a.z + (size_t)b * n;
-  ZStage<real, NT> zst;
-  const real* zzb = a.zzp + (size_t)b * a.NZ;
-  ZZParts<real, 5> zz;
-  const bool dma = stage_z_dma<real, NT>(zb, zs, n, tid);
-  if (!dma) zst.issue(zb, n, tid);
-  zz.issue(zzb, a.NZ, lane);
-  const real last = a.t > 0 ? ld_vmem(a.tau + (size_t)b * a.T1 + a.t - 1) : (real)0;
-  load_buckets_off<EQ, KH>(ibase, ioff, 0, a.nhi, M, lane, tb);
-  load_section<real, EQ>(bl, bprev, lane, Mq);
-  const real cl = ld_vmem(a.c + (size_t)b * a.cst + lc);
-  const real tau = zz.tau(zzb, a.NZ, n);
-  if (a.bzero) {
-#pragma unroll
-    for (int i = 0; i < EQ; ++i) bprev[i] = 0;
-  }
-  const bool stop = a.early_stop && (tau == last);
-  if (g == 0 && tid == 0) {
-    a.tau[(size_t)b * a.T1 + a.t] = tau;
-    if (stop && a.iters[b] < 0) a.iters[b] = a.t;
-    if (a.itset != 0 && !stop) a.iters[b] = a.itset;
-  }
-  if (stop) {
-    if (dma) asm volatile("s_waitcnt vmcnt(0)" ::: "memory");
-    if (a.bzero && have) {
-      store_section<real, EQ>(a.beta + (size_t)b * LM + (size_t)lc * M + eoff, bprev, lane, Mq);
-    }
-    return;
-  }
-  const real tau2 = tau * tau;
-  const real inv_sn = (real)1 / a.sqrt_n;
-  const real kk = cl / tau2;
-  STAMP(1);
-  if (!dma) zst.store(zs, zb, n, tid);
-  else finish_z_dma<real>(zb, zs, n, tid);
-  __syncthreads();
-  STAMP(2);
-#ifdef SA_STAMPS
-  asm volatile("s_waitcnt vmcnt(0)" ::: "memory");
-  STAMP(10);
-#endif
-#pragma unroll
-  for (int i = 0; i < EQ; ++i) v[i] = 0;
-  for (int h0 = 0; h0 < a.nhi; h0 += KH) {
-    ushort4 tn[KH][NQ];
-    const bool more = h0 + KH < a.nhi;
-    if (more) load_buckets_off<EQ, KH>(ibase, ioff, h0 + KH, a.nhi, M, lane, tn);
-    gather_buckets<real, EQ, KH>(zs, h0, a.nhi, tb, v);
-    if (more) {
-#pragma unroll
-      for (int hh = 0; hh < KH; ++hh)
-#pragma unroll
-        for (int j = 0; j < NQ; ++j) tb[hh][j] = tn[hh][j];
-    }
-  }
   real* xs = xb + sidx * M;
-#pragma unroll
-  for (int u = 0; u < KR; ++u) {
-    const int r = u * NT + tid;
-    f[u][0] = ld_off(fw, (unsigned)(r < n ? r : 0) * 4u);
-    if constexpr (SPW == 4) f[u][1] = ld_off(fw1, (unsigned)(r < n ? r : 0) * 4u);
-  }
-  STAMP(3);
-  fwht_wave<real, EQ>(v, lane, 64);
-  topq_stage<real, EQ, QW>(v, xs, lane, q);
-  STAMP(4);
-
-
-  real mx = neg_inf<real>();
-#pragma unroll
-  for (int i = 0; i < EQ; ++i) {
-    v[i] = fma(v[i], inv_sn, bprev[i]) * kk;
-    mx = v[i] > mx ? v[i] : mx;
-  }
-  mx = wave_max(mx);
-  if (lane == 0) red[wv * 4] = mx;
-  __syncthreads();
-  const int w0 = wv & ~(QW - 1);
-  mx = combine_q<real, QW, true>(red, w0, 0);
-  real S = 0, S2 = 0;
-#pragma unroll
-  for (int i = 0; i < EQ; ++i) {
-    v[i] = dexp<real>(v[i] - mx);
-    S += v[i];
-    S2 += v[i] * v[i];
-  }
-  wave_sum2(S, S2);
-  if (lane == 0) {
-    red[wv * 4 + 1] = S;
-    red[wv * 4 + 2] = S2;
-  }
-  __syncthreads();
-  S = combine_q<real, QW, false>(red, w0, 1);
-  S2 = combine_q<real, QW, false>(red, w0, 2);
-  const real scale = cl * rcp_fast(S);
-#pragma unroll
-  for (int i = 0; i < EQ; ++i) v[i] = have ? v[i] * scale : (real)0;
-  if (have) store_section<real, EQ>(blo, v, lane, Mq);
-  const real bb = have ? S2 * scale * scale : (real)0;
+  real bb = 0;
   real dbest = neg_inf<real>();
   int dbi = M;
-  if (a.dec) {
+
+  if (part == SEC_PART_ROWS) {
+#pragma unroll
+    for (int u = 0; u < KR; ++u) {
+      const int r = u * NT + tid;
+      f[u][0] = ld_off(fw, (unsigned)(r < n ? r : 0) * 4u);
+      if constexpr (SPW == 4) f[u][1] = ld_off(fw1, (unsigned)(r < n ? r : 0) * 4u);
+    }
+    load_section<real, EQ>(blo, v, lane, Mq);
+    if (!have) {
+#pragma unroll
+      for (int i = 0; i < EQ; ++i) v[i] = 0;
+    }
+  } else {
+    const real* zb = a.z + (size_t)b * n;
+    ZStage<real, NT> zst;
+    const real* zzb = a.zzp + (size_t)b * a.NZ;
+    ZZParts<real, 5> zz;
+    const bool dma = stage_z_dma<real, NT>(zb, zs, n, tid);
+    if (!dma) zst.issue(zb, n, tid);
+    zz.issue(zzb, a.NZ, lane);
+    const real last = a.t > 0 ? ld_vmem(a.tau + (size_t)b * a.T1 + a.t - 1) : (real)0;
+    load_buckets_off<EQ, KH>(ibase, ioff, 0, a.nhi, M, lane, tb);
+    load_section<real, EQ>(bl, bprev, lane, Mq);
+    const real cl = ld_vmem(a.c + (size_t)b * a.cst + lc);
+    const real tau = zz.tau(zzb, a.NZ, n);
+    if (a.bzero) {
+#pragma unroll
+      for (int i = 0; i < EQ; ++i) bprev[i] = 0;
+    }
+    const bool stop = a.early_stop && (tau == last);
+    if (g == 0 && tid == 0) {
+      a.tau[(size_t)b * a.T1 + a.t] = tau;
+      if (stop && a.iters[b] < 0) a.iters[b] = a.t;
+      if (a.itset != 0 && !stop) a.iters[b] = a.itset;
+    }
+    if (stop) {
+      if (dma) asm volatile("s_waitcnt vmcnt(0)" ::: "memory");
+      if (a.bzero && have) {
+        store_section<real, EQ>(a.beta + (size_t)b * LM + (size_t)lc * M + eoff, bprev, lane, Mq);
+      }
+      return;
+    }
+    const real tau2 = tau * tau;
+    const real inv_sn = (real)1 / a.sqrt_n;
+    const real kk = cl / tau2;
+    STAMP(1);
+    if (!dma) zst.store(zs, zb, n, tid);
+    else finish_z_dma<real>(zb, zs, n, tid);
+    __syncthreads();
+    STAMP(2);
+#ifdef SA_STAMPS
+    asm volatile("s_waitcnt vmcnt(0)" ::: "memory");
+    STAMP(10);
+#endif
+#pragma unroll
+    for (int i = 0; i < EQ; ++i) v[i] = 0;
+    for (int h0 = 0; h0 < a.nhi; h0 += KH) {
+      ushort4 tn[KH][NQ];
+      const bool more = h0 + KH < a.nhi;
+      if (more) load_buckets_off<EQ, KH>(ibase, ioff, h0 + KH, a.nhi, M, lane, tn);
+      gather_buckets<real, EQ, KH>(zs, h0, a.nhi, tb, v);
+      if (more) {
+#pragma unroll
+        for (int hh = 0; hh < KH; ++hh)
+#pragma unroll
+          for (int j = 0; j < NQ; ++j) tb[hh][j] = tn[hh][j];
+      }
+    }
+    if (part != SEC_PART_EST) {
+#pragma unroll
+      for (int u = 0; u < KR; ++u) {
+        const int r = u * NT + tid;
+        f[u][0] = ld_off(fw, (unsigned)(r < n ? r : 0) * 4u);
+        if constexpr (SPW == 4) f[u][1] = ld_off(fw1, (unsigned)(r < n ? r : 0) * 4u);
+      }
+    }
+    STAMP(3);
+    fwht_wave<real, EQ>(v, lane, 64);
+    topq_stage<real, EQ, QW>(v, xs, lane, q);
+    STAMP(4);
+
+
+    real mx = neg_inf<real>();
 #pragma unroll
     for (int i = 0; i < EQ; ++i) {
-      const int e = eoff + elem_index<EQ>(lane, i);
-      if (v[i] > dbest || (v[i] == dbest && e < dbi)) { dbest = v[i]; dbi = e; }
-    }
-#pragma unroll
-    for (int m = 32; m >= 1; m >>= 1) {
-      const real ob = __shfl_xor(dbest, m);
-      const int oi = __shfl_xor(dbi, m);
-      if (ob > dbest || (ob == dbest && oi < dbi)) { dbest = ob; dbi = oi; }
+      v[i] = fma(v[i], inv_sn, bprev[i]) * kk;
+      mx = v[i] > mx ? v[i] : mx;
+    }
+    mx = wave_max(mx);
+    if (lane == 0) red[wv * 4] = mx;
+    __syncthreads();
+    const int w0 = wv & ~(QW - 1);
+    mx = combine_q<real, QW, true>(red, w0, 0);
+    real S = 0, S2 = 0;
+#pragma unroll
+    for (int i = 0; i < EQ; ++i) {
+      v[i] = dexp<real>(v[i] - mx);
+      S += v[i];
+      S2 += v[i] * v[i];
+    }
+    wave_sum2(S, S2);
+    if (lane == 0) {
+      red[wv * 4 + 1] = S;
+      red[wv * 4 + 2] = S2;
+    }
+    __syncthreads();
+    S = combine_q<real, QW, false>(red, w0, 1);
+    S2 = combine_q<real, QW, false>(red, w0, 2);
+    const real scale = cl * rcp_fast(S);
+#pragma unroll
+    for (int i = 0; i < EQ; ++i) v[i] = have ? v[i] * scale : (real)0;
+    if (have) store_section<real, EQ>(blo, v, lane, Mq);
+    bb = have ? S2 * scale * scale : (real)0;
+    if (a.dec) {
+#pragma unroll
+      for (int i = 0; i < EQ; ++i) {
+        const int e = eoff + elem_index<EQ>(lane, i);
+        if (v[i] > dbest || (v[i] == dbest && e < dbi)) { dbest = v[i]; dbi = e; }
+      }
+#pragma unroll
+      for (int m = 32; m >= 1; m >>= 1) {
+        const real ob = __shfl_xor(dbest, m);
+        const int oi = __shfl_xor(dbi, m);
+        if (ob > dbest || (ob == dbest && oi < dbi)) { dbest = ob; dbi = oi; }
+      }
     }
   }
 
   STAMP(5);
-  fwht_wave<real, EQ>(v, lane, 64);
-  topq_stage<real, EQ, QW>(v, xs, lane, q);
-  STAMP(6);
-  {
+  if (part != SEC_PART_EST) {
+    fwht_wave<real, EQ>(v, lane, 64);
+    topq_stage<real, EQ, QW>(v, xs, lane, q);
+    STAMP(6);
     real* tl = ts + sidx * M + eoff;
 #pragma unroll
     for (int i = 0; i < EQ; ++i) tl[elem_index<EQ>(lane, i)] = v[i];
   }
   if (lane == 0) {
-    red[wv * 4 + 3] = bb;
-    if (a.dec) {
-      red[wv * 4] = dbest;
-      red[wv * 4 + 1] = (real)dbi;
+    if constexpr (SPLIT) {
+      if (q == 0) {
+        red[wv * 4 + 3] = bb;
+      } else if (a.dec) {
+        red[wv * 4] = dbest;
+        red[wv * 4 + 3] = (real)dbi;
+      }
+    } else {
+      red[wv * 4 + 3] = bb;
+      if (a.dec) {
+        red[wv * 4] = dbest;
+        red[wv * 4 + 1] = (real)dbi;
+      }
     }
   }
   __syncthreads();
   STAMP(7);
   if (a.dec && have && q == 0 && lane == 0) {
-    real best = red[wv * 4];
-    int bi = (int)red[wv * 4 + 1];
+    constexpr int islot = SPLIT ? 3 : 1;
+    real best = SPLIT ? dbest : red[wv * 4];
+    int bi = SPLIT ? dbi : (int)red[wv * 4 + 1];
 #pragma unroll
     for (int j = 1; j < QW; ++j) {
       const real ob = red[(wv + j) * 4];
-      const int oi = (int)red[(wv + j) * 4 + 1];
+      const int oi = (int)red[(wv + j) * 4 + islot];
       if (ob > best || (ob == best && oi < bi)) { best = ob; bi = oi; }
     }
     a.dec[(size_t)b * a.L + l] = bi >= M ? 0 : bi;
   }
-  if (tid == 0) {
+  if (tid == 0 && part != SEC_PART_ROWS) {
     real bsum = red[0 * 4 + 3] + red[QW * 4 + 3];
     if constexpr (SPW >= 3) bsum += red[2 * QW * 4 + 3];
     if constexpr (SPW == 4) bsum += red[3 * QW * 4 + 3];
     a.bbp[(size_t)b * a.G + g] = bsum;
   }
+  if (part == SEC_PART_EST) return;
   real* abp = a.abp + ((size_t)b * a.G + g) * n;
   const int psh = a.pt == 16 ? 4 : 5;
   const size_t npad = (size_t)((n + (1 << psh) - 1) >> psh) << psh;
@@ -764,12 +793,12 @@
 #endif
 }
 
-template <typename real, int E4>
-__global__ void __launch_bounds__(512) k_sec4(SecArgs<real> a) { secq_body<real, E4, 4, 2>(a); }
-template <typename real, int E4>
-__global__ void __launch_bounds__(768) k_sec43(SecArgs<real> a) { secq_body<real, E4, 4, 3>(a); }
-template <typename real, int E4>
-__global__ void __launch_bounds__(1024) k_sec44(SecArgs<real> a) { secq_body<real, E4, 4, 4>(a); }
+template <typename real, int E4, bool SPLIT = false>
+__global__ void __launch_bounds__(512) k_sec4(SecArgs<real> a) { secq_body<real, E4, 4, 2, SPLIT>(a); }
+template <typename real, int E4, bool SPLIT = false>
+__global__ void __launch_bounds__(768) k_sec43(SecArgs<real> a) { secq_body<real, E4, 4, 3, SPLIT>(a); }
+template <typename real, int E4, bool SPLIT = false>
+__global__ void __launch_bounds__(1024) k_sec44(SecArgs<real> a) { secq_body<real, E4, 4, 4, SPLIT>(a); }
 
 template <typename real, int E>
 void launch_sec_e(sa_ctx* c, const Plan& p, int B, SecArgs<real> a) {
@@ -785,9 +814,14 @@
 
 template <typename real>
 int launch_sec2(sa_ctx* c, const Plan& p, int B, int t, int es, void* bin, void* bout, int bzero, int32_t* dec,
-                int itset) {
+                int itset, int part, const void* z, const void* zzp) {
   SecArgs<real> a = sec_args<real>(c, p, SEC_AMP, t, es);
   a.pt = p.pt;
+  if (part != SEC_PART_ALL && (!p.bzero() || es || c->dead))
+    return fail(SA_ERR_UNSUPPORTED, "launch_sec2: no split launch on this path");
+  a.mode = part;
+  if (z) a.z = (const real*)z;
+  if (zzp) a.zzp = (const real*)zzp;
   if (bzero && !p.bzero()) return fail(SA_ERR_UNSUPPORTED, "k_sec2 reads its previous estimate");
   if ((dec || itset) && (!p.bzero() || es || c->dead))
     return fail(SA_ERR_UNSUPPORTED, "launch_sec2: no fused decision on this path");
@@ -798,29 +832,57 @@
   a.beta_out = (real*)bout;
   a.G = p.G;
   dim3 grid(a.G, B);
+  const bool split = part != SEC_PART_ALL;
   if (c->prof) c->prof->begin(c->at().stream, K_SEC);
   switch (p.sec) {
     case SA_SEC_K_SEC43:
       switch (c->M / 256) {
-        case 1: plaunch(c, k_sec43<real, 1>, grid, 768, c->sec3_lds, a); break;
-        case 2: plaunch(c, k_sec43<real, 2>, grid, 768, c->sec3_lds, a); break;
+        case 1:
+          if (split) plaunch(c, k_sec43<real, 1, true>, grid, 768, c->sec3_lds, a);
+          else plaunch(c, k_sec43<real, 1>, grid, 768, c->sec3_lds, a);
+          break;
+        case 2:
+          if (split) plaunch(c, k_sec43<real, 2, true>, grid, 768, c->sec3_lds, a);
+          else plaunch(c, k_sec43<real, 2>, grid, 768, c->sec3_lds, a);
+          break;
         default: return fail(SA_ERR_UNSUPPORTED, "k_sec43: M");
       }
       break;
     case SA_SEC_K_SEC44:
       switch (c->M / 256) {
-        case 1: plaunch(c, k_sec44<real, 1>, grid, 1024, c->sec4q_lds, a); break;
-        case 2: plaunch(c, k_sec44<real, 2>, grid, 1024, c->sec4q_lds, a); break;
+        case 1:
+          if (split) plaunch(c, k_sec44<real, 1, true>, grid, 1024, c->sec4q_lds, a);
+          else plaunch(c, k_sec44<real, 1>, grid, 1024, c->sec4q_lds, a);
+          break;
+        case 2:
+          if (split) plaunch(c, k_sec44<real, 2, true>, grid, 1024, c->sec4q_lds, a);
+          else plaunch(c, k_sec44<real, 2>, grid, 1024, c->sec4q_lds, a);
+          break;
         default: return fail(SA_ERR_UNSUPPORTED, "k_sec44: M");
       }
       break;
     case SA_SEC_K_SEC4:
       switch (c->M / 256) {
-        case 1: plaunch(c, k_sec4<real, 1>, grid, 512, c->sec4_lds, a); break;
-        case 2: plaunch(c, k_sec4<real, 2>, grid, 512, c->sec4_lds, a); break;
-        case 4: plaunch(c, k_sec4<real, 4>, grid, 512, c->sec4_lds, a); break;
-        case 8: plaunch(c, k_sec4<real, 8>, grid, 512, c->sec4_lds, a); break;
-        case 16: plaunch(c, k_sec4<real, 16>, grid, 512, c->sec4_lds, a); break;
+        case 1:
+          if (split) plaunch(c, k_sec4<real, 1, true>, grid, 512, c->sec4_lds, a);
+          else plaunch(c, k_sec4<real, 1>, grid, 512, c->sec4_lds, a);
+          break;
+        case 2:
+          if (split) plaunch(c, k_sec4<real, 2, true>, grid, 512, c->sec4_lds, a);
+          else plaunch(c, k_sec4<real, 2>, grid, 512, c->sec4_lds, a);
+          break;
+        case 4:
+          if (split) plaunch(c, k_sec4<real, 4, true>, grid, 512, c->sec4_lds, a);
+          else plaunch(c, k_sec4<real, 4>, grid, 512, c->sec4_lds, a);
+          break;
+        case 8:
+          if (split) plaunch(c, k_sec4<real, 8, true>, grid, 512, c->sec4_lds, a);
+          else plaunch(c, k_sec4<real, 8>, grid, 512, c->sec4_lds, a);
+          break;
+        case 16:
+          if (split) plaunch(c, k_sec4<real, 16, true>, grid, 512, c->sec4_lds, a);
+          else plaunch(c, k_sec4<real, 16>, grid, 512, c->sec4_lds, a);
+          break;
         default: return fail(SA_ERR_UNSUPPORTED, "k_sec4: M");
       }
       break;
@@ -863,8 +925,10 @@
 
 template int launch_sec<float>(sa_ctx*, const Plan&, int, int, int, int, void*, void*);
 template int launch_sec<double>(sa_ctx*, const Plan&, int, int, int, int, void*, void*);
-template int launch_sec2<float>(sa_ctx*, const Plan&, int, int, int, void*, void*, int, int32_t*, int);
-template int launch_sec2<double>(sa_ctx*, const Plan&, int, int, int, void*, void*, int, int32_t*, int);
+template int launch_sec2<float>(sa_ctx*, const Plan&, int, int, int, void*, void*, int, int32_t*, int, int, const void*,
+                                const void*);
+template int launch_sec2<double>(sa_ctx*, const Plan&, int, int, int, void*, void*, int, int32_t*, int, int, const void*,
+                                 const void*);
 
 template <typename real>
 static hipError_t sec_lds_attrs_t() {
@@ -881,6 +945,10 @@
   SA_A((k_sec4<real, 16>))
   SA_A((k_sec43<real, 1>)) SA_A((k_sec43<real, 2>))
   SA_A((k_sec44<real, 1>)) SA_A((k_sec44<real, 2>))
+  SA_A((k_sec4<real, 1, true>)) SA_A((k_sec4<real, 2, true>)) SA_A((k_sec4<real, 4, true>)) SA_A((k_sec4<real, 8, true>))
+  SA_A((k_sec4<real, 16, true>))
+  SA_A((k_sec43<real, 1, true>)) SA_A((k_sec43<real, 2, true>))
+  SA_A((k_sec44<real, 1, true>)) SA_A((k_sec44<real, 2, true>))
 #undef SA_A
   return e;
 }
diff --git a/sparc_ldpc_amd/csrc/sparc_amp.hip b/sparc_ldpc_amd/csrc/sparc_amp.hip
--- a/sparc_ldpc_amd/csrc/sparc_amp.hip
+++ b/sparc_ldpc_amd/csrc/sparc_amp.hip
@@ -136,6 +136,7 @@
   if ((rc = dev_alloc(c, &l.d_abp, nBp * Gmax * ((size_t)c->NZ16 * kRow2Rows) * s))) return rc;
   if ((rc = dev_alloc(c, &l.d_bbp, nB * Gmax * s))) return rc;
   if ((rc = dev_alloc(c, &l.d_zzp, nB * c->NZh * s))) return rc;
+  if ((rc = dev_alloc(c, &l.d_yyp, nB * c->NZh * s))) return rc;
   if ((rc = dev_alloc(c, &l.d_tau, nB * (T + 1) * s))) return rc;
   if ((rc = dev_alloc(c, (void**)&l.d_iters, nB * sizeof(int)))) return rc;
   if (hipHostMalloc((void**)&l.h_dec, nB * c->L * sizeof(int32_t), hipHostMallocDefault) != hipSuccess ||
@@ -148,7 +149,8 @@
 }
 
 static void lane_free(sa_lane& l) {
-  void** bufs[] = {&l.d_y, &l.d_z, &l.d_beta, &l.d_beta2, &l.d_abp, &l.d_bbp, &l.d_zzp, &l.d_tau, (void**)&l.d_iters};
+  void** bufs[] = {&l.d_y,   &l.d_z,   &l.d_beta, &l.d_beta2, &l.d_abp,
+                   &l.d_bbp, &l.d_zzp, &l.d_yyp,  &l.d_tau,   (void**)&l.d_iters};
   for (void** p : bufs) {
     dev_free(*p);
     *p = nullptr;
@@ -157,6 +159,8 @@
   if (l.h_dec) (void)hipHostFree(l.h_dec);
   l.h_dec = l.d_dec = nullptr;
   l.fused_B = l.row_B = l.row_T = 0;
+  l.row_short = false;
+  l.yy_B = l.yy_nz = 0;
 }
 
 static void dec_rescue(sa_ctx* c, int k) {
@@ -364,6 +368,7 @@
   const bool bzero = !has_b0 && p.bzero() && T > 0;
   const int flip = (bzero && !es) ? (T & 1) : 0;
   const bool ft = fused_tail(c, p, T, flags);
+  const bool sc = short_chain(c, p, T, flags, has_b0);
   if (!it_row) k_fill32<<<(B + 255) / 256, 256, 0, ln.stream>>>((uint32_t*)ln.d_iters, 0xffffffffu, (size_t)B);
   if (has_b0) {
     if (dense) {
@@ -377,7 +382,7 @@
       const size_t nw = (size_t)B * c->L * c->M * rsz(c) / 4;
       k_fill32<<<(int)std::min<size_t>((nw + 255) / 256, 8192), 256, 0, ln.stream>>>((uint32_t*)ln.d_beta, 0u, nw);
     }
-    if ((rc = launch_row<real>(c, p, B, ROW_INIT0, 0, 0, p.G, p.Gb, it_row ? -1 : 0))) return rc;
+    if (!sc && (rc = launch_row<real>(c, p, B, ROW_INIT0, 0, 0, p.G, p.Gb, it_row ? -1 : 0))) return rc;
   }
   for (int t = 0; t < T; ++t) {
     if (dense) {
@@ -389,14 +394,19 @@
       void* pout = ((t ^ flip) & 1) ? ln.d_beta : ln.d_beta2;
       if (p.multiwave()) {
         const bool tail = ft && t == T - 1;
-        if ((rc = launch_sec2<real>(c, p, B, t, es, pin, pout, bzero && t == 0, tail ? ln.d_dec : nullptr, tail ? T : 0)))
+        const bool y0 = sc && t == 0;
+        if ((rc = launch_sec2<real>(c, p, B, t, es, pin, pout, bzero && t == 0, tail ? ln.d_dec : nullptr, tail ? T : 0,
+                                    sc && tail ? SEC_PART_EST : SEC_PART_ALL, y0 ? ln.d_y : nullptr,
+                                    y0 ? ln.d_yyp : nullptr)))
           return rc;
       } else if ((rc = launch_sec<real>(c, p, B, SEC_AMP, t, es, pin, pout))) {
         return rc;
       }
     }
     if (ft && t == T - 1) break;
-    if ((rc = launch_row<real>(c, p, B, ROW_AMP, t, es, p.G, p.Gb, it_row && t == T - 1 ? T : 0))) return rc;
+    if ((rc = launch_row<real>(c, p, B, ROW_AMP, t, es, p.G, p.Gb, it_row && t == T - 1 ? T : 0, nullptr,
+                               sc && t == 0 ? ln.d_y : nullptr)))
+      return rc;
   }
   if (!it_row) k_iters_final<<<(B + 255) / 256, 256, 0, ln.stream>>>(ln.d_iters, B, T);
   HIP_TRY(hipGetLastError());
@@ -414,21 +424,43 @@
   sa_lane& l = c->lane[k];
   if (!l.row_B) return SA_OK;
   const int B = l.row_B, T = l.row_T, keep = c->cur;
+  const bool sc = l.row_short;
   l.row_B = l.row_T = 0;
+  l.row_short = false;
   const Plan p = plan_for(c, B);
   lane_switch(c, k);
-  const int rc = c->prec == SA_PREC_F64 ? launch_row<double>(c, p, B, ROW_AMP, T - 1, 0, p.G, p.Gb, 0)
-                                        : launch_row<float>(c, p, B, ROW_AMP, T - 1, 0, p.G, p.Gb, 0);
+  int rc = SA_OK;
+  if (sc)
+    rc = c->prec == SA_PREC_F64
+             ? launch_sec2<double>(c, p, B, T - 1, 0, l.d_beta, l.d_beta, 0, nullptr, 0, SEC_PART_ROWS)
+             : launch_sec2<float>(c, p, B, T - 1, 0, l.d_beta, l.d_beta, 0, nullptr, 0, SEC_PART_ROWS);
+  const void* z_in = sc && T == 1 ? l.d_y : nullptr;
+  if (!rc)
+    rc = c->prec == SA_PREC_F64 ? launch_row<double>(c, p, B, ROW_AMP, T - 1, 0, p.G, p.Gb, 0, nullptr, z_in)
+                                : launch_row<float>(c, p, B, ROW_AMP, T - 1, 0, p.G, p.Gb, 0, nullptr, z_in);
   lane_switch(c, keep);
   return rc;
 }
 
-static void tail_mark(sa_ctx* c, int B, int T, int flags) {
+template <typename real>
+static int yy_refresh(sa_ctx* c, const Plan& p, int B) {
+  sa_lane& l = c->at();
+  if (l.yy_ver == l.y_ver && l.yy_nz == p.nz && l.yy_B >= B) return SA_OK;
+  if (int rc = launch_row<real>(c, p, B, ROW_INIT0, 0, 0, p.G, p.Gb, 0, nullptr, nullptr, l.d_yyp)) return rc;
+  l.yy_ver = l.y_ver;
+  l.yy_nz = p.nz;
+  l.yy_B = B;
+  return SA_OK;
+}
+
+static void tail_mark(sa_ctx* c, int B, int T, int flags, int has_b0) {
   sa_lane& ln = c->at();
-  const bool ft = fused_tail(c, plan_for(c, B), T, flags);
+  const Plan p = plan_for(c, B);
+  const bool ft = fused_tail(c, p, T, flags);
   ln.fused_B = ft ? B : 0;
   ln.row_B = ft ? B : 0;
   ln.row_T = ft ? T : 0;
+  ln.row_short = short_chain(c, p, T, flags, has_b0);
 }
 
 int ensure_beta2(sa_ctx* c, int B) {
@@ -456,17 +488,23 @@
   {
     sa_lane& l = c->at();
     l.row_B = l.row_T = 0;
+    l.row_short = false;
     if (int rcd = dec_spill(c, c->cur)) return rcd;
     l.fused_B = 0;
   }
   if (int rcy = y_sync(c)) return rcy;
+  {
+    const Plan p = plan_for(c, B);
+    if (short_chain(c, p, T, flags, has_b0))
+      if (int rcq = yy_refresh<real>(c, p, B)) return rcq;
+  }
   sa_lane& ln = c->at();
   if (c->plan & SA_PLAN_EAGER) {
     HIP_TRY(hipEventRecord(ln.ev0, ln.stream));
     int rc = seq_amp<real>(c, B, T, flags, has_b0);
     if (rc) return rc;
     HIP_TRY(hipEventRecord(ln.ev1, ln.stream));
-    tail_mark(c, B, T, flags);
+    tail_mark(c, B, T, flags, has_b0);
     c->last_B = B;
     c->last_T = T;
     c->zil_last = zil_for(c, B);
@@ -482,7 +520,7 @@
   HIP_TRY(hipEventRecord(ln.ev0, ln.stream));
   HIP_TRY(hipGraphLaunch(it->second, ln.stream));
   HIP_TRY(hipEventRecord(ln.ev1, ln.stream));
-  tail_mark(c, B, T, flags);
+  tail_mark(c, B, T, flags, has_b0);
   c->last_B = B;
   c->last_T = T;
   c->zil_last = zil_for(c, B);
@@ -1304,7 +1342,7 @@
     if (rc) return rc;
   }
   if (beta0) {
-    c->at().fused_B = 0;
+    if ((rc = beta_settle(c))) return rc;
     if ((rc = upload_sections(c, c->at().d_beta, beta0, B))) return rc;
   }
   return SA_OK;
@@ -1366,6 +1404,18 @@
   return SA_OK;
 }
 
+int sa_fetch_tau(sa_ctx* c, int B, int T, double* tau_out) {
+  if (check_ctx(c) || !tau_out) return fail(SA_ERR_ARG, "sa_fetch_tau: bad arguments");
+  if (B <= 0 || B > c->Bcap || T <= 0 || T > c->Tcap) return fail(SA_ERR_ARG, "sa_fetch_tau: bad batch or T");
+  HIP_TRY(hipSetDevice(c->device));
+  const size_t T1 = (size_t)c->Tcap + 1;
+  std::vector<double> all((size_t)B * T1);
+  if (int rc = download(c, all.data(), c->at().d_tau, all.size())) return rc;
+  HIP_TRY(hipStreamSynchronize(c->at().stream));
+  for (int b = 0; b < B; ++b) std::memcpy(tau_out + (size_t)b * T, all.data() + (size_t)b * T1, (size_t)T * sizeof(double));
+  return SA_OK;
+}
+
 int sa_fetch_y(sa_ctx* c, int B, double* y_out) {
   if (check_ctx(c) || !y_out) return fail(SA_ERR_ARG, "sa_fetch_y: bad arguments");
   if (B <= 0 || B > c->Bcap) return fail(SA_ERR_ARG, "sa_fetch_y: bad batch");
@@ -1398,7 +1448,7 @@
   if (rc) return rc;
   if ((rc = sa_stage(c, B, y, Pl, beta0))) return rc;
   if (T == 0) {
-    c->at().fused_B = 0;
+    if ((rc = beta_settle(c))) return rc;
     if (!beta0) HIP_TRY(hipMemsetAsync(c->at().d_beta, 0, (size_t)B * c->L * c->M * rsz(c), c->at().stream));
     HIP_TRY(hipMemsetAsync(c->at().d_iters, 0, (size_t)B * sizeof(int), c->at().stream));
   } else {
@@ -1422,6 +1472,7 @@
   if (int rcb = ensure_beta2(c, B)) return rcb;
   if (use_batched(c, B)) lane_switch(c, 0);
   c->at().row_B = c->at().row_T = 0;
+  c->at().row_short = false;
   c->at().fused_B = 0;
   if (int rcy = y_sync(c)) return rcy;
   if (use_batched(c, B))
@@ -1559,6 +1610,18 @@
   return SA_OK;
 }
 
+int sa_plan_run(sa_ctx* c, int B, int T, int flags, int64_t* o) {
+  if (check_ctx(c) || !o || B <= 0 || T < 0) return fail(SA_ERR_ARG, "sa_plan_run: bad arguments");
+  const Plan p = plan_for(c, B);
+  const int has_b0 = (flags & SA_FLAG_BETA0) ? 1 : 0, fl = flags & 0xff;
+  const bool ft = fused_tail(c, p, T, fl), sc = short_chain(c, p, T, fl, has_b0);
+  o[0] = decode_launches(c, p, T, fl, has_b0);
+  o[1] = ft ? 1 : 0;
+  o[2] = sc ? 1 : 0;
+  o[3] = ft ? (sc ? 2 : 1) : 0;
+  return SA_OK;
+}
+
 int sa_plan_batched(sa_ctx* c, int B, int64_t* o) {
   if (check_ctx(c) || !o || B <= 0) return fail(SA_ERR_ARG, "sa_plan_batched: bad arguments");
   if (is_dense(c) || !use_batched(c, B)) return fail(SA_ERR_ARG, "sa_plan_batched: this batch does not run k_secb");
diff --git a/sparc_ldpc_amd/operators.py b/sparc_ldpc_amd/operators.py
--- a/sparc_ldpc_amd/operators.py
+++ b/sparc_ldpc_amd/operators.py
@@ -272,6 +272,11 @@
         check(self._lib.sa_fetch_z(self._ctx, int(B), z.ctypes.data_as(_lib.ct.POINTER(_lib.ct.c_double))))
         return z
 
+    def fetch_tau(self, B, T):
+        tau = np.empty((B, int(T)))
+        check(self._lib.sa_fetch_tau(self._ctx, int(B), int(T), dptr(tau)))
+        return tau
+
     def fetch_y(self, B):
         y = np.empty((B, self.n))
         check(self._lib.sa_fetch_y(self._ctx, int(B), dptr(y)))
@@ -283,6 +288,12 @@
         return dict(section_kernel=self.SECTION_KERNELS[int(o[0])], partials=int(o[1]), row_splits=int(o[2]),
                     codewords_per_wg=int(o[3]), zz_partials=int(o[4]), w=int(o[5]),
                     row_kernel=self.ROW_KERNELS[int(o[6])], cus=int(o[7]))
+
+    def plan_run(self, B, T, early_stop=True, beta0=False):
+        flags = (0 if early_stop else _lib.SA_FLAG_NO_EARLY_STOP) | (_lib.SA_FLAG_BETA0 if beta0 else 0)
+        o = np.zeros(4, dtype=np.int64)
+        check(self._lib.sa_plan_run(self._ctx, int(B), int(T), flags, o.ctypes.data_as(_lib.ct.POINTER(_lib.ct.c_int64))))
+        return dict(launches=int(o[0]), fused_tail=bool(o[1]), short_chain=bool(o[2]), deferred_launches=int(o[3]))
 
     def mc_supported(self, B):
         if self.backend != "hadamard" or not 4 <= int(B) <= 1024:
```

Result: no change. 2383 codewords/s (median of 6 runs) (+0.4%).
